# DJjjjhao/FIRA-ICSE

Measured on AMD Instinct MI355X. Metric: training commits/sec (FIRA default config), higher is better.
Workload: dtype f32; 1 GPU; BASELINE configs[1]: FIRA training step (fwd+bwd+Adam, dropout 0.1/0.2), batch 32 commits/GPU, fp32, 650-node graphs (mean nnz 1066/graph), vocab 24650; global_batch=32, parallelism=dp1

## Files before the change

### fira_icse_amd/_lib.py

```python
from __future__ import annotations

import ctypes as C
import os

HERE = os.path.dirname(os.path.abspath(__file__))
LIB_PATH = os.environ.get("FIRA_HIP_LIB") or os.path.join(HERE, "libfira_hip.so")


class FiraError(RuntimeError):
    pass


class Dims(C.Structure):
    _fields_ = [("sou_len", C.c_int32), ("sub_len", C.c_int32), ("ast_len", C.c_int32), ("tar_len", C.c_int32),
                ("d_model", C.c_int32), ("n_head", C.c_int32), ("n_layer", C.c_int32), ("vocab", C.c_int32),
                ("ast_vocab", C.c_int32), ("d_ff", C.c_int32)]


class Batch(C.Structure):
    _fields_ = [("B", C.c_int32), ("nnz", C.c_int32), ("sou", C.c_void_p), ("tar", C.c_void_p), ("mark", C.c_void_p),
                ("ast_change", C.c_void_p), ("tar_label", C.c_void_p), ("sub_token", C.c_void_p),
                ("n_nodes", C.c_int32), ("node_rows", C.c_void_p), ("rowptr", C.c_void_p), ("col", C.c_void_p),
                ("val", C.c_void_p), ("n_code", C.c_int32), ("code_rows", C.c_void_p), ("code_mark", C.c_void_p),
                ("n_mem", C.c_int32), ("mem_rows", C.c_void_p), ("mem_dst", C.c_void_p), ("head_rows", C.c_void_p),
                ("n_head_rows", C.c_int32), ("n_emb_items", C.c_int32), ("emb_item_tok", C.c_void_p),
                ("emb_item_ptr", C.c_void_p), ("emb_rows", C.c_void_p), ("n_ast_items", C.c_int32),
                ("ast_rows", C.c_void_p), ("ast_ids", C.c_void_p), ("dec_off", C.c_void_p), ("n_dec_rows", C.c_int32),
                ("dec_off_host", C.c_void_p)]


class TrainOpts(C.Structure):
    _fields_ = [("dropout", C.c_float), ("gcn_dropout", C.c_float), ("seed", C.c_uint64), ("compact_head", C.c_int32),
                ("dtype", C.c_int32), ("compact_dec", C.c_int32), ("zero_grads", C.c_int32)]


class LrSchedule(C.Structure):
    _fields_ = [("kind", C.c_int32), ("base_lr", C.c_float), ("warmup_steps", C.c_int32), ("decay_steps", C.c_int32),
                ("min_lr", C.c_float)]


class AdamOpts(C.Structure):
    _fields_ = [("lr", C.c_float), ("beta1", C.c_float), ("beta2", C.c_float), ("eps", C.c_float), ("step", C.c_int32),
                ("m", C.c_void_p), ("v", C.c_void_p), ("sched", C.POINTER(LrSchedule))]


def sched_ptr(sched):
    return None if sched is None else C.pointer(sched)


class ClipState(C.Structure):
    _fields_ = [("sq", C.c_float * 4), ("norm", C.c_float), ("coef", C.c_float), ("zero_flag", C.c_int32),
                ("n_clipped", C.c_int32), ("n_nonfinite", C.c_int32), ("reserved", C.c_int32 * 7)]


_P, _I, _F, _L, _Z = C.c_void_p, C.c_int, C.c_float, C.c_int64, C.c_size_t
_U64, _U32 = C.c_uint64, C.c_uint32
_DP, _BP, _OP = C.POINTER(Dims), C.POINTER(Batch), C.POINTER(TrainOpts)

SIGNATURES = {
    "fira_last_error": (C.c_char_p, []),
    "fira_abi_version": (_I, []),
    "fira_param_count": (_I, [_DP]),
    "fira_param_info": (_I, [_DP, _I, C.c_char_p, C.POINTER(_L), C.POINTER(_L), C.POINTER(C.c_int32), C.POINTER(_L)]),
    "fira_param_total": (_L, [_DP]),
    "fira_workspace_bytes": (_Z, [_DP, _I, _I]),
    "fira_decode_workspace_bytes": (_Z, [_DP, _I, _I]),
    "fira_decode_workspace_bytes_ex": (_Z, [_DP, _I, _I, _I]),
    "fira_gemm_f32": (_I, [_P, _I, _I, _I, _I, _I, _P, _I, _P, _I, _P, _I, _P, _I, _I]),
    "fira_gemm_bf16": (_I, [_P, _I, _I, _I, _I, _I, _P, _I, _P, _I, _P, _I, _P, _I, _I]),
    "fira_weight_shadow": (_I, [_P, _I, _I, _P, _P, _P]),
    "fira_gemm_bf16_wb": (_I, [_P, _I, _I, _I, _P, _I, _P, _I, _P, _I, _P, _I, _I]),
    "fira_csr_spmm_f32": (_I, [_P, _I, _P, _P, _P, _P, _I, _P, _I, _I, _I]),
    "fira_csr_spmm": (_I, [_P, _I, _L, _P, _P, _P, _P, _I, _P, _I, _I, _I, _I]),
    "fira_gcn_layer_fwd": (_I, [_P, _I, _P, _P, _P, _P, _P, _P, _P, _P, _P, _P, _P, _P, _P, _F, _U64, _U32, _I]),
    "fira_gcn_layer_bwd": (_I, [_P, _I, _P, _P, _P, _P, _P, _P, _P, _I]),
    "fira_gcn_weight_planes": (_I, [_P, _I, _P, _P]),
    "fira_linear_x3": (_I, [_P, _I, _I, _P, _I, _P, _P, _P, _I, _I]),
    "fira_linear_dgrad_x3": (_I, [_P, _I, _I, _P, _I, _P, _P, _I, _I, _I]),
    "fira_dgrad_x3_splitk_planes_bytes": (_Z, [_I]),
    "fira_dgrad_x3_splitk": (_I, [_P, _I, _I, _P, _I, _P, _P, _P, _I, _I]),
    "fira_head_logits_x3_scratch_bytes": (_Z, [_I]),
    "fira_head_logits_x3": (_I, [_P, _I, _I, _P, _I, _P, _P, _P, _I, _P]),
    "fira_combination_block_fwd": (_I, [_P, _I, _P, _P, _P, _P, _P, _P, _P, _I, _P, _P, _P, _P, _P, _P, _P, _P, _P, _F, _U64, _U32, _U32, _I]),
    "fira_combination_block_bwd": (_I, [_P, _I, _P, _P, _P, _P, _P, _P, _P, _P, _P, _I, _P, _P, _P, _P, _P, _P, _I, _P, _F, _U64, _U32, _U32, _I]),
    "fira_combination_block_bwd_part_floats": (_I, []),
    "fira_embed_gather_fwd": (_I, [_P, _I, _I, _P, _P, _P, _P, _I, _I]),
    "fira_embed_gather_bwd": (_I, [_P, _I, _I, _P, _P, _P, _I, _I, _I]),
    "fira_combination_fwd": (_I, [_P, _I, _P, _P, _P, _P, _F, _U64, _U32]),
    "fira_combination_bwd": (_I, [_P, _I, _P, _P, _P, _P, _P, _P, _F, _U64, _U32]),
    "fira_add_layernorm_fwd": (_I, [_P, _I, _P, _P, _P, _P, _P, _P, _F, _U64, _U32]),
    "fira_linear_presum_f32": (_I, [_P, _I, _I, _P, _I, _P, _P, _P, _P, _F, _U64, _U32]),
    "fira_ln_linear_f32": (_I, [_P, _I, _I, _P, _I, _P, _P, _P, _I, _I, _P, _P, _P, _P]),
    "fira_ln_bwd_linear_f32": (_I, [_P, _I, _I, _P, _P, _P, _P, _P, _P, _P, _P, _P, _P, _P, _P, _F, _U64, _U32]),
    "fira_linear_layernorm_bf16_fwd": (_I, [_P, _I, _P, _I, _P, _I, _P, _P, _P, _P, _P, _P, _P, _F, _U64, _U32]),
    "fira_add_layernorm_bwd": (_I, [_P, _I, _P, _P, _P, _P, _P, _P, _P, _P, _F, _U64, _U32]),
    "fira_dropout_mask": (_I, [_P, _U64, _U32, _L, _F, _P]),
    "fira_colsum_f32": (_I, [_P, _I, _I, _P, _I, _P]),
    "fira_attention_fwd": (_I, [_P, _I, _I, _I, _I, _P, _I, _P, _I, _P, _I, _P, _I, _I, _P, _I]),
    "fira_attention_bwd": (_I, [_P, _I, _I, _I, _I, _P, _I, _P, _I, _P, _I, _P, _I, _I, _P, _I, _P, _I,
                                _P, _I, _P, _I, _P, _I]),
    "fira_attention_fwd_ex": (_I, [_P, _I, _I, _I, _I, _P, _I, _P, _I, _P, _I, _P, _I, _I, _P, _I, _P, _I, _I, _P]),
    "fira_attention_bwd_ex": (_I, [_P, _I, _I, _I, _I, _P, _I, _P, _I, _P, _I, _P, _I, _I, _P, _I, _P, _I,
                                   _P, _I, _P, _I, _P, _I, _P, _I, _I, _P]),
    "fira_decode_attention": (_I, [_P, _I, _I, _I, _P, _I, _P, _I, _P, _I, _P, _P, _I, _I, _I, _I, _P, _P, _I, _P, _P, _P]),
    "fira_copy_score_fwd": (_I, [_P, _I, _I, _I, _P, _P, _P, _P, _P]),
    "fira_copy_score_bwd": (_I, [_P, _I, _I, _I, _P, _P, _P, _P, _P, _P, _P, _P]),
    "fira_head_loss": (_I, [_P, _I, _I, _I, _I, _P, _P, _I, _P, _P, _P, _P, _P, _P, _P, _I]),
    "fira_adam_step": (_I, [_P, _L, _P, _P, _P, _P, _F, _F, _F, _F, _I, _P]),
    "fira_adam_step_mb": (_I, [_P, _L, _P, _P, _P, _P, _P, _F, _F, _F, _F, _I, _P, _P]),
    "fira_inv_count": (_I, [_P, _P, _P]),
    "fira_adam_step_count": (_I, [_P, _L, _P, _P, _P, _P, _F, _F, _F, _F, _I, _P]),
    "fira_pack_stats": (_I, [_P, _P, _P, _P]),
    "fira_debug_chain": (_I, [_P, _I, _I, _P]),
    "fira_train_fwd_bwd": (_I, [_P, _DP, _BP, _P, _P, _P, _Z, _OP, _P, _P, _P]),
    "fira_train_step": (_I, [_P, _DP, _BP, _P, _P, _P, _Z, _OP, _P, _P, C.POINTER(AdamOpts)]),
    "fira_gemm_wgrad_panel": (_I, [_P, _I, _I, _I, _I, _P, _I, _P, _I, _P, _I, _P, _P, _Z]),
    "fira_ffn_fwd": (_I, [_P, _I, _I] + [_P] * 11 + [_F, _U64, _U32, _I]),
    "fira_ffn_bwd": (_I, [_P, _I, _I] + [_P] * 17 + [_F, _U64, _U32, _I]),
    "fira_head_topk": (_I, [_P, _I, _I, _I, _P, _P, _P, _P, _I, _P, _P, _I]),
    "fira_train_step_rows": (_I, [_P, _DP, _BP, _P, _P, _P, _Z, _OP, _P, _P, C.POINTER(AdamOpts), _P]),
    "fira_adam_rows_sync": (_I, [_P, _DP, _P, C.POINTER(AdamOpts), _P]),
    "fira_adam_rows_catchup": (_I, [_P, _DP, _P, C.POINTER(AdamOpts), _P, _I, _P, _I]),
    "fira_adam_rows_step": (_I, [_P, _DP, _P, _P, C.POINTER(AdamOpts), _P, _P, _P, _I]),
    "fira_train_step_begin_rows": (_I, [_P, _DP, _BP, _P, _P, _P, _Z, _OP, _P, _P, _P, C.POINTER(AdamOpts), _P]),
    "fira_train_step_end_rows": (_I, [_P, _P, C.POINTER(AdamOpts), _P, _P, _P]),
    "fira_grad_sqsum_scratch_bytes": (_Z, []),
    "fira_grad_sqsum": (_I, [_P, _L, _P, _P, _I, _P]),
    "fira_clip_finish": (_I, [_P, _P, _I, _P, _P, _F]),
    "fira_adam_step_clip": (_I, [_P, _L, _P, _P, _P, _P, _F, _F, _F, _F, _I, _P, _P, _P]),
    "fira_adam_rows_step_clip": (_I, [_P, _DP, _P, _P, C.POINTER(AdamOpts), _P, _P, _P, _I, _P]),
    "fira_train_step_clip": (_I, [_P, _DP, _BP, _P, _P, _P, _Z, _OP, _P, _P, C.POINTER(AdamOpts), _P, _F, _P, _P]),
    "fira_lr_at": (_F, [C.POINTER(LrSchedule), _I]),
    "fira_lr_schedule_check": (_I, [C.POINTER(LrSchedule)]),
    "fira_train_step_begin": (_I, [_P, _DP, _BP, _P, _P, _P, _Z, _OP, _P, _P, _P]),
    "fira_train_step_end": (_I, [_P, _P, C.POINTER(AdamOpts), _P, _P]),
    "fira_f32_to_bf16": (_I, [_P, _L, _P, _P]),
    "fira_bf16_to_f32": (_I, [_P, _L, _P, _P]),
    "fira_prof_enable": (None, [_I]),
    "fira_prof_report": (_I, [_I, C.POINTER(C.c_double), C.POINTER(C.c_double), C.POINTER(C.c_double), C.POINTER(_L)]),
    "fira_param_groups": (_I, [_DP, C.POINTER(_L), C.POINTER(_L)]),
    "fira_host_node_lists": (_I, [_I, _I, _I, _I, _I] + [_P] * 7 + [_I] + [_P] * 14),
    "fira_host_collate_csr": (_I, [_I, _I, _P, _L, _P, _P, _P, _P, _P, _P, _P]),
    "fira_forward_dev": (_I, [_P, _DP, _BP, _P, _P, _Z, _P, _P, _P, _I]),
    "fira_dev_bleu_stats": (_I, [_P, _I, _I, _I, _I, _I, _P, _P, _P, _P, _P, _P]),
    "fira_mbr_bleu_stats": (_I, [_P, _I, _I, _I, _P, _P, _P]),
    "fira_constrain_dist": (_I, [_P, _DP, _I, _I, _P, _P, _P, _P, _I, _I, _P, _I, _P, _P, _P]),
    "fira_merge_dist": (_I, [_P, _DP, _I, _I, _P, _P, _P, _P, _P]),
    "fira_mix_dist": (_I, [_P, _I, _I, _I, C.POINTER(_P), C.POINTER(_F), _P, _P, _P]),
    "fira_decode_begin": (_I, [_P, _DP, _BP, _P, _P, _Z, _I]),
    "fira_decode_begin_ex": (_I, [_P, _DP, _BP, _P, _P, _Z, _I, _I]),
    "fira_decode_step_ex": (_I, [_P, _DP, _P, _P, _Z, _I, _I, _I, _P, _P, _P, _P, _P, _I]),
    "fira_beam_prepare": (_I, [_P, _I, _I, _I, _I, _P, _P, _P, _P, _P, _P]),
    "fira_beam_select": (_I, [_P, _DP, _I, _I, _P, _P, _P, _P, _P, _P, _P, _P, _P, _P, _P, _P, _P]),
    "fira_beam_select_scored": (_I, [_P, _DP, _I, _I, _P, _P, _P, _P, _P, _P, _P, _P, _P, _P, _P, _P, _P, _P, _I, _F, _P]),
    "fira_greedy_advance": (_I, [_P, _DP, _I, _I, _P, _P, _P, _P, _P, _P, _P, _P, _P, _P]),
    "fira_decode_step": (_I, [_P, _DP, _P, _P, _Z, _I, _I, _I, _P, _P, _P, _P, _P]),
    "fira_decode_step_sample": (_I, [_P, _DP, _P, _P, _Z, _I, _I, _I, _P, _P, _P, _F, _I, _F, _P, _P, _P, _I]),
    "fira_decode_step_score": (_I, [_P, _DP, _P, _P, _Z, _I, _I, _I] + [_P] * 15 + [_I]),
    "fira_sample_advance": (_I, [_P, _DP, _I, _I, _I, _P, _P, _P, _P, _P, _P, _P, _P, _P, _P, _P]),
    "fira_decoder_forward": (_I, [_P, _DP, _P, _P, _Z, _I, _P, _P, _P, _P]),
    "fira_decode_memory": (_P, [_DP, _P, _I, _I]),
    "fira_decode_mem_valid": (_P, [_DP, _P, _I, _I]),
}


def _ensure_built():
    if os.path.exists(LIB_PATH):
        return
    import fcntl
    from . import build as _build
    with open(os.path.join(HERE, ".build.lock"), "w") as lock:
        fcntl.flock(lock, fcntl.LOCK_EX)
        try:
            if not os.path.exists(LIB_PATH):
                _build.build()
        finally:
            fcntl.flock(lock, fcntl.LOCK_UN)


def load():
    try:
        _ensure_built()
    except Exception as e:
        raise ImportError(
            "fira_icse_amd: %s is missing and could not be built (%s). Build it with `python -m fira_icse_amd.build` "
            "(needs hipcc, gfx950). There is no CPU fallback." % (LIB_PATH, e))
    lib = C.CDLL(LIB_PATH)
    if lib.fira_abi_version() != 10:
        raise ImportError("libfira_hip.so ABI version mismatch")
    for name, (res, args) in SIGNATURES.items():
        fn = getattr(lib, name)
        fn.restype = res
        fn.argtypes = args
    return lib


_lib = None


def lib():
    global _lib
    if _lib is None:
        _lib = load()
    return _lib


_host_warned = False
_host_failed = False


def host_lib():
    global _host_warned, _host_failed
    if _host_failed:
        return None
    try:
        return lib()
    except (ImportError, OSError, AttributeError) as e:
        _host_failed = True
        if not _host_warned:
            _host_warned = True
            import warnings
            warnings.warn("fira_icse_amd: libfira_hip.so unavailable (%s); host collate falls back to numpy" % (e,))
        return None


def check(rc: int, what: str = ""):
    if rc != 0:
        msg = lib().fira_last_error()
        raise FiraError("%s failed: %s" % (what or "libfira_hip call", msg.decode() if msg else "unknown error"))


def ptr(t):
    return None if t is None else C.c_void_p(t.data_ptr())


def cur_stream():
    import torch
    return C.c_void_p(torch.cuda.current_stream().cuda_stream)


def make_dims(cfg) -> Dims:
    return Dims(cfg.sou_len, cfg.sub_token_len, cfg.ast_change_len, cfg.tar_len, cfg.embedding_dim, cfg.num_head,
                cfg.num_layers, cfg.vocab_size, cfg.ast_change_vocab_size, 4 * cfg.embedding_dim)
```

### fira_icse_amd/csrc/attention.hip

```cpp
#include "engine.h"
#include "epilogue.h"
#include "mfma_frag.h"

namespace fira {

constexpr float SQRT_DH = 5.656854249492381f;
constexpr float INV_SQRT_DH = 1.0f / SQRT_DH;
constexpr int MAX_TK = 384;

constexpr float LOG2E = 1.4426950408889634f;
constexpr float SCORE2 = INV_SQRT_DH * LOG2E;
constexpr float MASKED2 = -1e9f * LOG2E;
__device__ __forceinline__ constexpr int acc_c(int s) { return (s & 3) + 8 * (s >> 2); }
__device__ __forceinline__ uint32_t low_bits(int n) { return n <= 0 ? 0u : (n >= 32 ? 0xffffffffu : (1u << n) - 1u); }
__device__ __forceinline__ float bit_select(int sel, float a, float b) {
    return __int_as_float((sel & __float_as_int(a)) | (~sel & __float_as_int(b)));
}
__device__ __forceinline__ int bit_of(uint32_t word, int c) { return __builtin_amdgcn_sbfe((int)word, c, 1); }

__device__ __forceinline__ void buf_frag(float (&f)[16], rsrc_t r, unsigned off) {
#pragma unroll
    for (int i = 0; i < 4; ++i) {
        const f32x4v v = __builtin_bit_cast(f32x4v, __builtin_amdgcn_raw_buffer_load_b128(r, off + 16u * i, 0, 0));
        f[4 * i + 0] = v.x; f[4 * i + 1] = v.y; f[4 * i + 2] = v.z; f[4 * i + 3] = v.w;
    }
}
__device__ __forceinline__ void buf_rows(float (&f)[16], rsrc_t r, unsigned off0, unsigned ld4) {
#pragma unroll
    for (int s = 0; s < 16; ++s) f[s] = buf_load_f32(r, off0 + (unsigned)acc_c(s) * ld4);
}
__device__ __forceinline__ rsrc_t rows_rsrc(const float* base, int n, int ld) {
    return buf_rsrc(base, n > 0 ? (unsigned)(n - 1) * (unsigned)ld * 4u + 128u : 0u);
}

struct AttnRanges { int qb, tq, k0, tk; };
__device__ __forceinline__ AttnRanges attn_ranges(const int32_t* __restrict__ q_off, const int32_t* __restrict__ k_off, int b,
                                                  int bk, int Tq, int Tk, bool selfk, int lane) {
    int v = 0;
    const int32_t* src = nullptr;
    if (lane < 2 && q_off) src = q_off + b + lane;
    if (lane >= 2 && lane < 4 && k_off && !selfk) src = k_off + bk + (lane - 2);
    if (src) v = *src;
    AttnRanges r;
    r.qb = q_off ? __builtin_amdgcn_readlane(v, 0) : b * Tq;
    r.tq = q_off ? __builtin_amdgcn_readlane(v, 1) - r.qb : Tq;
    r.k0 = (k_off && !selfk) ? __builtin_amdgcn_readlane(v, 2) : 0;
    r.tk = selfk ? r.tq : (k_off ? min(__builtin_amdgcn_readlane(v, 3) - r.k0, Tk) : Tk);
    return r;
}

struct TileMask {
    bool ok;
    uint32_t valid;
    uint32_t outside;
    bool live;
};
__device__ __forceinline__ TileMask tile_mask(int kvld, int n_in, int kh) {
    TileMask m;
    m.ok = kvld != 0;
    const uint32_t vbits = (uint32_t)__ballot(m.ok);
    m.live = vbits != 0;
    m.valid = vbits >> (4 * kh);
    m.outside = ~low_bits(n_in) >> (4 * kh);
    return m;
}

template <int NW, bool BF>
__global__ __launch_bounds__(NW * 64) void attention_fwd_kernel(int H, int Tq, int Tk, const float* __restrict__ Q,
                                                                int ldq, const float* __restrict__ K, int ldk,
                                                                const float* __restrict__ V, int ldv,
                                                                const int32_t* __restrict__ key_valid, int causal,
                                                                int q_pos0, float* __restrict__ O, int ldo, int kb,
                                                                int kvb, int qpk, const int32_t* __restrict__ q_off,
                                                                int self_kv, const int32_t* __restrict__ k_off) {
    __shared__ float sm_red[NW][32];
    __shared__ float sm_o[NW > 1 ? NW * 1024 : 1];
    const int b = blockIdx.x / H, h = blockIdx.x % H;
    const int bk = b / qpk;
    const int t = threadIdx.x, lane = t & 63, wave = t >> 6;
    const int l31 = lane & 31, kh = lane >> 5;
    const bool selfk = q_off && self_kv;
    const AttnRanges rg = attn_ranges(q_off, k_off, b, bk, Tq, Tk, selfk, lane);
    const int qb = rg.qb, tq = rg.tq, k0 = rg.k0, tk = rg.tk;
    const int NT = (tk + 31) / 32;
    if (tk <= 0) {
        for (int idx = t; idx < tq * FIRA_DH; idx += NW * 64)
            O[((size_t)qb + idx / FIRA_DH) * ldo + h * FIRA_DH + idx % FIRA_DH] = 0.f;
        return;
    }
    const size_t krow0 = selfk ? (size_t)qb : (k_off ? (size_t)k0 : (size_t)bk * kb);
    const rsrc_t rQ = rows_rsrc(Q + (size_t)qb * ldq + h * FIRA_DH, tq, ldq);
    const rsrc_t rK = rows_rsrc(K + krow0 * ldk + h * FIRA_DH, tk, ldk);
    const rsrc_t rV = rows_rsrc(V + krow0 * ldv + h * FIRA_DH, tk, ldv);
    const rsrc_t rO = rows_rsrc(O + (size_t)qb * ldo + h * FIRA_DH, tq, ldo);
    const rsrc_t rM = buf_rsrc(key_valid + (k_off && !selfk ? (size_t)k0 : (size_t)bk * kvb), (unsigned)tk * 4u);
    const unsigned ldk4 = (unsigned)ldk * 4u, ldv4 = (unsigned)ldv * 4u, ldo4 = (unsigned)ldo * 4u;
    const int kt = wave;
    const bool mine = kt < NT;

    float bq[16], ak[16], vv[16];
    int kvld = 0;
    buf_frag(bq, rQ, (unsigned)l31 * (unsigned)ldq * 4u + (unsigned)kh * 64u);
    if (mine) {
        buf_frag(ak, rK, (unsigned)(kt * 32 + l31) * ldk4 + (unsigned)kh * 64u);
        buf_rows(vv, rV, (unsigned)(kt * 32 + 4 * kh) * ldv4 + (unsigned)l31 * 4u, ldv4);
        kvld = __builtin_amdgcn_raw_buffer_load_b32(rM, (unsigned)(kt * 32 + l31) * 4u, 0, 0);
    }
    const TileMask tm = tile_mask(kvld, tk - kt * 32, kh);
    const bool live = mine && tm.live;
    const uint32_t maskedT = ~tm.valid | (causal ? ~low_bits(l31 + q_pos0 - kt * 32 - 4 * kh + 1) : 0u);

    f32x16 st;
    float mx = -INFINITY;
    if (live) {
#pragma unroll
        for (int s = 0; s < 16; ++s) vv[s] = bit_select(bit_of(tm.valid, acc_c(s)), vv[s], 0.f);
        f32x16 acc;
#pragma unroll
        for (int r = 0; r < 16; ++r) acc[r] = 0.f;
        acc = chain16<BF>(ak, bq, acc);
#pragma unroll
        for (int r = 0; r < 16; ++r) {
            float x = bit_select(bit_of(maskedT, acc_c(r)), MASKED2, acc[r] * SCORE2);
            x = bit_select(bit_of(tm.outside, acc_c(r)), -INFINITY, x);
            st[r] = x;
            mx = fmaxf(mx, x);
        }
    } else {
#pragma unroll
        for (int r = 0; r < 16; ++r) {
            const float x = mine ? bit_select(bit_of(tm.outside, acc_c(r)), -INFINITY, MASKED2) : -INFINITY;
            st[r] = x;
            mx = fmaxf(mx, x);
        }
    }
    mx = fmaxf(mx, __shfl_xor(mx, 32, 64));
    if (NW > 1) {
        if (kh == 0) sm_red[wave][l31] = mx;
        __syncthreads();
#pragma unroll
        for (int w = 0; w < NW; ++w) mx = fmaxf(mx, sm_red[w][l31]);
        __syncthreads();
    }
    float sum = 0.f;
#pragma unroll
    for (int r = 0; r < 16; ++r) {
        const float p = __builtin_amdgcn_exp2f(st[r] - mx);
        st[r] = p;
        sum += p;
    }
    sum += __shfl_xor(sum, 32, 64);
    if (NW > 1) {
        if (kh == 0) sm_red[wave][l31] = sum;
        __syncthreads();
        sum = 0.f;
#pragma unroll
        for (int w = 0; w < NW; ++w) sum += sm_red[w][l31];
    }
    const float inv_sum = 1.0f / sum;
    f32x16 o;
#pragma unroll
    for (int r = 0; r < 16; ++r) o[r] = 0.f;
    if (live) {
        float pn[16];
#pragma unroll
        for (int s = 0; s < 16; ++s) pn[s] = st[s] * inv_sum;
        o = chain16<BF>(pn, vv, o);
    }
    if (NW > 1) {
        const int nwa = min(NW, NT);
        if (wave < nwa) {
#pragma unroll
            for (int r = 0; r < 16; ++r) sm_o[wave * 1024 + r * 64 + lane] = o[r];
        }
        __syncthreads();
        for (int idx = t; idx < 1024; idx += NW * 64) {
            float v = 0.f;
            for (int w = 0; w < nwa; ++w) v += sm_o[w * 1024 + idx];
            const int r = idx >> 6, ln = idx & 63;
            __builtin_amdgcn_raw_buffer_store_b32(__float_as_int(v), rO,
                                                  (unsigned)acc_row(r, ln >> 5) * ldo4 + (unsigned)(ln & 31) * 4u, 0, 0);
        }
    } else {
#pragma unroll
        for (int r = 0; r < 16; ++r)
            __builtin_amdgcn_raw_buffer_store_b32(__float_as_int(o[r]), rO,
                                                  (unsigned)(4 * kh + acc_c(r)) * ldo4 + (unsigned)l31 * 4u, 0, 0);
    }
}

template <int NW, bool BF>
__global__ __launch_bounds__(NW * 64) void attention_bwd_kernel(
    int H, int Tq, int Tk, const float* __restrict__ Q, int ldq, const float* __restrict__ K, int ldk,
    const float* __restrict__ V, int ldv, const int32_t* __restrict__ key_valid, int causal, int q_pos0,
    const float* __restrict__ O, int ldo, const float* __restrict__ dO, int lddo, float* __restrict__ dQ, int lddq,
    float* __restrict__ dK, int lddk, float* __restrict__ dV, int lddv, const int32_t* __restrict__ q_off, int self_kv,
    const int32_t* __restrict__ k_off) {
    __shared__ float sm_red[NW][32];
    __shared__ __attribute__((aligned(16))) float sm_m[32], sm_sum[32], sm_delta[32];
    __shared__ float sm_o[NW > 1 ? NW * 1024 : 1];
    const int b = blockIdx.x / H, h = blockIdx.x % H;
    const int t = threadIdx.x, lane = t & 63, wave = t >> 6;
    const int l31 = lane & 31, kh = lane >> 5;
    const bool selfk = q_off && self_kv;
    const AttnRanges rg = attn_ranges(q_off, k_off, b, b, Tq, Tk, selfk, lane);
    const int qb = rg.qb, tq = rg.tq, k0 = rg.k0, tk = rg.tk;
    const size_t kbase = selfk ? (size_t)qb : (k_off ? (size_t)k0 : (size_t)b * Tk);
    const int NT = (tk + 31) / 32;
    if (tk <= 0) {
        for (int idx = t; idx < tq * FIRA_DH; idx += NW * 64)
            dQ[((size_t)qb + idx / FIRA_DH) * lddq + h * FIRA_DH + idx % FIRA_DH] = 0.f;
        return;
    }
    const rsrc_t rQ = rows_rsrc(Q + (size_t)qb * ldq + h * FIRA_DH, tq, ldq);
    const rsrc_t rO = rows_rsrc(O + (size_t)qb * ldo + h * FIRA_DH, tq, ldo);
    const rsrc_t rdO = rows_rsrc(dO + (size_t)qb * lddo + h * FIRA_DH, tq, lddo);
    const rsrc_t rdQ = rows_rsrc(dQ + (size_t)qb * lddq + h * FIRA_DH, tq, lddq);
    const rsrc_t rK = rows_rsrc(K + kbase * ldk + h * FIRA_DH, tk, ldk);
    const rsrc_t rV = rows_rsrc(V + kbase * ldv + h * FIRA_DH, tk, ldv);
    const rsrc_t rdK = rows_rsrc(dK + kbase * lddk + h * FIRA_DH, tk, lddk);
    const rsrc_t rdV = rows_rsrc(dV + kbase * lddv + h * FIRA_DH, tk, lddv);
    const rsrc_t rM = buf_rsrc(key_valid + (k_off && !selfk ? (size_t)k0 : (size_t)b * Tk), (unsigned)tk * 4u);
    const unsigned ldq4 = (unsigned)ldq * 4u, ldk4 = (unsigned)ldk * 4u, ldv4 = (unsigned)ldv * 4u;
    const unsigned lddo4 = (unsigned)lddo * 4u, lddq4 = (unsigned)lddq * 4u, lddk4 = (unsigned)lddk * 4u, lddv4 = (unsigned)lddv * 4u;
    const int kt = wave;
    const bool mine = kt < NT;

    float bq[16], bdo[16], bo[16];
    const unsigned fq = (unsigned)kh * 64u;
    buf_frag(bq, rQ, (unsigned)l31 * ldq4 + fq);
    buf_frag(bdo, rdO, (unsigned)l31 * lddo4 + fq);
    buf_frag(bo, rO, (unsigned)l31 * (unsigned)ldo * 4u + fq);
    float ak[16], av[16], kvv[16];
    float qrow[16], dorow[16];
    int kvld = 0;
    if (mine) {
        const unsigned krow = (unsigned)(kt * 32 + l31);
        buf_frag(ak, rK, krow * ldk4 + fq);
        buf_frag(av, rV, krow * ldv4 + fq);
        buf_rows(kvv, rK, (unsigned)(kt * 32 + 4 * kh) * ldk4 + (unsigned)l31 * 4u, ldk4);
        kvld = __builtin_amdgcn_raw_buffer_load_b32(rM, krow * 4u, 0, 0);
        buf_rows(qrow, rQ, (unsigned)(4 * kh) * ldq4 + (unsigned)l31 * 4u, ldq4);
        buf_rows(dorow, rdO, (unsigned)(4 * kh) * lddo4 + (unsigned)l31 * 4u, lddo4);
    }
    const TileMask tm = tile_mask(kvld, tk - kt * 32, kh);
    const bool live = mine && tm.live;
    const uint32_t maskedT = ~tm.valid | (causal ? ~low_bits(l31 + q_pos0 - kt * 32 - 4 * kh + 1) : 0u);
    float delta;
    {
        float d = 0.f;
#pragma unroll
        for (int s = 0; s < 16; ++s) d = fmaf(bdo[s], bo[s], d);
        delta = d + __shfl_xor(d, 32, 64);
    }

    f32x16 st;
    float mx = -INFINITY;
    if (live) {
#pragma unroll
        for (int s = 0; s < 16; ++s) kvv[s] = bit_select(bit_of(tm.valid, acc_c(s)), kvv[s], 0.f);
        if (!tm.ok) {
#pragma unroll
            for (int s = 0; s < 16; ++s) { ak[s] = 0.f; av[s] = 0.f; }
        }
        f32x16 acc;
#pragma unroll
        for (int r = 0; r < 16; ++r) acc[r] = 0.f;
        acc = chain16<BF>(ak, bq, acc);
#pragma unroll
        for (int r = 0; r < 16; ++r) {
            float x = bit_select(bit_of(maskedT, acc_c(r)), MASKED2, acc[r] * SCORE2);
            x = bit_select(bit_of(tm.outside, acc_c(r)), -INFINITY, x);
            st[r] = x;
            mx = fmaxf(mx, x);
        }
    } else {
#pragma unroll
        for (int r = 0; r < 16; ++r) {
            const float x = mine ? bit_select(bit_of(tm.outside, acc_c(r)), -INFINITY, MASKED2) : -INFINITY;
            st[r] = x;
            mx = fmaxf(mx, x);
        }
    }
    mx = fmaxf(mx, __shfl_xor(mx, 32, 64));
    if (NW > 1) {
        if (kh == 0) sm_red[wave][l31] = mx;
        __syncthreads();
#pragma unroll
        for (int w = 0; w < NW; ++w) mx = fmaxf(mx, sm_red[w][l31]);
        __syncthreads();
    }
    float sum = 0.f;
#pragma unroll
    for (int r = 0; r < 16; ++r) {
        const float p = __builtin_amdgcn_exp2f(st[r] - mx);
        st[r] = p;
        sum += p;
    }
    sum += __shfl_xor(sum, 32, 64);
    if (NW > 1) {
        if (kh == 0) sm_red[wave][l31] = sum;
        __syncthreads();
        sum = 0.f;
#pragma unroll
        for (int w = 0; w < NW; ++w) sum += sm_red[w][l31];
    }
    const float inv_sum = 1.0f / sum;
    if (wave == 0 && kh == 0) {
        sm_m[l31] = mx;
        sm_sum[l31] = inv_sum;
        sm_delta[l31] = delta;
    }
    __syncthreads();

    f32x16 dq;
#pragma unroll
    for (int r = 0; r < 16; ++r) dq[r] = 0.f;
    if (live) {
        f32x16 dpt;
#pragma unroll
        for (int r = 0; r < 16; ++r) dpt[r] = 0.f;
        dpt = chain16<BF>(av, bdo, dpt);
        float dsv[16];
        const float sc = inv_sum * INV_SQRT_DH;
#pragma unroll
        for (int s = 0; s < 16; ++s)
            dsv[s] = bit_select(bit_of(maskedT, acc_c(s)), 0.f, st[s] * sc * (dpt[s] - delta));
        dq = chain16<BF>(dsv, kvv, dq);
    }
    if (NW > 1) {
        const int nwa = min(NW, NT);
        if (wave < nwa) {
#pragma unroll
            for (int r = 0; r < 16; ++r) sm_o[wave * 1024 + r * 64 + lane] = dq[r];
        }
        __syncthreads();
        for (int idx = t; idx < 1024; idx += NW * 64) {
            float v = 0.f;
            for (int w = 0; w < nwa; ++w) v += sm_o[w * 1024 + idx];
            const int r = idx >> 6, ln = idx & 63;
            __builtin_amdgcn_raw_buffer_store_b32(__float_as_int(v), rdQ,
                                                  (unsigned)acc_row(r, ln >> 5) * lddq4 + (unsigned)(ln & 31) * 4u, 0, 0);
        }
    } else {
#pragma unroll
        for (int r = 0; r < 16; ++r)
            __builtin_amdgcn_raw_buffer_store_b32(__float_as_int(dq[r]), rdQ,
                                                  (unsigned)(4 * kh + acc_c(r)) * lddq4 + (unsigned)l31 * 4u, 0, 0);
    }

    if (mine) {
        f32x16 dk, dv;
#pragma unroll
        for (int r = 0; r < 16; ++r) { dk[r] = 0.f; dv[r] = 0.f; }
        if (live) {
            float qm[16], qs[16], qd[16];
#pragma unroll
            for (int g = 0; g < 4; ++g) {
                const f32x4v m4 = *reinterpret_cast<const f32x4v*>(&sm_m[4 * kh + 8 * g]);
                const f32x4v s4 = *reinterpret_cast<const f32x4v*>(&sm_sum[4 * kh + 8 * g]);
                const f32x4v d4 = *reinterpret_cast<const f32x4v*>(&sm_delta[4 * kh + 8 * g]);
#pragma unroll
                for (int j = 0; j < 4; ++j) { qm[4 * g + j] = m4[j]; qs[4 * g + j] = s4[j]; qd[4 * g + j] = d4[j]; }
            }
            f32x16 sN, dpN;
#pragma unroll
            for (int r = 0; r < 16; ++r) { sN[r] = 0.f; dpN[r] = 0.f; }
            sN = chain16<BF>(bq, ak, sN);
            dpN = chain16<BF>(bdo, av, dpN);
            const int key = kt * 32 + l31;
            const uint32_t maskedN = tm.ok ? (causal ? low_bits(key - q_pos0 - 4 * kh) : 0u) : 0xffffffffu;
            const float gone = key < tk ? MASKED2 : -INFINITY;
            float pv[16], dsn[16];
#pragma unroll
            for (int s = 0; s < 16; ++s) {
                const int sel = bit_of(maskedN, acc_c(s));
                const float x = bit_select(sel, gone, sN[s] * SCORE2);
                const float p = __builtin_amdgcn_exp2f(x - qm[s]) * qs[s];
                pv[s] = p;
                dsn[s] = bit_select(sel, 0.f, p * (dpN[s] - qd[s]) * INV_SQRT_DH);
            }
            dk = chain16<BF>(dsn, qrow, dk);
            dv = chain16<BF>(pv, dorow, dv);
        }
#pragma unroll
        for (int r = 0; r < 16; ++r) {
            const unsigned row = (unsigned)(kt * 32 + 4 * kh + acc_c(r));
            __builtin_amdgcn_raw_buffer_store_b32(__float_as_int(dk[r]), rdK, row * lddk4 + (unsigned)l31 * 4u, 0, 0);
            __builtin_amdgcn_raw_buffer_store_b32(__float_as_int(dv[r]), rdV, row * lddv4 + (unsigned)l31 * 4u, 0, 0);
        }
    }
}

__device__ __forceinline__ f32x4v widen4(uint2 u) {
    return f32x4v{__uint_as_float(u.x << 16), __uint_as_float(u.x & 0xffff0000u), __uint_as_float(u.y << 16),
                  __uint_as_float(u.y & 0xffff0000u)};
}
template <int NSLOT, bool KV16>
__global__ __launch_bounds__(256) void decode_attention_kernel(int H, int Tk, const float* __restrict__ Q, int ldq,
                                                               const void* __restrict__ Kv, int ldk,
                                                               const void* __restrict__ Vv, int ldv,
                                                               const int32_t* __restrict__ key_valid, float* __restrict__ O,
                                                               int ldo, int kb, int kvb, int qpk,
                                                               const float* __restrict__ Knew,
                                                               const float* __restrict__ Vnew, int ldn,
                                                               float* __restrict__ Kc_out, float* __restrict__ Vc_out,
                                                               const int32_t* __restrict__ k_off) {
    __shared__ int sm_list[MAX_TK];
    __shared__ int sm_cnt[8];
    __shared__ float sm_f[4][36];
    const int bk = blockIdx.x / H, h = blockIdx.x % H;
    const int t = threadIdx.x, lane = t & 63, wave = t >> 6;
    const int r = lane >> 3, c = lane & 7;
    int nv;
    const int kbeg = k_off ? k_off[bk] : 0;
    if (k_off) Tk = min(Tk, k_off[bk + 1] - kbeg);
    const size_t krow0 = k_off ? (size_t)kbeg : (size_t)bk * kb;
    {
        const int32_t* kvp = key_valid + (k_off ? (size_t)kbeg : (size_t)bk * kvb);
        const int k0 = t, k1 = t + 256;
        const bool v0 = k0 < Tk && kvp[k0] != 0;
        const bool v1 = k1 < Tk && kvp[k1] != 0;
        const unsigned long long m0 = __ballot(v0), m1 = __ballot(v1);
        if (lane == 0) { sm_cnt[wave] = __popcll(m0); sm_cnt[4 + wave] = __popcll(m1); }
        __syncthreads();
        int base0 = 0, base1 = 0, tot0 = 0, tot1 = 0;
#pragma unroll
        for (int w = 0; w < 4; ++w) {
            const int c0 = sm_cnt[w], c1 = sm_cnt[4 + w];
            if (w < wave) { base0 += c0; base1 += c1; }
            tot0 += c0; tot1 += c1;
        }
        nv = tot0 + tot1;
        const unsigned long long below = (1ull << lane) - 1ull;
        if (v0) sm_list[base0 + __popcll(m0 & below)] = k0;
        if (v1) sm_list[tot0 + base1 + __popcll(m1 & below)] = k1;
        __syncthreads();
    }
    const size_t hoff = (size_t)h * FIRA_DH + c * 4;
    const float* K = static_cast<const float*>(Kv);
    const float* V = static_cast<const float*>(Vv);
    const float* Kb = K + krow0 * ldk + hoff;
    const float* Vb = V + krow0 * ldv + hoff;
    const uint16_t* Kh = static_cast<const uint16_t*>(Kv) + krow0 * ldk + hoff;
    const uint16_t* Vh = static_cast<const uint16_t*>(Vv) + krow0 * ldv + hoff;
    f32x4v kf[NSLOT], vf[NSLOT];
    bool have[NSLOT];
#pragma unroll
    for (int j = 0; j < NSLOT; ++j) {
        const int idx = j * 32 + wave * 8 + r;
        have[j] = idx < nv;
        const int key = have[j] ? sm_list[idx] : 0;
        const float* pk = Kb + (size_t)key * ldk;
        const float* pv = Vb + (size_t)key * ldv;
        if (Knew && key == Tk - 1) {
            pk = Knew + (size_t)bk * ldn + hoff;
            pv = Vnew + (size_t)bk * ldn + hoff;
        }
        if (KV16) {
            kf[j] = have[j] ? widen4(*reinterpret_cast<const uint2*>(Kh + (size_t)key * ldk)) : f32x4v{0.f, 0.f, 0.f, 0.f};
            vf[j] = have[j] ? widen4(*reinterpret_cast<const uint2*>(Vh + (size_t)key * ldv)) : f32x4v{0.f, 0.f, 0.f, 0.f};
        } else {
            kf[j] = have[j] ? *reinterpret_cast<const f32x4v*>(pk) : f32x4v{0.f, 0.f, 0.f, 0.f};
            vf[j] = have[j] ? *reinterpret_cast<const f32x4v*>(pv) : f32x4v{0.f, 0.f, 0.f, 0.f};
        }
    }
    if (Knew && Kc_out && t < 16) {
        const int cc = t & 7;
        const size_t src = (size_t)bk * ldn + (size_t)h * FIRA_DH + cc * 4;
        const size_t dst = ((size_t)bk * kb + (Tk - 1)) * ldk + (size_t)h * FIRA_DH + cc * 4;
        if (t < 8) *reinterpret_cast<f32x4v*>(Kc_out + dst) = *reinterpret_cast<const f32x4v*>(Knew + src);
        else *reinterpret_cast<f32x4v*>(Vc_out + ((size_t)bk * kb + (Tk - 1)) * ldv + (size_t)h * FIRA_DH + cc * 4) =
                 *reinterpret_cast<const f32x4v*>(Vnew + src);
    }
    for (int qi = 0; qi < qpk; ++qi) {
        const int b = bk * qpk + qi;
        const f32x4v q4 = *reinterpret_cast<const f32x4v*>(Q + (size_t)b * ldq + hoff);
        float sc[NSLOT];
        float mx = -INFINITY;
#pragma unroll
        for (int j = 0; j < NSLOT; ++j) {
            float d = q4.x * kf[j].x;
            d = fmaf(q4.y, kf[j].y, d); d = fmaf(q4.z, kf[j].z, d); d = fmaf(q4.w, kf[j].w, d);
            d = sum8(d);
            sc[j] = have[j] ? d * INV_SQRT_DH : -INFINITY;
            mx = fmaxf(mx, sc[j]);
        }
        mx = wave_max(mx);
        if (lane == 0) sm_f[wave][33] = mx;
        __syncthreads();
        mx = fmaxf(fmaxf(sm_f[0][33], sm_f[1][33]), fmaxf(sm_f[2][33], sm_f[3][33]));
        f32x4v acc = {0.f, 0.f, 0.f, 0.f};
        float sum = 0.f;
#pragma unroll
        for (int j = 0; j < NSLOT; ++j) {
            const float p = have[j] ? __expf(sc[j] - mx) : 0.f;
            sum += p;
            acc += vf[j] * p;
        }
        sum += dpp_take<DPP_ROR8, 0xf>(sum, sum);
        acc.x += dpp_take<DPP_ROR8, 0xf>(acc.x, acc.x); acc.y += dpp_take<DPP_ROR8, 0xf>(acc.y, acc.y);
        acc.z += dpp_take<DPP_ROR8, 0xf>(acc.z, acc.z); acc.w += dpp_take<DPP_ROR8, 0xf>(acc.w, acc.w);
#pragma unroll
        for (int o = 16; o < 64; o <<= 1) {
            sum += __shfl_xor(sum, o, 64);
            acc.x += __shfl_xor(acc.x, o, 64); acc.y += __shfl_xor(acc.y, o, 64);
            acc.z += __shfl_xor(acc.z, o, 64); acc.w += __shfl_xor(acc.w, o, 64);
        }
        if (lane < 8) {
            *reinterpret_cast<f32x4v*>(&sm_f[wave][lane * 4]) = acc;
            if (lane == 0) sm_f[wave][34] = sum;
        }
        __syncthreads();
        if (t < 32) {
            const float tot = (sm_f[0][34] + sm_f[1][34]) + (sm_f[2][34] + sm_f[3][34]);
            const float o = (sm_f[0][t] + sm_f[1][t]) + (sm_f[2][t] + sm_f[3][t]);
            O[(size_t)b * ldo + (size_t)h * FIRA_DH + t] = nv > 0 ? o / tot : 0.f;
        }
        __syncthreads();
    }
}

__global__ __launch_bounds__(256) void decode_self_block_kernel(int Tk, int T, const float* __restrict__ qkv,
                                                                float* __restrict__ Kc, float* __restrict__ Vc,
                                                                const int32_t* __restrict__ hist,
                                                                const float* __restrict__ WoT, const float* __restrict__ bo,
                                                                const float* __restrict__ xres,
                                                                const float* __restrict__ gamma, const float* __restrict__ beta,
                                                                const float* __restrict__ WqT, const float* __restrict__ bq,
                                                                float* __restrict__ xa, float* __restrict__ qc) {
    __shared__ __attribute__((aligned(16))) float s_q[FIRA_D], s_o[FIRA_D], s_x[FIRA_D];
    __shared__ float s_p[8][32];
    __shared__ float s_red[2][4];
    __shared__ __attribute__((aligned(16))) float s_part[4][FIRA_D];
    const int row = blockIdx.x, t = threadIdx.x, lane = t & 63, wave = t >> 6;
    const float* my = qkv + (size_t)row * 3 * FIRA_D;
    const float knew = my[FIRA_D + t], vnew = my[2 * FIRA_D + t];
    s_q[t] = my[t];
    float* kc_row = Kc + (size_t)row * T * FIRA_D;
    float* vc_row = Vc + (size_t)row * T * FIRA_D;
    kc_row[(size_t)(Tk - 1) * FIRA_D + t] = knew;
    vc_row[(size_t)(Tk - 1) * FIRA_D + t] = vnew;
    __syncthreads();
    {
        const int h = t >> 5, j = t & 31;
        const bool valid = j < Tk && hist[(size_t)row * T + j] != 0;
        const float* kp = (j == Tk - 1) ? my + FIRA_D + h * FIRA_DH : kc_row + (size_t)min(j, Tk - 1) * FIRA_D + h * FIRA_DH;
        float d = 0.f;
#pragma unroll
        for (int c = 0; c < FIRA_DH / 4; ++c) {
            const f32x4v k4 = *reinterpret_cast<const f32x4v*>(kp + c * 4);
            const f32x4v q4 = *reinterpret_cast<const f32x4v*>(&s_q[h * FIRA_DH + c * 4]);
            d = fmaf(q4.x, k4.x, d); d = fmaf(q4.y, k4.y, d); d = fmaf(q4.z, k4.z, d); d = fmaf(q4.w, k4.w, d);
        }
        const float sc = valid ? d * INV_SQRT_DH : -INFINITY;
        float mx = sc;
#pragma unroll
        for (int o = 1; o < 32; o <<= 1) mx = fmaxf(mx, __shfl_xor(mx, o, 64));
        const float pr = valid ? __expf(sc - mx) : 0.f;
        float sum = pr;
#pragma unroll
        for (int o = 1; o < 32; o <<= 1) sum += __shfl_xor(sum, o, 64);
        s_p[h][j] = sum > 0.f ? pr / sum : 0.f;
    }
    __syncthreads();
    {
        const int h = t >> 5;
        float o = 0.f;
        int j = 0;
        for (; j + 4 <= Tk - 1; j += 4) {
            const float v0 = vc_row[(size_t)j * FIRA_D + t], v1 = vc_row[(size_t)(j + 1) * FIRA_D + t];
            const float v2 = vc_row[(size_t)(j + 2) * FIRA_D + t], v3 = vc_row[(size_t)(j + 3) * FIRA_D + t];
            o = fmaf(s_p[h][j], v0, o); o = fmaf(s_p[h][j + 1], v1, o); o = fmaf(s_p[h][j + 2], v2, o); o = fmaf(s_p[h][j + 3], v3, o);
        }
        for (; j < Tk - 1; ++j) o = fmaf(s_p[h][j], vc_row[(size_t)j * FIRA_D + t], o);
        o = fmaf(s_p[h][Tk - 1], vnew, o);
        s_o[t] = o;
    }
    __syncthreads();
    auto matvec = [&](const float* __restrict__ WT, const float* v, float bias_n) -> float {
        f32x4v acc = {0.f, 0.f, 0.f, 0.f};
        const float* wp = WT + (size_t)(wave * 64) * FIRA_D + lane * 4;
#pragma unroll
        for (int k0 = 0; k0 < 64; k0 += 16) {
            f32x4v w[16];
#pragma unroll
            for (int u = 0; u < 16; ++u) w[u] = *reinterpret_cast<const f32x4v*>(wp + (size_t)(k0 + u) * FIRA_D);
#pragma unroll
            for (int u = 0; u < 16; ++u) acc += w[u] * v[wave * 64 + k0 + u];
        }
        __syncthreads();
        *reinterpret_cast<f32x4v*>(&s_part[wave][lane * 4]) = acc;
        __syncthreads();
        return bias_n + ((s_part[0][t] + s_part[1][t]) + (s_part[2][t] + s_part[3][t]));
    };
    const float sres = matvec(WoT, s_o, bo[t]) + xres[(size_t)row * FIRA_D + t];
    float part = wave_sum(sres);
    if (lane == 0) s_red[0][wave] = part;
    __syncthreads();
    const float mean = ((s_red[0][0] + s_red[0][1]) + (s_red[0][2] + s_red[0][3])) * (1.0f / FIRA_D);
    const float dv = sres - mean;
    part = wave_sum(dv * dv);
    if (lane == 0) s_red[1][wave] = part;
    __syncthreads();
    const float var = ((s_red[1][0] + s_red[1][1]) + (s_red[1][2] + s_red[1][3])) * (1.0f / FIRA_D);
    const float y = dv * (1.0f / sqrtf(var + 1e-5f)) * gamma[t] + beta[t];
    xa[(size_t)row * FIRA_D + t] = y;
    s_x[t] = y;
    __syncthreads();
    qc[(size_t)row * FIRA_D + t] = matvec(WqT, s_x, bq[t]);
}
int decode_self_block(hipStream_t s, int BR, int Tk, int T, const float* qkv, float* Kc, float* Vc, const int32_t* hist,
                      const float* WoT, const float* bo, const float* xres, const float* gamma, const float* beta,
                      const float* WqT, const float* bq, float* xa, float* qc) {
    ProfScope prof(s, PROF_ATTN, 0.0);
    if (BR <= 0) return 0;
    FIRA_REQUIRE(Tk >= 1 && Tk <= 32 && Tk <= T, "decode_self_block: %d keys (at most 32)", Tk);
    hipLaunchKernelGGL(decode_self_block_kernel, dim3(BR), dim3(256), 0, s, Tk, T, qkv, Kc, Vc, hist, WoT, bo, xres, gamma, beta,
                       WqT, bq, xa, qc);
    FIRA_CHECK_LAUNCH("decode_self_block");
    return 0;
}

int decode_attention_kv16(hipStream_t s, int BR, int H, int Tk, const float* Q, int ldq, const uint16_t* K, int ldk,
                          const uint16_t* V, int ldv, const int32_t* key_valid, float* O, int ldo, int kb, int kvb, int qpk,
                          const int32_t* k_off) {
    ProfScope prof(s, PROF_ATTN, 0.0);
    if (BR <= 0) return 0;
    FIRA_REQUIRE(Tk >= 1 && Tk <= MAX_TK && qpk >= 1 && BR % qpk == 0 && kb >= Tk && kvb >= Tk, "decode_attention: bad geometry");
    FIRA_REQUIRE(ldq % 4 == 0 && ldk % 4 == 0 && ldv % 4 == 0 && (uintptr_t)Q % 16 == 0 && (uintptr_t)K % 8 == 0 &&
                     (uintptr_t)V % 8 == 0, "decode_attention: rows must be 8-byte (bf16) / 16-byte (fp32) aligned");
    const dim3 grid((BR / qpk) * H);
    if (Tk <= 32)
        hipLaunchKernelGGL((decode_attention_kernel<1, true>), grid, dim3(256), 0, s, H, Tk, Q, ldq, K, ldk, V, ldv, key_valid, O,
                           ldo, kb, kvb, qpk, nullptr, nullptr, 0, nullptr, nullptr, k_off);
    else
        hipLaunchKernelGGL((decode_attention_kernel<12, true>), grid, dim3(256), 0, s, H, Tk, Q, ldq, K, ldk, V, ldv, key_valid, O,
                           ldo, kb, kvb, qpk, nullptr, nullptr, 0, nullptr, nullptr, k_off);
    FIRA_CHECK_LAUNCH("decode_attention_kv16");
    return 0;
}
int decode_attention(hipStream_t s, int BR, int H, int Tk, const float* Q, int ldq, const float* K, int ldk,
                     const float* V, int ldv, const int32_t* key_valid, float* O, int ldo, int kb, int kvb, int qpk,
                     const float* Knew, const float* Vnew, int ldn, float* Kc_out, float* Vc_out, const int32_t* k_off) {
    ProfScope prof(s, PROF_ATTN, 0.0);
    if (BR <= 0) return 0;
    FIRA_REQUIRE(Tk >= 1 && Tk <= MAX_TK && qpk >= 1 && BR % qpk == 0 && kb >= Tk && kvb >= Tk, "decode_attention: bad geometry");
    FIRA_REQUIRE(ldq % 4 == 0 && ldk % 4 == 0 && ldv % 4 == 0 && (uintptr_t)Q % 16 == 0 && (uintptr_t)K % 16 == 0 &&
                     (uintptr_t)V % 16 == 0 && (!Knew || (ldn % 4 == 0 && (uintptr_t)Knew % 16 == 0 && (uintptr_t)Vnew % 16 == 0)),
                 "decode_attention: rows must be 16-byte aligned");
    FIRA_REQUIRE(!Knew || (qpk == 1 && !k_off), "decode_attention: merged new keys need one query per K/V entry and dense key rows");
    const dim3 grid((BR / qpk) * H);
    if (Tk <= 32)
        hipLaunchKernelGGL((decode_attention_kernel<1, false>), grid, dim3(256), 0, s, H, Tk, Q, ldq, K, ldk, V, ldv, key_valid, O,
                           ldo, kb, kvb, qpk, Knew, Vnew, ldn, Kc_out, Vc_out, k_off);
    else
        hipLaunchKernelGGL((decode_attention_kernel<12, false>), grid, dim3(256), 0, s, H, Tk, Q, ldq, K, ldk, V, ldv, key_valid, O,
                           ldo, kb, kvb, qpk, Knew, Vnew, ldn, Kc_out, Vc_out, k_off);
    FIRA_CHECK_LAUNCH("decode_attention");
    return 0;
}

static int check_geometry(const char* who, int Tq, int Tk, int ldq, int ldk, int ldv, const void* Q, const void* K,
                          const void* V) {
    FIRA_REQUIRE(Tq >= 1 && Tq <= 32, "%s: Tq=%d must be in 1..32", who, Tq);
    FIRA_REQUIRE(Tk >= 1 && Tk <= MAX_TK, "%s: Tk=%d must be in 1..%d", who, Tk, MAX_TK);
    FIRA_REQUIRE(ldq % 4 == 0 && ldk % 4 == 0 && ldv % 4 == 0 && (uintptr_t)Q % 16 == 0 && (uintptr_t)K % 16 == 0 &&
                     (uintptr_t)V % 16 == 0,
                 "%s: Q/K/V rows must be 16-byte aligned", who);
    return 0;
}

int attention_fwd_ex(hipStream_t s, int B, int H, int Tq, int Tk, const float* Q, int ldq, const float* K, int ldk,
                     const float* V, int ldv, const int32_t* key_valid, int causal, int q_pos0, float* O, int ldo,
                     int kb, int kvb, int qpk, const int32_t* q_off, int self_kv, int bf16, const int32_t* k_off) {
    ProfScope prof(s, PROF_ATTN, 0.0);
    if (B <= 0) return 0;
    if (int e = check_geometry("attention_fwd", Tq, Tk, ldq, ldk, ldv, Q, K, V)) return e;
    FIRA_REQUIRE(kb >= Tk && kvb >= Tk && qpk >= 1, "attention_fwd: bad batch strides");
#define FIRA_ATT_FWD(NW_, BF_)                                                                                      \
    hipLaunchKernelGGL((attention_fwd_kernel<NW_, BF_>), dim3(B * H), dim3(NW_ * 64), 0, s, H, Tq, Tk, Q, ldq, K, ldk, V, \
                       ldv, key_valid, causal, q_pos0, O, ldo, kb, kvb, qpk, q_off, self_kv, k_off)
    if (Tk <= 32) { if (bf16) FIRA_ATT_FWD(1, true); else FIRA_ATT_FWD(1, false); }
    else { if (bf16) FIRA_ATT_FWD(12, true); else FIRA_ATT_FWD(12, false); }
#undef FIRA_ATT_FWD
    FIRA_CHECK_LAUNCH("attention_fwd");
    return 0;
}
int attention_fwd(hipStream_t s, int B, int H, int Tq, int Tk, const float* Q, int ldq, const float* K, int ldk,
                  const float* V, int ldv, const int32_t* key_valid, int causal, int q_pos0, float* O, int ldo,
                  const int32_t* q_off, int self_kv, int bf16, const int32_t* k_off) {
    return attention_fwd_ex(s, B, H, Tq, Tk, Q, ldq, K, ldk, V, ldv, key_valid, causal, q_pos0, O, ldo, Tk, Tk, 1, q_off, self_kv,
                            bf16, k_off);
}

int attention_bwd(hipStream_t s, int B, int H, int Tq, int Tk, const float* Q, int ldq, const float* K, int ldk,
                  const float* V, int ldv, const int32_t* key_valid, int causal, int q_pos0, const float* O, int ldo,
                  const float* dO, int lddo, float* dQ, int lddq, float* dK, int lddk, float* dV, int lddv,
                  const int32_t* q_off, int self_kv, int bf16, const int32_t* k_off) {
    ProfScope prof(s, PROF_ATTN, 0.0);
    if (B <= 0) return 0;
    if (int e = check_geometry("attention_bwd", Tq, Tk, ldq, ldk, ldv, Q, K, V)) return e;
    FIRA_REQUIRE(ldo % 4 == 0 && lddo % 4 == 0 && (uintptr_t)O % 16 == 0 && (uintptr_t)dO % 16 == 0,
                 "attention_bwd: O/dO rows must be 16-byte aligned");
#define FIRA_ATT_BWD(NW_, BF_)                                                                                      \
    hipLaunchKernelGGL((attention_bwd_kernel<NW_, BF_>), dim3(B * H), dim3(NW_ * 64), 0, s, H, Tq, Tk, Q, ldq, K, ldk, V, \
                       ldv, key_valid, causal, q_pos0, O, ldo, dO, lddo, dQ, lddq, dK, lddk, dV, lddv, q_off, self_kv, k_off)
    if (Tk <= 32) { if (bf16) FIRA_ATT_BWD(1, true); else FIRA_ATT_BWD(1, false); }
    else { if (bf16) FIRA_ATT_BWD(12, true); else FIRA_ATT_BWD(12, false); }
#undef FIRA_ATT_BWD
    FIRA_CHECK_LAUNCH("attention_bwd");
    return 0;
}

}

extern "C" {
int fira_attention_fwd(void* stream, int B, int H, int Tq, int Tk, const float* Q, int ldq, const float* K, int ldk,
                       const float* V, int ldv, const int32_t* key_valid, int causal, int q_pos0, float* O, int ldo) {
    return fira::attention_fwd((hipStream_t)stream, B, H, Tq, Tk, Q, ldq, K, ldk, V, ldv, key_valid, causal, q_pos0, O,
                               ldo);
}
int fira_decode_attention(void* stream, int BR, int H, int Tk, const float* Q, int ldq, const float* K, int ldk,
                          const float* V, int ldv, const int32_t* key_valid, float* O, int ldo, int kb, int kvb, int qpk,
                          const float* Knew, const float* Vnew, int ldn, float* Kc_out, float* Vc_out,
                          const int32_t* k_off) {
    FIRA_REQUIRE(Q && K && V && key_valid && O, "fira_decode_attention: null pointer argument");
    return fira::decode_attention((hipStream_t)stream, BR, H, Tk, Q, ldq, K, ldk, V, ldv, key_valid, O, ldo, kb, kvb, qpk, Knew,
                                  Vnew, ldn, Kc_out, Vc_out, k_off);
}
int fira_attention_bwd(void* stream, int B, int H, int Tq, int Tk, const float* Q, int ldq, const float* K, int ldk,
                       const float* V, int ldv, const int32_t* key_valid, int causal, int q_pos0, const float* O,
                       int ldo, const float* dO, int lddo, float* dQ, int lddq, float* dK, int lddk, float* dV,
                       int lddv) {
    return fira::attention_bwd((hipStream_t)stream, B, H, Tq, Tk, Q, ldq, K, ldk, V, ldv, key_valid, causal, q_pos0, O,
                               ldo, dO, lddo, dQ, lddq, dK, lddk, dV, lddv);
}
int fira_attention_fwd_ex(void* stream, int B, int H, int Tq, int Tk, const float* Q, int ldq, const float* K, int ldk,
                          const float* V, int ldv, const int32_t* key_valid, int causal, int q_pos0, float* O, int ldo,
                          const int32_t* q_off, int self_kv, int dtype, const int32_t* k_off) {
    FIRA_REQUIRE(dtype == FIRA_F32 || dtype == FIRA_BF16, "fira_attention_fwd_ex: dtype must be FIRA_F32 or FIRA_BF16");
    FIRA_REQUIRE(!(k_off && self_kv), "fira_attention_fwd_ex: k_off (ragged memory rows) and self_kv exclude each other");
    return fira::attention_fwd((hipStream_t)stream, B, H, Tq, Tk, Q, ldq, K, ldk, V, ldv, key_valid, causal, q_pos0, O,
                               ldo, q_off, self_kv, dtype == FIRA_BF16, k_off);
}
int fira_attention_bwd_ex(void* stream, int B, int H, int Tq, int Tk, const float* Q, int ldq, const float* K, int ldk,
                          const float* V, int ldv, const int32_t* key_valid, int causal, int q_pos0, const float* O,
                          int ldo, const float* dO, int lddo, float* dQ, int lddq, float* dK, int lddk, float* dV,
                          int lddv, const int32_t* q_off, int self_kv, int dtype, const int32_t* k_off) {
    FIRA_REQUIRE(dtype == FIRA_F32 || dtype == FIRA_BF16, "fira_attention_bwd_ex: dtype must be FIRA_F32 or FIRA_BF16");
    FIRA_REQUIRE(!(k_off && self_kv), "fira_attention_bwd_ex: k_off (ragged memory rows) and self_kv exclude each other");
    return fira::attention_bwd((hipStream_t)stream, B, H, Tq, Tk, Q, ldq, K, ldk, V, ldv, key_valid, causal, q_pos0, O,
                               ldo, dO, lddo, dQ, lddq, dK, lddk, dV, lddv, q_off, self_kv, dtype == FIRA_BF16, k_off);
}
}
```

### fira_icse_amd/csrc/engine.h

```cpp
#pragma once
#include "common.h"
#include <string>
#include <vector>

namespace fira {

int gemm_f32(hipStream_t s, int tA, int tB, int M, int N, int K, const float* A, int lda, const float* B, int ldb,
             float* C, int ldc, const float* bias, int flags, int splitk);
int gemm_f32_ex(hipStream_t s, int tA, int tB, int M, int N, int K, const float* A, int lda, const float* B, int ldb,
                float* C, int ldc, const float* bias, int flags, int splitk, float* colsum,
                const int32_t* c_rows = nullptr, const float* relu_mask = nullptr);
int gemm_bf16_ex(hipStream_t s, int tA, int tB, int M, int N, int K, const float* A, int lda, const float* B, int ldb,
                 float* C, int ldc, const float* bias, int flags, int splitk, float* colsum,
                 const int32_t* c_rows = nullptr, const float* relu_mask = nullptr);
struct ShadowEntry { int64_t offset; int rows, cols, pitch_t; int64_t offset_t; };
constexpr int SHADOW_MAX = 64;
struct ShadowTable {
    int n = 0;
    int64_t wbt_elems = 0;
    int tile_start[SHADOW_MAX + 1] = {0};
    ShadowEntry e[SHADOW_MAX];
};
int weight_shadows(hipStream_t s, const ShadowTable& tab, const float* P, uint16_t* Wb, uint16_t* WbT);
int gemm_bf16_wb_ex(hipStream_t s, int M, int N, int K, const float* A, int lda, const uint16_t* Bb, int ldb, float* C,
// ... 1 lines not shown
                    const float* relu_mask = nullptr);
int gemm_bf16_group_add_wgrad(hipStream_t s, int M, int N, int K, const float* A, int lda, const float* B, int ldb,
                              float* C, int ldc, float* colsum, int max_split = 0);
int gemm_bf16_group_flush(hipStream_t s);
bool gemm_bf16_takes(int M, int N, int K);
void gemm_bf16_group_reset();
bool gemm_bf16_group_full();
bool gemm_wgrad_panel_takes(int M, int N, int K, const float* A, int lda, const float* B, int ldb, int ldc);
void gemm_wgrad_panel_reset();
bool gemm_wgrad_panel_full();
int gemm_wgrad_panel_pending();
int gemm_wgrad_panel_add(int M, int N, int K, const float* A, int lda, const float* B, int ldb, float* C, int ldc, float* colsum);
int gemm_wgrad_panel_flush(hipStream_t s, int np);
void gemm_wgrad_panel_scratch(float* buf, size_t n_floats);
int gemm_wgrad_panel(hipStream_t s, int np, int M, int N, int K, const float* A, int lda, const float* B, int ldb, float* C,
                     int ldc, float* colsum);
int gemm_group_add_wgrad(hipStream_t s, int M, int N, int K, const float* A, int lda, const float* B, int ldb, float* C,
                         int ldc, float* colsum, int max_split = 0);
int gemm_group_flush(hipStream_t s);
void gemm_group_reset();
bool gemm_group_full();
void gemm_set_pad_stream(hipStream_t s);
struct EpiRes;
bool gemm_tile32_takes(int tB, int M, int N, int K, const float* A, int lda, const float* B, int ldb);
bool gemm_tile32_try(hipStream_t s, int tB, int M, int N, int K, const float* A, int lda, const float* B, int ldb,
                     float* C, int ldc, const float* bias, int flags, int* rc, const int32_t* c_rows,
                     const float* relu_mask, const int32_t* a_rows, const EpiRes* er);
bool gemm_tile32_ln_try(hipStream_t s, int M, int N, const float* S, int lds, const float* W, const float* bias, float* Y,
                        int ldy, int flags, const float* gamma, const float* beta, float* x_out, float* stats_out, int* rc);
int gemm_tile32_lnb_blocks(int M);
bool gemm_tile32_lnb_try(hipStream_t s, int M, int N, const float* dy, const float* W, int ldw, float* dX, int lddx,
                         const float* relu_mask, const float* sum, const float* stats, const float* gamma, float* ds,
                         float* dx_drop, float* part, float dropout, uint64_t seed, uint32_t site, int* rc,
                         uint32_t idx0 = 0);
bool gemm_small_try(hipStream_t s, int tA, int tB, int M, int N, int K, const float* A, int lda, const float* B, int ldb,
                    float* C, int ldc, const float* bias, int flags, int* rc, const int32_t* c_rows = nullptr,
                    const float* relu_mask = nullptr);
int csr_spmm(hipStream_t s, int n_rows, const int32_t* rowptr, const int32_t* col, const float* val, const float* X,
             int ldx, float* Y, int ldy, int graph_rows, int variant);
int csr_spmm_ex(hipStream_t s, int n_rows, const int32_t* rowptr, const int32_t* col, const float* val, const float* X,
                int ldx, float* Y, int ldy, int graph_rows, int variant, int accum, float* rowsum);
int gcn_fused_fwd(hipStream_t s, int n_rows, const int32_t* rowptr, const int32_t* col, const float* val, const float* X,
                  const float* Wk, const float* bias, const float* r1_col, const float* gamma, const float* beta, float* sum,
                  float* y, float* stats, float* rowsum_out, const int32_t* slot2, float* y2, float dropout, uint64_t seed,
                  uint32_t site, int bf16, const uint16_t* Wx = nullptr);
int gcn_fused_bwd(hipStream_t s, int n_rows, const int32_t* rowptr, const int32_t* col, const float* val, const float* dY,
                  const float* Wk, float* u_out, float* acc_out, int bf16, const uint16_t* Wx = nullptr);
int gcn_split_planes(hipStream_t s, int n, const float* const* src, uint16_t* const* dst);
size_t head_logits_x3_scratch_elems(int R);
int head_logits_x3(hipStream_t s, int R, int V, const float* x, int ldx, const float* W, const float* bias, float* out, int ldo,
                   uint16_t* xplanes);
int transpose256(hipStream_t s, int nl, const float* W, float* Wt);
int linear_x3(hipStream_t s, int M, const float* X, int ldx, const uint16_t* Wx, int nb, const float* bias, float* out, int ldo,
              bool one_plane);
int split_planes_t(hipStream_t s, const float* W, int V, uint16_t* planes, bool one_plane);
int dgrad_x3_splitk(hipStream_t s, int M, int K, const float* A, int lda, const uint16_t* Wx, float* out, int ldo, bool one_plane);
int linear_x3_kacc(hipStream_t s, int M, const float* A, int lda, const uint16_t* Wx, int nkb, float* out, int ldo, bool accum,
                   bool one_plane);
int comb_fused_fwd(hipStream_t s, int n_rows, const float* Xc, const float* WqT, const float* WkT, const float* WoT,
                   const float* bqk, const float* bo, const float* vtab, int ldv, const int32_t* mark, float* qk, float* c,
                   const float* gamma, const float* beta, float* sum, float* y, const int32_t* y_rows, float* stats,
                   float dropout, uint64_t seed, uint32_t site_gate, uint32_t site_out, int bf16, const uint16_t* Wx = nullptr);
int comb_fused_bwd_parts();
int comb_fused_bwd(hipStream_t s, int n_rows, float* dG, const int32_t* rows, const float* sum, const float* stats,
                   const float* gamma, const float* Wo, const float* Wqk, const float* qk, const float* vtab, int ldv,
                   const int32_t* mark, float* dYc, float* dqk, float* part_ln, float* part_v, float dropout, uint64_t seed,
                   uint32_t site_gate, uint32_t site_out, int bf16, const uint16_t* WTx = nullptr);
struct TransposeTable { int n = 0; const float* src[24]; float* dst[24]; };
int transpose256_table(hipStream_t s, const TransposeTable& tab);
int embed_gather_fwd(hipStream_t s, int B, int L, const int32_t* idx, const float* table, const float* pos, float* out,
                     int out_bstride, int out_off);
int embed_grouped_bwd(hipStream_t s, int n_items, const int32_t* item_tok, const int32_t* item_ptr, const int32_t* rows,
                      float* dtable, const float* dnode);
int embed_list_bwd_small(hipStream_t s, int n, const int32_t* rows, const int32_t* ids, float* dtable, const float* dnode,
                         int table_rows);
int embed_gather_bwd(hipStream_t s, int B, int L, const int32_t* idx, float* dtable, const float* dout,
                     int out_bstride, int out_off, int padding_idx);
int embed_gather_bwd_small(hipStream_t s, int B, int L, const int32_t* idx, float* dtable, const float* dout,
                           int out_bstride, int out_off, int padding_idx, int table_rows);
int combination_fwd(hipStream_t s, int M, const float* qk, const float* vtab, int ldv, const int32_t* mark, float* out,
                    float dropout, uint64_t seed, uint32_t site);
int combination_bwd(hipStream_t s, int M, const float* qk, const float* vtab, int ldv, const int32_t* mark,
                    const float* dout, float* dqk, float* dvtab, int lddv, float dropout, uint64_t seed, uint32_t site,
                    float* part = nullptr);
int combination_bwd_blocks(int M);
struct RedEntry { float* dst; const float* src; int width, n_part, stride; };
constexpr int RED_MAX = 96;
struct RedTable {
    int n = 0;
    int wg_start[RED_MAX + 1] = {0};
    RedEntry e[RED_MAX];
};
int deferred_reduce(hipStream_t s, RedTable& tab);
int add_layernorm_fwd(hipStream_t s, int M, float* x, const float* res, const float* gamma, const float* beta,
                      float* y, float* stats, float dropout, uint64_t seed, uint32_t site, const int32_t* y_rows, const float* r1_row = nullptr,
                      const float* r1_col = nullptr,
                      const int32_t* slot2 = nullptr, float* y2 = nullptr,
                      uint32_t idx0 = 0);
bool gemm_bf16_k256_try(hipStream_t s, int M, int N, int K, const float* A, int lda, const uint16_t* Bb, int ldb, float* C,
                        int ldc, const float* bias, int flags, const int32_t* c_rows, const float* relu_mask, int* rc);
bool linear_ln_bf16_try(hipStream_t s, int M, int K, const float* X, int ldx, const uint16_t* Wb, int ldb, const float* bias,
                        const float* res, const float* gamma, const float* beta, float* sum, float* y, float* stats,
                        float dropout, uint64_t seed, uint32_t site, const int32_t* y_rows, const float* r1_row,
                        const float* r1_col, int* rc, bool force = false);
int add_layernorm_bwd(hipStream_t s, int M, const float* dy, const float* sum, const float* stats, const float* gamma,
                      float* ds, float* dx_drop, float* dgamma, float* dbeta, float dropout, uint64_t seed,
                      uint32_t site, const int32_t* rows = nullptr,
                      float* part = nullptr,
                      const float* row_w = nullptr, uint32_t idx0 = 0);
int add_layernorm_bwd_blocks(int M);
int gcn_bias_unfold(hipStream_t s, const float* W2, const float* b1, const float* dc, float* dW2, float* db1);
struct UnfoldEntry { const float *W2, *b1, *dc; float *dW2, *db1; };
struct UnfoldTable { int n = 0; UnfoldEntry e[16]; };
int gcn_bias_unfold_all(hipStream_t s, const UnfoldTable& tab);
int gcn_fold_weights(hipStream_t s, int n_layers, const float* const* W2, const float* const* W1, const float* const* b1,
                     float* W21, float* W21t, float* c21);
int gcn_unfold_products(hipStream_t s, int n_layers, const float* const* dW21, const float* const* W1, const float* const* W2,
                        float* const* dW1, float* const* dW2);
int colsum(hipStream_t s, int M, int N, const float* X, int ldx, float* out, const float* row_weight = nullptr);
int rank2_rows(hipStream_t s, int M, const float* g, const float* w, float* out);
int prep(hipStream_t s, int B, int L, int S, int T, const int32_t* sou, const int32_t* sub, const int32_t* tar,
         int32_t* mem_valid, int32_t* tar_valid, float* pos_code, float* pos_tar, int R, const int32_t* rows,
         int32_t* compact_row, int32_t* iota, float* loss_sum = nullptr, int32_t* n_tok = nullptr,
         int Nc = 0, const int32_t* code_rows = nullptr, int Cc = 0, int32_t* code_slot = nullptr,
         const int32_t* mem_rows = nullptr, int Mc = 0, int32_t* mem_slot = nullptr,
         const int32_t* dec_off = nullptr, int32_t* row_bt = nullptr, int32_t* rows_c = nullptr,
         const int32_t* mem_dst = nullptr, int32_t* mem_off = nullptr, int32_t* mem_valid_c = nullptr);
struct AdamRowsView;
int embed_rows_fwd(hipStream_t s, int R, int T, const int32_t* row_bt, const int32_t* idx, const float* table,
                   const float* pos, float* out, const AdamRowsView* vw = nullptr);
int embed_rows_bwd(hipStream_t s, int R, const int32_t* row_bt, const int32_t* idx, float* dtable, const float* dout,
                   int padding_idx);
int node_features(hipStream_t s, int Nc, const int32_t* node_rows, int N, int L, int S, const int32_t* sou,
                  const int32_t* sub, const int32_t* ast, const float* emb, const float* ast_emb, const float* pos_code,
                  float* X, const int32_t* slot2 = nullptr, float* X2 = nullptr,
                  const AdamRowsView* vw = nullptr);
int rows_move(hipStream_t s, int mode, int R, int W, float* out, const float* in, const int32_t* src, const int32_t* dst);
int rows_move_ld(hipStream_t s, int mode, int R, int W, float* out, int ld_out, const float* in, int ld_in,
                 const int32_t* src, const int32_t* dst);
int rows_gather_idx(hipStream_t s, int R, float* compact, const float* src, const int32_t* rows);
int rows_scatter_add_idx(hipStream_t s, int R, const float* compact, float* dst, const int32_t* rows);
int fill_pos_tables(hipStream_t s, int L, float* pos_code, int T, float* pos_tar);
int tar_mask(hipStream_t s, int n, const int32_t* tar, int32_t* valid);
int permute_cache(hipStream_t s, int nl, int BR, int T, int len, const int32_t* parent, const float* ksrc,
                  const float* vsrc, float* kdst, float* vdst, const int32_t* hist_src, int32_t* hist_dst);
int mark_history(hipStream_t s, int BR, int T, int step, const int32_t* tokens, int32_t* hist);
int decode_embed(hipStream_t s, int BR, int T, int step, const int32_t* tokens, const float* table, const float* pos_row,
                 float* x, int32_t* hist);

int attention_fwd(hipStream_t s, int B, int H, int Tq, int Tk, const float* Q, int ldq, const float* K, int ldk,
                  const float* V, int ldv, const int32_t* key_valid, int causal, int q_pos0, float* O, int ldo,
                  const int32_t* q_off = nullptr, int self_kv = 0,
                  int bf16 = 0,
                  const int32_t* k_off = nullptr);
int attention_fwd_ex(hipStream_t s, int B, int H, int Tq, int Tk, const float* Q, int ldq, const float* K, int ldk,
                     const float* V, int ldv, const int32_t* key_valid, int causal, int q_pos0, float* O, int ldo,
                     int kb, int kvb, int qpk, const int32_t* q_off = nullptr, int self_kv = 0, int bf16 = 0,
                     const int32_t* k_off = nullptr);
int decode_attention(hipStream_t s, int BR, int H, int Tk, const float* Q, int ldq, const float* K, int ldk,
                     const float* V, int ldv, const int32_t* key_valid, float* O, int ldo, int kb, int kvb, int qpk,
                     const float* Knew = nullptr, const float* Vnew = nullptr, int ldn = 0, float* Kc_out = nullptr,
                     float* Vc_out = nullptr, const int32_t* k_off = nullptr);
int decode_self_block(hipStream_t s, int BR, int Tk, int T, const float* qkv, float* Kc, float* Vc, const int32_t* hist,
                      const float* WoT, const float* bo, const float* xres, const float* gamma, const float* beta,
                      const float* WqT, const float* bq, float* xa, float* qc);
int decode_attention_kv16(hipStream_t s, int BR, int H, int Tk, const float* Q, int ldq, const uint16_t* K, int ldk,
                          const uint16_t* V, int ldv, const int32_t* key_valid, float* O, int ldo, int kb, int kvb, int qpk,
                          const int32_t* k_off = nullptr);
int rows_to_bf16(hipStream_t s, int64_t n, const float* in, uint16_t* out);
int rows_from_bf16(hipStream_t s, int64_t n, const uint16_t* in, float* out);
int attention_bwd(hipStream_t s, int B, int H, int Tq, int Tk, const float* Q, int ldq, const float* K, int ldk,
                  const float* V, int ldv, const int32_t* key_valid, int causal, int q_pos0, const float* O, int ldo,
                  const float* dO, int lddo, float* dQ, int lddq, float* dK, int lddk, float* dV, int lddv,
                  const int32_t* q_off = nullptr, int self_kv = 0, int bf16 = 0, const int32_t* k_off = nullptr);
int copy_score_fwd(hipStream_t s, int B, int T, int S, const float* src, const float* tgt, const float* w,
                   const float* bias, float* score);
int copy_score_fwd_ex(hipStream_t s, int B, int T, int S, const float* src, const float* tgt, const float* w,
                      const float* bias, float* score, int qpk, const int32_t* mem_valid,
                      const int32_t* tar_label = nullptr, int V = 0,
                      const int32_t* t_off = nullptr);
int copy_score_bwd_ex(hipStream_t s, int B, int T, int S, const float* src, const float* tgt, const float* w,
                      const float* dscore, float* dsrc, float* dtgt, float* dw, float* dbias, const int32_t* mem_valid,
                      float* part = nullptr, const int32_t* t_off = nullptr);
int copy_score_bwd_blocks(int B, int S);
constexpr int COPY_PART_STRIDE = 264;
int decode_dist(hipStream_t s, int R, int V, int S, const float* logits, int ldl, const float* score,
                const int32_t* mem_valid, int qpk, const float* gate_logits, float* dist, int32_t* best_id,
                float* best_p, const float* x = nullptr, const float* wp = nullptr, const float* bp = nullptr);
int inv_count(hipStream_t s, const int32_t* n_tok, float* out);
int sample_dist(hipStream_t s, int R, int n_sample, int V, int S, const float* logits, int ldl, const float* score,
                const int32_t* mem_valid, const float* x, const float* wp, const float* bp, int T, int step,
                const int32_t* key, const uint64_t* seed_dev, float temperature, int top_k, float top_p, float* dist,
                int32_t* best_id, float* best_p);
int score_dist(hipStream_t s, int R, int n_cand, int V, int L, int S, const float* logits, int ldl, const float* score,
               const int32_t* mem_valid, const float* x, const float* wp, const float* bp, const int32_t* target,
               const int32_t* label, const int32_t* sou, const int32_t* sub, float* dist, float* p_word, float* p_entry,
               int32_t* entry, float* copy_share, float* p_label, int32_t* top_id, float* logp_word, float* logp_entry,
               float* logp_label);
int row_topk(hipStream_t s, int R, int V, int k, const float* logits, int ldl, int32_t* ids, float* vals);
int copy_score_bwd(hipStream_t s, int B, int T, int S, const float* src, const float* tgt, const float* w,
                   const float* dscore, float* dsrc, float* dtgt, float* dw, float* dbias);
int head_loss(hipStream_t s, int BT, int T, int V, int S, const int32_t* compact_row, float* logits, int ldl,
              float* score, const int32_t* mem_valid, float* gate_logits, const int32_t* tar_label, float* loss_sum,
              int32_t* n_tok, int32_t* argmax_out, int want_grad,
              const int32_t* row_bt = nullptr);
int adam_step(hipStream_t s, int64_t n, float* p, const float* g, float* m, float* v, float lr, float beta1,
              float beta2, float eps, int step, const float* scale_ptr, int scale_is_count = 0);
int adam_step_mb(hipStream_t s, int64_t n, float* p, const float* g0, const float* g1, float* m, float* v, float lr,
                 float beta1, float beta2, float eps, int step, const int32_t* n0, const int32_t* n1);
constexpr int ADAM_ROWS_K = 32;
struct AdamRowsHist { float bc1[ADAM_ROWS_K], bc2s[ADAM_ROWS_K], lr[ADAM_ROWS_K]; };
struct AdamLr {
    float lr = 0.f;
    bool scheduled = false;
    fira_lr_schedule sched{};
    float at(int step) const { return scheduled ? fira_lr_at(&sched, step) : lr; }
};
inline AdamLr adam_lr(const fira_adam_opts& ad) {
    AdamLr r;
    r.lr = ad.lr;
    if (ad.sched) { r.scheduled = true; r.sched = *ad.sched; }
    return r;
}
struct AdamRowsTables { float *p, *m, *v; int64_t off[2]; int rows[2]; int32_t* last; };
struct AdamRowsView {
    const float *m = nullptr, *v = nullptr;
    const int32_t* last = nullptr;
    int to = 0;
    float beta1 = 0.f, beta2 = 0.f, eps = 0.f, gz = 0.f;
    AdamRowsHist h;
};
AdamRowsView adam_rows_view(const AdamRowsTables& tb, int table, const AdamLr& lr, float beta1, float beta2, float eps, int to);
struct AdamRowsLists { int n_lists; int end[4]; int table[4]; const int32_t* ids[4]; };
int adam_rows_step(hipStream_t s, const AdamRowsTables& tb, const float* g, const AdamLr& lr, float beta1, float beta2, float eps,
                   int step, const int32_t* n0, const float* count, int tables = 3);
int adam_rows_catchup(hipStream_t s, const AdamRowsTables& tb, const AdamRowsLists* ls, const AdamLr& lr, float beta1, float beta2,
                      float eps, int to);
AdamRowsHist adam_rows_hist(const AdamLr& lr, float beta1, float beta2, int end);
struct ClipClose {
    const int32_t* n_tok;
    const float* count;
    float max_norm;
    int n_slots;
};
size_t grad_sqsum_scratch_bytes();
int grad_sqsum(hipStream_t s, int64_t n, const float* g, fira_clip_state* st, int slot, void* scratch, const ClipClose* fin);
int clip_finish(hipStream_t s, fira_clip_state* st, const ClipClose& fin);
int adam_step_clip(hipStream_t s, int64_t n, float* p, const float* g, float* m, float* v, float lr, float beta1, float beta2,
                   float eps, int step, const int32_t* n0, const float* count, const fira_clip_state* st);
int adam_rows_step_clip(hipStream_t s, const AdamRowsTables& tb, const float* g, const AdamLr& lr, float beta1, float beta2, float eps,
                        int step, const int32_t* n0, const float* count, int tables, const fira_clip_state* st);

struct ParamInfo {
    std::string name;
    int64_t offset = -1, numel = 0;
    int ndim = 0;
    int64_t shape[2] = {0, 0};
};

struct EncLayer {
    int64_t wqk, bqk, w2, b2, wo, bo, ln1g, ln1b, fc1w, fc1b, fc2w, fc2b, ln2g, ln2b;
};
struct DecLayer {
    int64_t wqkv, bqkv, wo_s, bo_s, lns_g, lns_b, wq_c, bq_c, wkv_c, bkv_c, wo_c, bo_c, lnc_g, lnc_b, w1, b1, w2, b2,
        lnf_g, lnf_b;
};
struct Layout {
    fira_dims d;
    std::vector<ParamInfo> infos;
    int64_t total = 0;
    int64_t split = 0, live = 0;
    int64_t emb, ast_emb, mark_emb, w2_all, b2_all, dec_emb, wkv_all, bkv_all, wout, bout, ws, wt, wres, bres, wp, bp;
    std::vector<EncLayer> enc;
    std::vector<DecLayer> dec;
};
const Layout* get_layout(const fira_dims* d);

}
```

### fira_icse_amd/csrc/engine.hip

```cpp
#include "engine.h"
#include <hip/hip_ext.h>
#include "epilogue.h"
#include <stdlib.h>
#include <map>
#include <mutex>

namespace fira {

static int64_t shadow_wbt_elems(const Layout& L);

struct Arena {
    char* base;
    size_t used = 0;
    explicit Arena(void* b) : base((char*)b) {}
    template <typename T>
    T* get(size_t n) {
        size_t bytes = (n * sizeof(T) + 255) / 256 * 256;
        T* p = base ? (T*)(base + used) : nullptr;
        used += bytes;
        return p;
    }
    float* f(size_t n) { return get<float>(n); }
};

struct EncSave {
    float *Xc, *qk, *c, *s1, *st1, *Z, *s2, *st2;
};
struct DecSave {
    float *qkv, *ao, *s_a, *st_a, *x_a, *qc, *ao2, *s_c, *st_c, *x_c, *h, *s_f, *st_f, *x_f;
};

struct EncGrad {
    float *dY2, *dYc, *dqk;
};
struct DecGrad {
    float *dYf, *dh, *dYc, *dq, *dYs, *dqkv;
};


static constexpr int KV_ROW_PAD = 64;

struct Plan {
    int B, NB, CB, MB, TB, N, L, S, A, T, V, ldl, nl, F;
    int kvp;
    float *pos_code, *pos_tar;
    int32_t *mem_valid, *tar_valid, *compact_row, *iota, *code_slot, *mem_slot, *row_bt, *rows_c;
    int32_t *mem_off, *mem_valid_c;
    std::vector<float*> X;
    std::vector<EncSave> enc;
    std::vector<DecSave> dec;
    std::vector<EncGrad> encg;
    std::vector<DecGrad> decg;
    float *vtab_all, *H, *mem, *mem_c, *src_c, *x0, *kv_all, *src, *tgt, *score, *gate, *dec_c, *logits;
    float *W21, *c21, *rsum;
    float *W21t;
    uint16_t *W21x = nullptr, *W21tx = nullptr;
    uint16_t *WcX = nullptr, *WcTX = nullptr;
    uint16_t* WkvX = nullptr;
    float* WkvT = nullptr;
    uint16_t* WkvTX = nullptr;
    uint16_t* WoutTX = nullptr;
    uint16_t *xh_planes = nullptr;
    float *WcT;
    float *dW21, *dc21;
    float *inv_ntok;
    float *dXa, *dXb, *dNB2, *dCB_a, *dvtab_all;
    float *zero_beg = nullptr, *zero_end = nullptr;
    uint16_t *wb = nullptr, *wbt = nullptr;
    uint16_t *w21b = nullptr, *w21bt = nullptr;
    float* red_buf = nullptr;
    size_t red_cap = 0;
    float* panel_scratch = nullptr;
    size_t panel_floats = 0;
    float *dmem_c, *dsrc, *dsrc_c, *dtgt, *dkv_all, *ddec, *ddec_c, *dT_a, *dT_c;

    size_t build(void* ws, const fira_dims& d, int B_, bool training) {
        Arena a(ws);
        B = B_; L = d.sou_len; S = d.sub_len; A = d.ast_len; T = d.tar_len; V = d.vocab; nl = d.n_layer; F = d.d_ff;
        N = L + S + A;
        NB = B * N; CB = B * L; MB = B * (L + S); TB = B * T;
        ldl = (V + 63) / 64 * 64;
        const size_t D = FIRA_D;
        pos_code = a.f((size_t)L * D);
        pos_tar = a.f((size_t)T * D);
        mem_valid = a.get<int32_t>((size_t)MB);
        tar_valid = a.get<int32_t>((size_t)TB);
        compact_row = a.get<int32_t>((size_t)TB);
        iota = a.get<int32_t>((size_t)TB);
        row_bt = a.get<int32_t>((size_t)TB);
        rows_c = a.get<int32_t>((size_t)TB);
        code_slot = a.get<int32_t>((size_t)NB);
        mem_slot = a.get<int32_t>((size_t)NB);
        mem_off = a.get<int32_t>((size_t)B + 1);
        mem_valid_c = a.get<int32_t>((size_t)MB);
        inv_ntok = a.f(64);
        {
            const Layout* lay = get_layout(&d);
            const size_t tot = lay ? (size_t)lay->total : 0;
            wb = a.get<uint16_t>(tot);
            wbt = a.get<uint16_t>((lay ? (size_t)shadow_wbt_elems(*lay) : 0) + 64);
            w21b = a.get<uint16_t>((size_t)nl * D * D);
            w21bt = a.get<uint16_t>((size_t)nl * D * D + 64);
        }
        X.resize(nl + 1);
        for (int l = 0; l <= nl; ++l) X[l] = a.f((size_t)NB * D);
        enc.resize(nl);
        for (int l = 0; l < nl; ++l) {
            EncSave& e = enc[l];
            e.Xc = a.f((size_t)CB * D); e.qk = a.f((size_t)CB * 2 * D); e.c = a.f((size_t)CB * D);
            e.s1 = a.f((size_t)CB * D); e.st1 = a.f((size_t)CB * 2);
            e.Z = a.f((size_t)NB * D); e.s2 = a.f((size_t)NB * D); e.st2 = a.f((size_t)NB * 2);
        }
        vtab_all = a.f((size_t)4 * nl * D);
        W21 = a.f((size_t)nl * D * D); c21 = a.f((size_t)nl * D); rsum = a.f((size_t)NB);
        W21t = a.f((size_t)nl * D * D);
        W21x = a.get<uint16_t>((size_t)nl * 3 * D * D);
        W21tx = a.get<uint16_t>((size_t)nl * 3 * D * D);
        WcX = a.get<uint16_t>((size_t)nl * 9 * D * D);
        WcTX = a.get<uint16_t>((size_t)nl * 9 * D * D);
        WkvX = a.get<uint16_t>((size_t)nl * 6 * D * D);
        WkvT = a.f((size_t)nl * 2 * D * D);
        WkvTX = a.get<uint16_t>((size_t)nl * 6 * D * D);
        WoutTX = a.get<uint16_t>((size_t)cdiv(V, D) * 3 * D * D);
        xh_planes = a.get<uint16_t>(head_logits_x3_scratch_elems(TB));
        WcT = a.f((size_t)nl * 3 * D * D);
        H = a.f((size_t)NB * D);
        mem = a.f((size_t)MB * D);
        mem_c = a.f((size_t)MB * D);
        src_c = a.f((size_t)MB * D);
        x0 = a.f((size_t)TB * D);
        kvp = nl * 2 * D + KV_ROW_PAD;
        kv_all = a.f((size_t)MB * kvp);
        dec.resize(nl);
        for (int l = 0; l < nl; ++l) {
            DecSave& e = dec[l];
            e.qkv = a.f((size_t)TB * 3 * D); e.ao = a.f((size_t)TB * D); e.s_a = a.f((size_t)TB * D);
            e.st_a = a.f((size_t)TB * 2); e.x_a = a.f((size_t)TB * D); e.qc = a.f((size_t)TB * D);
            e.ao2 = a.f((size_t)TB * D); e.s_c = a.f((size_t)TB * D); e.st_c = a.f((size_t)TB * 2);
            e.x_c = a.f((size_t)TB * D); e.h = a.f((size_t)TB * F); e.s_f = a.f((size_t)TB * D);
            e.st_f = a.f((size_t)TB * 2); e.x_f = a.f((size_t)TB * D);
        }
        src = a.f((size_t)MB * D); tgt = a.f((size_t)TB * D);
        score = a.f((size_t)TB * (L + S)); gate = a.f((size_t)TB * 2);
        dec_c = a.f((size_t)TB * D); logits = a.f((size_t)TB * ldl);
        if (training) {
            dXa = a.f((size_t)NB * D); dXb = a.f((size_t)NB * D); dNB2 = a.f((size_t)NB * D);
            dCB_a = a.f((size_t)CB * D);
            red_cap = (size_t)nl * ((size_t)cdiv(NB, 16) * 4 * D + (size_t)cdiv(CB, 16) * 2 * D)
                    + (size_t)3 * nl * cdiv(TB, 16) * 2 * D
                    + (size_t)nl * std::max((size_t)cdiv(CB, 16) * 4 * D, (size_t)comb_fused_bwd_parts() * 6 * D + 64)
                    + (size_t)cdiv(L + S, 16) * B * COPY_PART_STRIDE + 4096;
            red_buf = a.f(red_cap);
            panel_floats = (size_t)320 * 256 * 256;
            panel_scratch = a.f(panel_floats);
            zero_beg = (float*)a.get<char>(0);
            dvtab_all = a.f((size_t)4 * nl * D);
            dW21 = a.f((size_t)nl * D * D + (size_t)nl * D); dc21 = dW21 + (size_t)nl * D * D;
            dtgt = a.f((size_t)TB * D);
            ddec_c = a.f((size_t)TB * D);
            zero_end = (float*)a.get<char>(0);
            dmem_c = a.f((size_t)MB * D); dsrc = a.f((size_t)MB * D); dsrc_c = a.f((size_t)MB * D);
            dkv_all = a.f((size_t)MB * kvp);
            ddec = a.f((size_t)TB * D);
            dT_a = a.f((size_t)TB * D); dT_c = a.f((size_t)TB * D);
            encg.resize(nl);
            decg.resize(nl);
            for (int l = 0; l < nl; ++l) {
                EncGrad& g = encg[l];
                g.dY2 = a.f((size_t)NB * D); g.dYc = a.f((size_t)CB * D);
                g.dqk = a.f((size_t)CB * 2 * D);
                DecGrad& h = decg[l];
                h.dYf = a.f((size_t)TB * D); h.dh = a.f((size_t)TB * F); h.dYc = a.f((size_t)TB * D);
                h.dq = a.f((size_t)TB * D); h.dYs = a.f((size_t)TB * D); h.dqkv = a.f((size_t)TB * 3 * D);
            }
        }
        return a.used;
    }
};

#define TRY(x)                 \
    do {                       \
        if (int e__ = (x)) return e__; \
    } while (0)

static int zero(hipStream_t s, void* p, size_t bytes) {
    hipError_t e = hipMemsetAsync(p, 0, bytes, s);
    if (e != hipSuccess) return set_err("hipMemsetAsync: %s", hipGetErrorString(e));
    return 0;
}

static thread_local int g_dtype = 0;
static thread_local int g_lanes = 1;
struct DtypeScope {
    int prev;
    explicit DtypeScope(int d) : prev(g_dtype) { g_dtype = d; }
    ~DtypeScope() { g_dtype = prev; }
};
static thread_local const float* g_P = nullptr;
static thread_local int64_t g_total = 0;
static thread_local const uint16_t* g_Wb = nullptr;
static thread_local const uint16_t* g_WbT = nullptr;
static thread_local const ShadowTable* g_tab = nullptr;
static thread_local const float* g_W21 = nullptr;
static thread_local int64_t g_W21n = 0;
static thread_local const uint16_t* g_W21b = nullptr;
static thread_local const uint16_t* g_W21bT = nullptr;

static const ShadowTable* shadow_table(const Layout& L) {
    static std::mutex mu;
    static std::map<const Layout*, ShadowTable*> cache;
    std::lock_guard<std::mutex> g(mu);
    auto it = cache.find(&L);
    if (it != cache.end()) return it->second;
    ShadowTable* t = new ShadowTable();
    const int D = FIRA_D;
    auto add = [&](int64_t off, int rows, int cols) {
        if (t->n == SHADOW_MAX) return;
        const int pitch = (rows + 7) / 8 * 8;
        t->e[t->n] = ShadowEntry{off, rows, cols, pitch, t->wbt_elems};
        t->wbt_elems += ((int64_t)cols * pitch + 63) / 64 * 64;
        t->tile_start[t->n + 1] = t->tile_start[t->n] + cdiv(rows, 64) * cdiv(cols, 64);
        ++t->n;
    };
    for (int l = 0; l < L.d.n_layer; ++l) {
        add(L.enc[l].wqk, 2 * D, D);
        add(L.enc[l].wo, D, D);
        add(L.dec[l].wqkv, 3 * D, D);
        add(L.dec[l].wo_s, D, D);
        add(L.dec[l].wq_c, D, D);
        add(L.dec[l].wo_c, D, D);
        add(L.dec[l].w1, L.d.d_ff, D);
        add(L.dec[l].w2, D, L.d.d_ff);
    }
    add(L.wkv_all, L.d.n_layer * 2 * D, D);
    add(L.wout, L.d.vocab, D);
    add(L.ws, D, D);
    add(L.wt, D, D);
    cache[&L] = t;
    return t;
}
static int64_t shadow_wbt_elems(const Layout& L) { return shadow_table(L)->wbt_elems; }
struct ShadowScope {
    ShadowScope(const float* P, int64_t total, const uint16_t* wb, const uint16_t* wbt, const ShadowTable* tab) {
        g_P = P; g_total = total; g_Wb = wb; g_WbT = wbt; g_tab = tab;
    }
    ~ShadowScope() {
        g_P = nullptr; g_total = 0; g_Wb = nullptr; g_WbT = nullptr; g_tab = nullptr;
        g_W21 = nullptr; g_W21n = 0; g_W21b = nullptr; g_W21bT = nullptr;
    }
};
static bool shadow_of(const float* W, bool transposed, const uint16_t** out, int* ld) {
    if (!g_Wb || !g_tab) return false;
    if (g_W21b && W >= g_W21 && W < g_W21 + g_W21n) {
        const int64_t off = W - g_W21;
        if (off % (FIRA_D * FIRA_D)) return false;
        *out = (transposed ? g_W21bT : g_W21b) + off;
        *ld = FIRA_D;
        return true;
    }
    if (W < g_P || W >= g_P + g_total) return false;
    const int64_t off = W - g_P;
    for (int i = 0; i < g_tab->n; ++i) {
        const ShadowEntry& e = g_tab->e[i];
        if (off < e.offset || off >= e.offset + (int64_t)e.rows * e.cols) continue;
        const int64_t rel = off - e.offset;
        if (rel % e.cols) return false;
        if (!transposed) { *out = g_Wb + off; *ld = e.cols; }
        else { *out = g_WbT + e.offset_t + rel / e.cols; *ld = e.pitch_t; }
        return true;
    }
    return false;
}
static inline int gemm_any(hipStream_t s, int tA, int tB, int M, int N, int K, const float* A, int lda, const float* B,
                           int ldb, float* C, int ldc, const float* bias, int flags, int splitk, float* colsum,
                           const int32_t* c_rows = nullptr, const float* relu_mask = nullptr) {
    if (g_dtype == 1) {
        const uint16_t* wb;
        int ldw;
        if (!tA && !colsum && gemm_bf16_takes(M, N, K) && lda % 4 == 0 && shadow_of(B, !tB, &wb, &ldw) &&
            (tB ? ldb == K : ldb == N) && ldw % 8 == 0 && ((uintptr_t)wb % 16) == 0)
            return gemm_bf16_wb_ex(s, M, N, K, A, lda, wb, ldw, C, ldc, bias, flags, splitk, c_rows, relu_mask);
        return gemm_bf16_ex(s, tA, tB, M, N, K, A, lda, B, ldb, C, ldc, bias, flags, splitk, colsum, c_rows, relu_mask);
    }
    return gemm_f32_ex(s, tA, tB, M, N, K, A, lda, B, ldb, C, ldc, bias, flags, splitk, colsum, c_rows, relu_mask);
}

static inline int linear(hipStream_t s, int M, int N, int K, const float* X, int ldx, const float* W, const float* b,
                         float* Y, int ldy, int flags = 0) {
    return gemm_any(s, 0, 1, M, N, K, X, ldx, W, K, Y, ldy, b, flags, 0, nullptr);
}
static inline int linear_ln(hipStream_t s, int M, int K, const float* X, int ldx, const float* W, const float* b,
                            const float* res, const float* gamma, const float* beta, float* sum, float* y, float* stats,
                            float p_drop, uint64_t seed, uint32_t st, const int32_t* y_rows = nullptr,
                            const float* r1_row = nullptr, const float* r1_col = nullptr,
                            const int32_t* slot2 = nullptr, float* y2 = nullptr, int n2 = 0, const int32_t* rows2 = nullptr,
                            uint32_t idx0 = 0) {
    bool fused = false;
    int rc = 0;
    if (g_dtype != 0 && idx0 == 0 && g_lanes == 1) {
        const uint16_t* wb;
        int ldw;
        fused = shadow_of(W, false, &wb, &ldw) && ldw == K &&
                linear_ln_bf16_try(s, M, K, X, ldx, wb, ldw, b, res, gamma, beta, sum, y, stats, p_drop, seed, st, y_rows, r1_row,
                                   r1_col, &rc);
    }
    if (fused) {
        TRY(rc);
        if (y2 && n2 > 0) TRY(rows_move(s, 0, n2, FIRA_D, y2, y, rows2, nullptr));
        return 0;
    }
    TRY(linear(s, M, FIRA_D, K, X, ldx, W, b, sum, FIRA_D));
    return add_layernorm_fwd(s, M, sum, res, gamma, beta, y, stats, p_drop, seed, st, y_rows, r1_row, r1_col, slot2, y2, idx0);
}
static inline bool linear_presum(hipStream_t s, int M, int K, const float* X, int ldx, const float* W, const float* b,
                                 const float* res, float* sum, float p_drop, uint64_t seed, uint32_t st, int* rc,
                                 uint32_t idx0 = 0) {
    if (g_dtype != 0 || !gemm_tile32_takes(1, M, FIRA_D, K, X, ldx, W, K)) return false;
    EpiRes er;
    er.res = res; er.ldr = FIRA_D; er.p = p_drop; er.inv_keep = p_drop > 0.f ? 1.0f / (1.0f - p_drop) : 1.0f;
    er.seed = seed; er.site = st; er.idx0 = idx0;
    ProfScope prof(s, PROF_GEMM, 2.0 * M * FIRA_D * (double)K, 4.0 * ((double)M * K + (double)FIRA_D * K + 2.0 * M * FIRA_D));
    return gemm_tile32_try(s, 1, M, FIRA_D, K, X, ldx, W, K, sum, FIRA_D, b, 0, rc, nullptr, nullptr, nullptr, &er);
}
static inline int linear_dgrad(hipStream_t s, int M, int N, int K, const float* dY, int lddy, const float* W, float* dX,
                               int lddx, bool accum) {
    return gemm_any(s, 0, 0, M, K, N, dY, lddy, W, K, dX, lddx, nullptr, accum ? FIRA_GEMM_ACCUM : 0, 0, nullptr);
// ... 471 lines not shown
    if (c.row_step)
        vw_emb = adam_rows_view(adam_rows_tables(L, nullptr, c.rows_ad, c.row_step), 1, c.rows_lr, c.rows_ad.beta1, c.rows_ad.beta2,
                                c.rows_ad.eps, c.rows_ad.step - 1);
    TRY(node_features(s, Nc, bt.node_rows, p.N, p.L, p.S, bt.sou, bt.sub_token, bt.ast_change, c.P + L.emb, c.P + L.ast_emb,
                      p.pos_code, p.X[0], p.code_slot, p.enc[0].Xc, &vw_emb));
    TRY(linear(s, 4, p.nl * D, D, c.P + L.mark_emb, D, c.P + L.w2_all, c.P + L.b2_all, p.vtab_all, p.nl * D));
    for (int l = 0; l < p.nl; ++l) {
        const EncLayer& w = L.enc[l];
        EncSave& e = p.enc[l];
        float* X = p.X[l];
        if (l < 8) {
            if (l == 0 && ev_comb) TRY(main_wait(s, ev_comb, __LINE__));
            else if (l == 0 && ev_fold0) { TRY(main_wait(s, ev_fold0, __LINE__)); fold_waited = true; }
            const float* wt = p.WcT + (size_t)l * 3 * D * D;
            TRY(comb_fused_fwd(s, Cc, e.Xc, wt, wt + (size_t)D * D, wt + (size_t)2 * D * D, c.P + w.bqk, c.P + w.bo,
                               p.vtab_all + l * D, p.nl * D, bt.code_mark, e.qk, e.c, c.P + w.ln1g, c.P + w.ln1b, e.s1, X,
                               bt.code_rows, e.st1, c.p_drop, c.seed, site(l, SITE_GATE), site(l, SITE_COMB_OUT), g_dtype == 1,
                               comb_x3_on(p.nl) ? p.WcX + (size_t)l * 9 * D * D : nullptr));
        } else {
        TRY(linear(s, Cc, 2 * D, D, e.Xc, D, c.P + w.wqk, c.P + w.bqk, e.qk, 2 * D));
        TRY(combination_fwd(s, Cc, e.qk, p.vtab_all + l * D, p.nl * D, bt.code_mark, e.c, c.p_drop, c.seed, site(l, SITE_GATE)));
        TRY(linear_ln(s, Cc, D, e.c, D, c.P + w.wo, c.P + w.bo, e.Xc, c.P + w.ln1g, c.P + w.ln1b, e.s1, X, e.st1, c.p_drop,
                      c.seed, site(l, SITE_COMB_OUT), bt.code_rows));
        }
        const bool fused = gcn_fused_on();
        if (!fused) TRY(csr_spmm_ex(s, Nc, bt.rowptr, bt.col, bt.val, X, D, e.Z, D, 0, 1, 0, l == 0 ? p.rsum : nullptr));
        if (l == 0 && ev_fold0 && !fold_waited) TRY(main_wait(s, ev_fold0, __LINE__));
        if (l == 1 && ev_fold && ev_fold != ev_fold0) TRY(main_wait(s, ev_fold, __LINE__));
        const bool last = l + 1 == p.nl;
        if (fused)
            TRY(gcn_fused_fwd(s, Nc, bt.rowptr, bt.col, bt.val, X, p.W21t + (size_t)l * D * D, c.P + w.fc2b, p.c21 + (size_t)l * D,
                              c.P + w.ln2g, c.P + w.ln2b, e.s2, p.X[l + 1], e.st2, l == 0 ? p.rsum : nullptr,
                              last ? p.mem_slot : p.code_slot, last ? p.mem_c : p.enc[l + 1].Xc, c.p_gcn, c.seed,
                              site(l, SITE_GCN), g_dtype == 1, gcn_x3_on(p.nl) ? p.W21x + (size_t)l * 3 * D * D : nullptr));
        else
        TRY(linear_ln(s, Nc, D, e.Z, D, p.W21 + (size_t)l * D * D, c.P + w.fc2b, X, c.P + w.ln2g, c.P + w.ln2b, e.s2,
                      p.X[l + 1], e.st2, c.p_gcn, c.seed, site(l, SITE_GCN), nullptr, p.rsum, p.c21 + (size_t)l * D,
                      last ? p.mem_slot : p.code_slot, last ? p.mem_c : p.enc[l + 1].Xc, last ? Mc : Cc,
                      last ? bt.mem_rows : bt.code_rows));
    }
    c.deferred = false;
    if (defer_memory_proj && side_on() && p.nl <= 16) {
        TRY(aux_fork(s));
        hipStream_t ss = side().aux;
        const bool kvx = c.G && kv_x3_on(p.nl);
        if (kvx) {
            const float* src[24];
            uint16_t* dst[24];
            for (int j = 0; j < p.nl * 2; ++j) { src[j] = c.P + L.wkv_all + (size_t)j * D * D; dst[j] = p.WkvX + (size_t)j * 3 * D * D; }
            TRY(gcn_split_planes(ss, p.nl * 2, src, dst));
        }
        for (int l = 0; l < p.nl; ++l) {
            const size_t o = (size_t)l * 2 * D;
            if (kvx) {
                const int l1 = l == 0 ? std::min(2, p.nl) : p.nl;
                if (l == 0 || l == std::min(2, p.nl))
                    TRY(linear_x3(ss, Mc, p.mem_c, D, p.WkvX + (size_t)l * 2 * 3 * D * D, (l1 - l) * 2, c.P + L.bkv_all + o, p.kv_all + o,
                                  p.kvp, g_dtype == 1));
            } else
            TRY(gemm_any(ss, 0, 1, Mc, 2 * D, D, p.mem_c, D, c.P + L.wkv_all + o * D, D, p.kv_all + o, p.kvp, c.P + L.bkv_all + o, 0,
                         0, nullptr));
            if (l == std::min(1, p.nl - 1) || l == p.nl - 1) TRY(side_mark(&c.ev_kv[l]));
        }
        TRY(gemm_any(ss, 0, 1, Mc, D, D, p.mem_c, D, c.P + L.ws, D, p.src, D, nullptr, 0, 0, nullptr, bt.mem_dst));
        TRY(side_mark(&c.ev_src));
        if (kvx && p.nl * 2 <= 24) {
            TransposeTable tt;
            const float* src[24];
            uint16_t* dst[24];
            for (int j = 0; j < p.nl * 2; ++j) {
                tt.src[tt.n] = c.P + L.wkv_all + (size_t)j * D * D; tt.dst[tt.n++] = p.WkvT + (size_t)j * D * D;
                src[j] = p.WkvT + (size_t)j * D * D; dst[j] = p.WkvTX + (size_t)j * 3 * D * D;
            }
            TRY(transpose256_table(ss, tt));
            TRY(gcn_split_planes(ss, p.nl * 2, src, dst));
            c.kv_planes = true;
        }
        if (c.G && g_dtype == 1) {
            TRY(split_planes_t(ss, c.P + L.wout, p.V, p.WoutTX, true));
            c.wout_planes = true;
        }
        c.deferred = true;
        return 0;
    }
    TRY(gemm_any(s, 0, 1, Mc, KV, D, p.mem_c, D, c.P + L.wkv_all, D, p.kv_all, p.kvp, c.P + L.bkv_all, 0, 0, nullptr));
    TRY(gemm_any(s, 0, 1, Mc, D, D, p.mem_c, D, c.P + L.ws, D, p.src, D, nullptr, 0, 0, nullptr, bt.mem_dst));
    return 0;
}

static int decoder_forward(Ctx& c) {
    Plan& p = *c.pl;
    const Layout& L = *c.L;
    const int D = FIRA_D, H = L.d.n_head, Sm = p.L + p.S;
    if (c.row_bt) {
        AdamRowsView vw;
        if (c.row_step)
            vw = adam_rows_view(adam_rows_tables(L, nullptr, c.rows_ad, c.row_step), 0, c.rows_lr, c.rows_ad.beta1, c.rows_ad.beta2,
                                c.rows_ad.eps, c.rows_ad.step - 1);
        TRY(embed_rows_fwd(c.s, c.Td, p.T, c.row_bt, c.bt->tar, c.P + L.dec_emb, p.pos_tar, p.x0, &vw));
    } else {
        if (c.row_step) TRY(adam_rows_prefetch(c, c.s));
        TRY(embed_gather_fwd(c.s, p.B, p.T, c.bt->tar, c.P + L.dec_emb, p.pos_tar, p.x0, p.T, 0));
    }
    ProfDecoderTag prof_tag;
    TRY(decoder_lanes(c));
    ProfScope prof_region(c.s, PROF_DEC_REGION, 0.0);
    TRY(lanes_fork(c));
    struct LaneState {
        const float *x = nullptr, *pend_sum = nullptr, *pend_g = nullptr, *pend_b = nullptr;
        float *pend_y = nullptr, *pend_st = nullptr;
        int kv_waited = 0;
    } state[2];
    for (int k = 0; k < c.n_lanes; ++k) state[k].x = p.x0;
    for (int l = 0; l < p.nl; ++l) {
        const DecLayer& w = L.dec[l];
        DecSave& e = p.dec[l];
        const bool last = l + 1 == p.nl;
        for (int k = 0; k < c.n_lanes; ++k) {
            const Lane& ln = c.lanes[k];
            LaneState& st = state[k];
            hipStream_t s = ln.s;
            const size_t r0 = (size_t)ln.r0;
            const int nr = ln.nr;
            const uint32_t idx0 = (uint32_t)(r0 * D);
            auto consume = [&](int N, const float* W, const float* b, float* Y, int flags) -> int {
                if (st.pend_sum) {
                    int rc = 0;
                    float* sum = const_cast<float*>(st.pend_sum) + r0 * D;
                    const bool fused = gemm_tile32_ln_try(s, nr, N, sum, D, W, b, Y + r0 * N, N, flags, st.pend_g, st.pend_b,
                                                          st.pend_y + r0 * D, st.pend_st + r0 * 2, &rc);
                    if (!fused)
                        rc = add_layernorm_fwd(s, nr, sum, nullptr, st.pend_g, st.pend_b, st.pend_y + r0 * D, st.pend_st + r0 * 2, 0.f, 0, 0,
                                               nullptr);
                    st.pend_sum = nullptr;
                    if (rc || fused) return rc;
                }
                return linear(s, nr, N, D, st.x + r0 * D, D, W, b, Y + r0 * N, N, flags);
            };
            auto close_block = [&](int K, const float* X, const float* W, const float* b, const float* res, const float* g,
                                   const float* be, float* sum, float* y, float* stt, uint32_t site_id, bool may_defer,
                                   const int32_t* slot2, float* y2, int n2, const int32_t* rows2) -> int {
                int rc = 0;
                if (may_defer && linear_presum(s, nr, K, X + r0 * K, K, W, b, res + r0 * D, sum + r0 * D, c.p_drop, c.seed, site_id,
                                               &rc, idx0)) {
                    st.pend_sum = sum; st.pend_g = g; st.pend_b = be; st.pend_y = y; st.pend_st = stt;
                    return rc;
                }
                return linear_ln(s, nr, K, X + r0 * K, K, W, b, res + r0 * D, g, be, sum + r0 * D, y + r0 * D, stt + r0 * 2, c.p_drop,
                                 c.seed, site_id, nullptr, nullptr, nullptr, slot2 ? slot2 + r0 : nullptr, y2, n2, rows2, idx0);
            };
            const int32_t* q_off = c.dec_off ? c.dec_off + ln.b0 : nullptr;
            TRY(consume(3 * D, c.P + w.wqkv, c.P + w.bqkv, e.qkv, 0));
            TRY(attention_fwd(s, ln.nb, H, p.T, p.T, e.qkv, 3 * D, e.qkv + D, 3 * D, e.qkv + 2 * D, 3 * D, p.tar_valid + (size_t)ln.b0 * p.T,
                              1, 0, e.ao, D, q_off, 1, attn_bf16()));
            TRY(close_block(D, e.ao, c.P + w.wo_s, c.P + w.bo_s, st.x, c.P + w.lns_g, c.P + w.lns_b, e.s_a, e.x_a, e.st_a,
                            site(l, SITE_SELF), true, nullptr, nullptr, 0, nullptr));
            st.x = e.x_a;
            TRY(consume(D, c.P + w.wq_c, c.P + w.bq_c, e.qc, 0));
            if (c.deferred) {
                int m = l;
                while (m < p.nl - 1 && c.ev_kv[m] == nullptr) ++m;
                if (c.ev_kv[m] != nullptr && st.kv_waited < m + 1) {
                    TRY(main_wait(s, c.ev_kv[m], __LINE__));
                    st.kv_waited = m + 1;
                }
            }
            TRY(attention_fwd(s, ln.nb, H, p.T, Sm, e.qc, D, p.kv_all + l * 2 * D, p.kvp, p.kv_all + l * 2 * D + D, p.kvp,
                              c.kv_ragged ? p.mem_valid_c : p.mem_valid, 0, 0, e.ao2, D, q_off, 0, attn_bf16(),
                              c.kv_ragged ? p.mem_off + ln.b0 : nullptr));
            TRY(close_block(D, e.ao2, c.P + w.wo_c, c.P + w.bo_c, e.x_a, c.P + w.lnc_g, c.P + w.lnc_b, e.s_c, e.x_c, e.st_c,
                            site(l, SITE_CROSS), true, nullptr, nullptr, 0, nullptr));
            st.x = e.x_c;
            TRY(consume(p.F, c.P + w.w1, c.P + w.b1, e.h, FIRA_GEMM_RELU));
            const bool head_copy = last && c.rows != nullptr && c.R > 0;
            TRY(close_block(p.F, e.h, c.P + w.w2, c.P + w.b2, e.x_c, c.P + w.lnf_g, c.P + w.lnf_b, e.s_f, e.x_f, e.st_f,
                            site(l, SITE_FFN), !last, head_copy ? p.compact_row : nullptr, head_copy ? p.dec_c : nullptr,
                            head_copy ? c.R : 0, head_copy ? c.rows : nullptr));
            st.x = e.x_f;
        }
    }
    TRY(lanes_join(c));
    return 0;
}

static int head_forward(Ctx& c, int R, const int32_t* rows, float* loss_sum, int32_t* n_tok, int32_t* argmax_out,
                        int want_grad) {
    Plan& p = *c.pl;
    const Layout& L = *c.L;
    hipStream_t s = c.s;
    const int D = FIRA_D, Sm = p.L + p.S;
    const float* dec = p.dec[p.nl - 1].x_f;
    const float* dec_rows = (c.rows != nullptr && rows == c.rows) ? p.dec_c : dec;
    if (dec_rows == dec && R != c.Td) {
        TRY(rows_gather_idx(s, R, p.dec_c, dec, rows));
        dec_rows = p.dec_c;
    }
    if (g_dtype == 0 && R >= 64 && R <= p.TB)
        TRY(head_logits_x3(s, R, p.V, dec_rows, D, c.P + L.wout, c.P + L.bout, p.logits, p.ldl, p.xh_planes));
    else
    TRY(linear(s, R, p.V, D, dec_rows, D, c.P + L.wout, c.P + L.bout, p.logits, p.ldl));
    TRY(gemm_any(s, 0, 1, c.Td, D, D, dec, D, c.P + L.wt, D, p.tgt, D, nullptr, 0, 0, nullptr));
    if (c.deferred) TRY(main_wait(s, c.ev_src, __LINE__));
    TRY(copy_score_fwd_ex(s, p.B, p.T, Sm, p.src, p.tgt, c.P + L.wres, c.P + L.bres, p.score, 1, p.mem_valid,
                          argmax_out ? nullptr : c.bt->tar_label, p.V, c.dec_off));
    TRY(linear(s, c.Td, 2, D, dec, D, c.P + L.wp, c.P + L.bp, p.gate, 2));
    TRY(head_loss(s, c.Td, p.T, p.V, Sm, p.compact_row, p.logits, p.ldl, p.score, p.mem_valid, p.gate,
                  c.bt->tar_label, loss_sum, n_tok, argmax_out, want_grad, c.row_bt));
    return 0;
}

static inline int enc_wgrad_every(int n_rows, int n_layers) {
    static const int forced = [] { const char* e = getenv("FIRA_ENC_WGRAD_EVERY"); const int v = e ? atoi(e) : 0; return v >= 1 ? v : 0; }();
    if (forced) return forced;
    return n_rows <= 32768 ? std::max(1, n_layers) : 1;
}

static int group_a_final_stream(hipStream_t s, hipStream_t* out) {
    SideStream& sd = side();
    *out = s;
    if (sd.stream && sd.enabled) {
        TRY(aux_fork(s));
        hipEvent_t e2 = sd.ev();
        if (hipEventRecord(e2, sd.stream) != hipSuccess || hipStreamWaitEvent(sd.aux, e2, 0) != hipSuccess)
            return set_err("group-A mark: weight-gradient stream mark failed");
        *out = sd.aux;
    }
    return 0;
}

struct BwdMid {
    hipEvent_t ev_dmem = nullptr;
    hipEvent_t ev_groupA = nullptr;
};

static int backward_decoder(Ctx& c, int R, const int32_t* rows, hipEvent_t mid_event, BwdMid& mid) {
    Plan& p = *c.pl;
    const Layout& L = *c.L;
    hipStream_t s = c.s;
    const int D = FIRA_D, H = L.d.n_head, KV = p.nl * 2 * D, Sm = p.L + p.S;
    const fira_batch& bt = *c.bt;
    const int Nc = bt.n_nodes, Cc = bt.n_code, Mc = bt.n_mem;
    const float* dec = p.dec[p.nl - 1].x_f;
    float* G = c.G;

    gemm_group_reset();
    gemm_bf16_group_reset();
    gemm_wgrad_panel_reset();
    gemm_wgrad_panel_scratch(p.panel_scratch, p.panel_floats);
    red().reset(p.red_buf, p.red_cap);
    const bool so = side_on();
    hipStream_t ss = so ? side().aux : s;
    hipEvent_t ev_dfc = nullptr;
    if (c.ev_zero) TRY(main_wait(s, c.ev_zero, __LINE__));
    else TRY(zero(s, p.zero_beg, (size_t)((char*)p.zero_end - (char*)p.zero_beg)));
    if (R > 0) {
        if (so) TRY(aux_fork(s));
        if (c.wout_planes) TRY(dgrad_x3_splitk(ss, R, p.V, p.logits, p.ldl, p.WoutTX, p.ddec_c, D, g_dtype == 1));
        else
        TRY(gemm_any(ss, 0, 0, R, D, p.V, p.logits, p.ldl, c.P + L.wout, D, p.ddec_c, D, nullptr, FIRA_GEMM_ACCUM, 0,
                        nullptr));
        if (so) TRY(side_mark(&ev_dfc));
    }
    if (R > 0)
        TRY(linear_wgrad(s, R, p.V, D, p.logits, p.ldl, (c.rows != nullptr && rows == c.rows) ? p.dec_c : dec, D, G + L.wout,
                         G + L.bout, PANEL_VOCAB));
    if (g_dtype == 0) TRY(rank2_rows(s, c.Td, p.gate, c.P + L.wp, p.ddec));
    else TRY(linear_dgrad(s, c.Td, 2, D, p.gate, 2, c.P + L.wp, p.ddec, D, false));
    TRY(linear_wgrad_grouped(s, c.Td, 2, D, p.gate, 2, dec, D, G + L.wp, G + L.bp));
    {
        const int nb = copy_score_bwd_blocks(p.B, Sm);
        float* part = red().alloc((size_t)nb * COPY_PART_STRIDE);
        TRY(copy_score_bwd_ex(s, p.B, p.T, Sm, p.src, p.tgt, c.P + L.wres, p.score, p.dsrc, p.dtgt, G + L.wres, G + L.bres,
                              p.mem_valid, part, c.dec_off));
        if (part) {
            red().add(G + L.wres, part, D, nb, COPY_PART_STRIDE);
            red().add(G + L.bres, part + D, 1, nb, COPY_PART_STRIDE);
        }
    }
    TRY(linear_dgrad(s, c.Td, D, D, p.dtgt, D, c.P + L.wt, p.ddec, D, true));
    TRY(linear_wgrad_grouped(s, c.Td, D, D, p.dtgt, D, dec, D, G + L.wt, nullptr));
    TRY(rows_move(s, 0, Mc, D, p.dsrc_c, p.dsrc, bt.mem_dst, nullptr));
    if (so) TRY(aux_fork(s));
    TRY(linear_dgrad(ss, Mc, D, D, p.dsrc_c, D, c.P + L.ws, p.dmem_c, D, false));
    TRY(linear_wgrad_grouped(s, Mc, D, D, p.dsrc_c, D, p.mem_c, D, G + L.ws, nullptr, 8));
    if (R > 0) {
        if (ev_dfc) TRY(main_wait(s, ev_dfc, __LINE__));
        TRY(rows_scatter_add_idx(s, R, p.ddec_c, p.ddec, rows));
    }

    float *bx = p.ddec, *by = p.dT_a, *bz = p.dT_c;
    constexpr int DEC_WGRAD_EVERY = 3;
    const int dec_every = p.nl % DEC_WGRAD_EVERY != 0 ? 0 : DEC_WGRAD_EVERY;
    {
    ProfScope prof_region(s, PROF_DEC_REGION, 0.0);
    TRY(lanes_fork(c));
    auto aux_fork_all = [&]() -> int { return c.n_lanes > 1 ? lanes_fork_to(c, side().aux) : aux_fork(s); };
    auto flush_wgrads_all = [&]() -> int {
        if (c.n_lanes == 1) return flush_grouped_wgrads(s);
        SideStream& sd = side();
        if (!(sd.stream && sd.enabled)) return 0;
        TRY(lanes_fork_to(c, sd.stream));
        return flush_wgrad_queues(sd.stream);
    };
    for (int l = p.nl - 1; l >= 0; --l) {
        ProfDecoderTag prof_tag;
        const DecLayer& w = L.dec[l];
        DecSave& e = p.dec[l];
        DecGrad& g = p.decg[l];
        const float* x_in = l == 0 ? p.x0 : p.dec[l - 1].x_f;
        hipEvent_t ev_kv_done[2] = {nullptr, nullptr};
        auto dmem_pair = [&]() -> int {
            if (!(so && (l % 2 == 0 || l == 0))) return 0;
            const int nlay = std::min(2, p.nl - l);
            const size_t o = (size_t)l * 2 * D;
            if (c.n_lanes > 1 && ev_kv_done[0] && ev_kv_done[1]) {
                for (int k = 0; k < c.n_lanes; ++k)
                    if (hipStreamWaitEvent(ss, ev_kv_done[k], 0) != hipSuccess) return set_err("lane -> auxiliary stream fork failed");
            } else
            TRY(aux_fork_all());
            prof_decoder_tag(-1);
            const int rc_kv = c.kv_planes
                    ? linear_x3_kacc(ss, Mc, p.dkv_all + o, p.kvp, p.WkvTX + (size_t)l * 2 * 3 * D * D, nlay * 2, p.dmem_c, D, true, g_dtype == 1)
                    : linear_dgrad(ss, Mc, nlay * 2 * D, D, p.dkv_all + o, p.kvp, c.P + L.wkv_all + o * D, p.dmem_c, D, true);
            prof_decoder_tag(+1);
            return rc_kv;
        };
        for (int k = 0; k < c.n_lanes; ++k) {
            const Lane& ln = c.lanes[k];
            hipStream_t ls = ln.s;
            const size_t r0 = (size_t)ln.r0;
            const int nr = ln.nr;
            const uint32_t idx0 = (uint32_t)(r0 * D);
            const int32_t* q_off = c.dec_off ? c.dec_off + ln.b0 : nullptr;
            const bool q = k == 0;
            TRY(ln_bwd_dgrad(ls, nr, p.F, bx + r0 * D, e.s_f + r0 * D, e.st_f + r0 * 2, c.P + w.lnf_g, by + r0 * D, g.dYf + r0 * D,
                             G + w.lnf_g, G + w.lnf_b, c.p_drop, c.seed, site(l, SITE_FFN), c.P + w.w2, p.F, g.dh + r0 * p.F, p.F,
                             e.h + r0 * p.F, idx0));
            if (q) TRY(linear_wgrad_grouped(s, c.Td, D, p.F, g.dYf, D, e.h, p.F, G + w.w2, G + w.b2));
            if (q) TRY(linear_wgrad_grouped(s, c.Td, p.F, D, g.dh, p.F, e.x_c, D, G + w.w1, G + w.b1));
            TRY(linear_dgrad(ls, nr, p.F, D, g.dh + r0 * p.F, p.F, c.P + w.w1, by + r0 * D, D, true));
            TRY(ln_bwd_dgrad(ls, nr, D, by + r0 * D, e.s_c + r0 * D, e.st_c + r0 * 2, c.P + w.lnc_g, bz + r0 * D, g.dYc + r0 * D,
                             G + w.lnc_g, G + w.lnc_b, c.p_drop, c.seed, site(l, SITE_CROSS), c.P + w.wo_c, D, bx + r0 * D, D, nullptr,
                             idx0));
            if (q) TRY(linear_wgrad_grouped(s, c.Td, D, D, g.dYc, D, e.ao2, D, G + w.wo_c, G + w.bo_c));
            TRY(attention_bwd(ls, ln.nb, H, p.T, Sm, e.qc, D, p.kv_all + l * 2 * D, p.kvp, p.kv_all + l * 2 * D + D, p.kvp,
                              p.mem_valid_c, 0, 0, e.ao2, D, bx, D, g.dq, D, p.dkv_all + l * 2 * D, p.kvp,
                              p.dkv_all + l * 2 * D + D, p.kvp, q_off, 0, attn_bf16(), p.mem_off + ln.b0));
            if (c.n_lanes == 1) TRY(dmem_pair());
            else if (so && l % 2 == 0 && k < 2) {
                ev_kv_done[k] = side().ev();
                if (hipEventRecord(ev_kv_done[k], ls) != hipSuccess) return set_err("lane event record failed");
            }
            if (q) TRY(linear_wgrad_grouped(s, c.Td, D, D, g.dq, D, e.x_a, D, G + w.wq_c, G + w.bq_c));
            TRY(linear_dgrad(ls, nr, D, D, g.dq + r0 * D, D, c.P + w.wq_c, bz + r0 * D, D, true));
            TRY(ln_bwd_dgrad(ls, nr, D, bz + r0 * D, e.s_a + r0 * D, e.st_a + r0 * 2, c.P + w.lns_g, by + r0 * D, g.dYs + r0 * D,
                             G + w.lns_g, G + w.lns_b, c.p_drop, c.seed, site(l, SITE_SELF), c.P + w.wo_s, D, bx + r0 * D, D, nullptr,
                             idx0));
            if (q) TRY(linear_wgrad_grouped(s, c.Td, D, D, g.dYs, D, e.ao, D, G + w.wo_s, G + w.bo_s));
            TRY(attention_bwd(ls, ln.nb, H, p.T, p.T, e.qkv, 3 * D, e.qkv + D, 3 * D, e.qkv + 2 * D, 3 * D,
                              p.tar_valid + (size_t)ln.b0 * p.T, 1, 0, e.ao, D, bx, D, g.dqkv, 3 * D, g.dqkv + D, 3 * D, g.dqkv + 2 * D,
                              3 * D, q_off, 1, attn_bf16()));
            if (q) TRY(linear_wgrad_grouped(s, c.Td, 3 * D, D, g.dqkv, 3 * D, x_in, D, G + w.wqkv, G + w.bqkv));
            TRY(linear_dgrad(ls, nr, 3 * D, D, g.dqkv + r0 * 3 * D, 3 * D, c.P + w.wqkv, by + r0 * D, D, true));
        }
        if (c.n_lanes > 1) TRY(dmem_pair());
        if (dec_every > 0 && l % dec_every == 0 && side().stream && side().enabled) {
            const int nlay = std::min(dec_every, p.nl - l);
            const size_t o = (size_t)l * 2 * D;
            prof_decoder_tag(-1);
            int rc_w = flush_wgrads_all();
            if (!rc_w)
                rc_w = wgrad_on(side().stream, PANEL_KV, Mc, nlay * 2 * D, D, p.dkv_all + o, p.kvp, p.mem_c, D, G + L.wkv_all + o * D,
                                G + L.bkv_all + o);
            prof_decoder_tag(+1);
            TRY(rc_w);
        }
        float* t = bx; bx = by; by = t;
    }
    TRY(lanes_join(c));
    }
    const float* dy = bx;
    TRY(flush_grouped_wgrads(s));
    {
        hipStream_t es = (side().stream && side().enabled) ? side().stream : s;
        if (c.row_bt) TRY(embed_rows_bwd(es, c.Td, c.row_bt, c.bt->tar, G + L.dec_emb, dy, 0));
        else TRY(embed_gather_bwd(es, p.B, p.T, c.bt->tar, G + L.dec_emb, dy, p.T, 0, 0));
    }
    hipEvent_t& ev_dmem = mid.ev_dmem;
    if (so) {
        TRY(side_mark(&ev_dmem));
    } else {
        TRY(linear_dgrad(s, Mc, KV, D, p.dkv_all, p.kvp, c.P + L.wkv_all, p.dmem_c, D, true));
    }
    if (!(side().stream && side().enabled))
        TRY(linear_wgrad(s, Mc, KV, D, p.dkv_all, p.kvp, p.mem_c, D, G + L.wkv_all, G + L.bkv_all, PANEL_KV));
    else if (dec_every == 0)
        TRY(wgrad_on(side().stream, PANEL_KV, Mc, KV, D, p.dkv_all, p.kvp, p.mem_c, D, G + L.wkv_all, G + L.bkv_all));
    TRY(deferred_reduce(side().stream && side().enabled ? side().stream : s, red().tab));
    hipEvent_t& ev_groupA = mid.ev_groupA;
    if (c.adam && side().stream && side().enabled) {
        ev_groupA = side().ev();
        if (hipEventRecord(ev_groupA, side().stream) != hipSuccess) return set_err("group-A mark failed");
    }
    if (mid_event || c.clip) {
        hipStream_t es = nullptr;
        TRY(group_a_final_stream(s, &es));
        if (mid_event) {
            hipError_t e = hipEventRecord(mid_event, es);
            if (e != hipSuccess) return set_err("hipEventRecord: %s", hipGetErrorString(e));
        }
        if (c.clip) TRY(grad_sqsum(es, L.split, G, c.clip->state, 0, c.clip->scratch, nullptr));
    }
    return 0;
}

static int backward_encoder(Ctx& c, BwdMid& mid) {
    Plan& p = *c.pl;
    const Layout& L = *c.L;
    hipStream_t s = c.s;
    const int D = FIRA_D;
    const fira_batch& bt = *c.bt;
    const int Nc = bt.n_nodes, Cc = bt.n_code, Mc = bt.n_mem;
    float* G = c.G;
    hipEvent_t ev_dmem = mid.ev_dmem, ev_groupA = mid.ev_groupA;
    float* dXn = p.dXa;
    float* other = p.dXb;
    UnfoldTable unfold_tab;
    static const bool unfold_late_off = [] { const char* e = getenv("FIRA_UNFOLD_LATE"); return e && e[0] == '0'; }();
    const bool unfold_late = !unfold_late_off && enc_group_on() && p.nl <= 16;
    const int wgrad_every = unfold_late ? enc_wgrad_every(Nc, p.nl) : 1;
    const float *uf_dW21[16], *uf_W1[16], *uf_W2[16];
    float *uf_dW1[16], *uf_dW2[16];
    int uf_n = 0;
    if (!c.ev_zero) TRY(zero(s, dXn, (size_t)Nc * D * sizeof(float)));
    if (ev_dmem) TRY(main_wait(s, ev_dmem, __LINE__));
    TRY(rows_move(s, 1, Mc, D, dXn, p.dmem_c, nullptr, bt.mem_rows));
    for (int l = p.nl - 1; l >= 0; --l) {
        const EncLayer& w = L.enc[l];
        EncSave& e = p.enc[l];
        EncGrad& g = p.encg[l];
        float* dc21 = p.dc21 + (size_t)l * D;
        bool sums = false;
        const bool room = unfold_tab.n < 16;
        TRY(ln_bwd(s, Nc, dXn, e.s2, e.st2, c.P + w.ln2g, other, g.dY2, G + w.ln2g, G + w.ln2b, c.p_gcn,
                              c.seed, site(l, SITE_GCN), nullptr, room ? p.rsum : nullptr, G + w.fc2b, dc21, &sums));
        if (sums) unfold_tab.e[unfold_tab.n++] = UnfoldEntry{c.P + w.fc2w, c.P + w.fc1b, dc21, G + w.fc2w, G + w.fc1b};
        float* dW21 = p.dW21 + (size_t)l * D * D;
        const bool grouped = enc_group_on();
        bool flushed = false;
        auto unfold = [&]() -> int {
            hipStream_t ws = s;
            if (side().stream && side().enabled) {
                if (!grouped || (!flushed && (!sums || !unfold_late))) TRY(side_fork(s));
                ws = side().stream;
            }
            if (!sums) TRY(colsum(ws, Nc, D, g.dY2, D, dc21, p.rsum));
            if (unfold_late) {
                uf_dW21[uf_n] = dW21; uf_W1[uf_n] = c.P + w.fc1w; uf_W2[uf_n] = c.P + w.fc2w;
                uf_dW1[uf_n] = G + w.fc1w; uf_dW2[uf_n] = G + w.fc2w;
                ++uf_n;
            } else {
            TRY(gemm_f32_ex(ws, 0, 1, D, D, D, dW21, D, c.P + w.fc1w, D, G + w.fc2w, D, nullptr, FIRA_GEMM_ACCUM, 0, nullptr));
            TRY(gemm_f32_ex(ws, 1, 0, D, D, D, c.P + w.fc2w, D, dW21, D, G + w.fc1w, D, nullptr, FIRA_GEMM_ACCUM, 0, nullptr));
            }
            if (!sums) TRY(gcn_bias_unfold(ws, c.P + w.fc2w, c.P + w.fc1b, dc21, G + w.fc2w, G + w.fc1b));
            return 0;
        };
        if (gcn_fused_on()) {
            TRY(gcn_fused_bwd(s, Nc, bt.rowptr, bt.col, bt.val, g.dY2, p.W21 + (size_t)l * D * D, e.Z, other, g_dtype == 1,
                              gcn_x3_on(p.nl) ? p.W21tx + (size_t)l * 3 * D * D : nullptr));
            TRY(enc_wgrad(s, Nc, D, D, e.Z, D, p.X[l], D, dW21, nullptr));
            if (!sums) TRY(colsum(s, Nc, D, g.dY2, D, G + w.fc2b));
            if (!grouped) TRY(unfold());
        } else {
        TRY(enc_wgrad(s, Nc, D, D, g.dY2, D, e.Z, D, dW21, sums ? nullptr : G + w.fc2b));
        if (!grouped) TRY(unfold());
        TRY(linear_dgrad(s, Nc, D, D, g.dY2, D, p.W21 + (size_t)l * D * D, p.dNB2, D, false));
        TRY(csr_spmm_ex(s, Nc, bt.rowptr, bt.col, bt.val, p.dNB2, D, other, D, 0, 1, 1, nullptr));
        }
        const int nb_comb = comb_fused_bwd_parts();
        float* part_ln = red().alloc((size_t)nb_comb * 6 * D, 6);
        const bool comb_done = part_ln != nullptr;
        if (comb_done) {
            float* part_v = part_ln + (size_t)nb_comb * 2 * D;
            TRY(comb_fused_bwd(s, Cc, other, bt.code_rows, e.s1, e.st1, c.P + w.ln1g, c.P + w.wo, c.P + w.wqk, e.qk,
                               p.vtab_all + l * D, p.nl * D, bt.code_mark, g.dYc, g.dqk, part_ln, part_v, c.p_drop, c.seed,
                               site(l, SITE_GATE), site(l, SITE_COMB_OUT), g_dtype == 1,
                               comb_x3_on(p.nl) ? p.WcTX + (size_t)l * 9 * D * D : nullptr));
            red().add(G + w.ln1g, part_ln, D, nb_comb, 2 * D);
            red().add(G + w.ln1b, part_ln + D, D, nb_comb, 2 * D);
            for (int k = 0; k < 4; ++k)
                red().add(p.dvtab_all + (size_t)k * p.nl * D + l * D, part_v + k * D, D, nb_comb, 4 * D);
            TRY(enc_wgrad(s, Cc, D, D, g.dYc, D, e.c, D, G + w.wo, G + w.bo));
        } else {
        TRY(ln_bwd(s, Cc, other, e.s1, e.st1, c.P + w.ln1g, other, g.dYc, G + w.ln1g, G + w.ln1b, c.p_drop,
                              c.seed, site(l, SITE_COMB_OUT), bt.code_rows));
        TRY(enc_wgrad(s, Cc, D, D, g.dYc, D, e.c, D, G + w.wo, G + w.bo));
        TRY(linear_dgrad(s, Cc, D, D, g.dYc, D, c.P + w.wo, p.dCB_a, D, false));
        {
            const int nb = combination_bwd_blocks(Cc);
            float* part = red().alloc((size_t)nb * 4 * D);
            TRY(combination_bwd(s, Cc, e.qk, p.vtab_all + l * D, p.nl * D, bt.code_mark, p.dCB_a, g.dqk,
                                p.dvtab_all + l * D, p.nl * D, c.p_drop, c.seed, site(l, SITE_GATE), part));
            if (part)
                for (int k = 0; k < 4; ++k)
                    red().add(p.dvtab_all + (size_t)k * p.nl * D + l * D, part + k * D, D, nb, 4 * D);
        }
        }
        TRY(enc_wgrad(s, Cc, 2 * D, D, g.dqk, 2 * D, e.Xc, D, G + w.wqk, G + w.bqk));
        if (grouped) {
            if ((p.nl - l) % wgrad_every == 0 || l == 0) { TRY(flush_grouped_wgrads(s)); flushed = true; }
            TRY(unfold());
        }
        if (!comb_done)
// ... 554 lines not shown
        float* kc = dp.kc[cur] + l * lay;
        float* vc = dp.vc[cur] + l * lay;
        TRY(consume(3 * D, dp.x, params + w.wqkv, params + w.bqkv, dp.qkv, 0));
        if (self_block) {
            TRY(decode_self_block(s, BR, step + 1, T, dp.qkv, kc, vc, dp.hist[cur], dp.wsT + (size_t)(2 * l) * D * D, params + w.bo_s,
                                  dp.x, params + w.lns_g, params + w.lns_b, dp.wsT + (size_t)(2 * l + 1) * D * D, params + w.bq_c, dp.xa,
                                  dp.qc));
        } else {
        TRY(decode_attention(s, BR, H, step + 1, dp.qkv, 3 * D, kc, D, vc, D, dp.hist[cur], dp.ao, D, T, T, 1,
                             dp.qkv + D, dp.qkv + 2 * D, 3 * D, kc, vc));
        TRY(close_block(D, dp.ao, params + w.wo_s, params + w.bo_s, dp.x, params + w.lns_g, params + w.lns_b, dp.xa, true));
        TRY(consume(D, dp.xa, params + w.wq_c, params + w.bq_c, dp.qc, 0));
        }
        if (flags & FIRA_DECODE_KV_BF16)
            TRY(decode_attention_kv16(s, BR, H, Sm, dp.qc, D, dp.kv16 + l * 2 * D, p.kvp, dp.kv16 + l * 2 * D + D, p.kvp, p.mem_valid_c,
                                      dp.ao, D, Sm, Sm, n_beam, p.mem_off));
        else
            TRY(decode_attention(s, BR, H, Sm, dp.qc, D, p.kv_all + l * 2 * D, p.kvp, p.kv_all + l * 2 * D + D, p.kvp, p.mem_valid_c,
                                 dp.ao, D, Sm, Sm, n_beam, nullptr, nullptr, 0, nullptr, nullptr, p.mem_off));
        TRY(close_block(D, dp.ao, params + w.wo_c, params + w.bo_c, dp.xa, params + w.lnc_g, params + w.lnc_b, dp.xc, true));
        TRY(consume(p.F, dp.xc, params + w.w1, params + w.b1, dp.h, FIRA_GEMM_RELU));
        TRY(close_block(p.F, dp.h, params + w.w2, params + w.b2, dp.xc, params + w.lnf_g, params + w.lnf_b, dp.x, true));
    }
    TRY(consume(D, dp.x, params + L.wt, nullptr, dp.tgt, 0));
    TRY(linear(s, BR, p.V, D, dp.x, D, params + L.wout, params + L.bout, dp.logits, p.ldl));
    TRY(copy_score_fwd_ex(s, BR, 1, Sm, p.src, dp.tgt, params + L.wres, params + L.bres, dp.score, n_beam, p.mem_valid));
    return 0;
}
}

extern "C" {
int fira_decode_step_ex(void* stream, const fira_dims* d, const float* params, void* workspace, size_t workspace_bytes,
                        int B, int n_beam, int step, const int32_t* tokens, const int32_t* parent, float* dist,
                        int32_t* best_id, float* best_p, int flags) {
    hipStream_t s = (hipStream_t)stream;
    DecodePlan dp;
    TRY(decode_step_body(s, d, params, workspace, workspace_bytes, B, n_beam, step, tokens, parent, flags, true,
                         "fira_decode_step_ex", dp));
    const Layout& L = *get_layout(d);
    const Plan& p = dp.enc;
    TRY(decode_dist(s, dp.BR, p.V, p.L + p.S, dp.logits, p.ldl, dp.score, p.mem_valid, n_beam, nullptr, dist, best_id, best_p,
                    dp.x, params + L.wp, params + L.bp));
    return 0;
}
int fira_decode_step_sample(void* stream, const fira_dims* d, const float* params, void* workspace, size_t workspace_bytes,
                            int B, int n_sample, int step, const int32_t* tokens, const int32_t* key, const uint64_t* seed_dev,
                            float temperature, int top_k, float top_p, float* dist, int32_t* best_id, float* best_p,
                            int flags) {
    FIRA_REQUIRE(d, "fira_decode_step_sample: bad argument");
    FIRA_REQUIRE(n_sample >= 1 && n_sample <= 8, "fira_decode_step_sample: n_sample %d outside 1..8", n_sample);
    FIRA_REQUIRE(temperature > 0.f && temperature < INFINITY, "fira_decode_step_sample: temperature %g must be finite and > 0",
                 (double)temperature);
    const int W = d->vocab + d->sou_len + d->sub_len;
    FIRA_REQUIRE(top_k >= 0 && top_k <= W, "fira_decode_step_sample: top_k %d outside 0..%d", top_k, W);
    FIRA_REQUIRE(top_p > 0.f && top_p <= 1.f, "fira_decode_step_sample: top_p %g outside (0, 1]", (double)top_p);
    FIRA_REQUIRE(key && seed_dev && best_id && best_p, "fira_decode_step_sample: key, seed_dev, best_id and best_p are required");
    hipStream_t s = (hipStream_t)stream;
    DecodePlan dp;
    TRY(decode_step_body(s, d, params, workspace, workspace_bytes, B, n_sample, step, tokens, nullptr, flags, false,
                         "fira_decode_step_sample", dp));
    const Layout& L = *get_layout(d);
    const Plan& p = dp.enc;
    TRY(sample_dist(s, dp.BR, n_sample, p.V, p.L + p.S, dp.logits, p.ldl, dp.score, p.mem_valid, dp.x, params + L.wp,
                    params + L.bp, p.T, step, key, seed_dev, temperature, top_k, top_p, dist, best_id, best_p));
    return 0;
}
int fira_decode_step_score(void* stream, const fira_dims* d, const float* params, void* workspace, size_t workspace_bytes,
                           int B, int n_cand, int step, const int32_t* tokens, const int32_t* target, const int32_t* label,
                           const int32_t* sou, const int32_t* sub_token, float* dist, float* p_word, float* p_entry,
                           int32_t* entry, float* copy_share, float* p_label, int32_t* top_id, float* logp_word,
                           float* logp_entry, float* logp_label, int flags) {
    FIRA_REQUIRE(d, "fira_decode_step_score: bad argument");
    FIRA_REQUIRE(n_cand >= 1 && n_cand <= 8, "fira_decode_step_score: n_cand %d outside 1..8", n_cand);
    FIRA_REQUIRE(target && sou && sub_token, "fira_decode_step_score: target, sou and sub_token are required");
    FIRA_REQUIRE(p_word && p_entry && entry && copy_share && top_id && logp_word && logp_entry,
                 "fira_decode_step_score: p_word, p_entry, entry, copy_share, top_id, logp_word and logp_entry are required");
    FIRA_REQUIRE((label != nullptr) == (p_label != nullptr) && (label != nullptr) == (logp_label != nullptr),
                 "fira_decode_step_score: label, p_label and logp_label are given together or not at all");
    hipStream_t s = (hipStream_t)stream;
    DecodePlan dp;
    TRY(decode_step_body(s, d, params, workspace, workspace_bytes, B, n_cand, step, tokens, nullptr, flags, false,
                         "fira_decode_step_score", dp));
    const Layout& L = *get_layout(d);
    const Plan& p = dp.enc;
    TRY(score_dist(s, dp.BR, n_cand, p.V, p.L, p.L + p.S, dp.logits, p.ldl, dp.score, p.mem_valid, dp.x, params + L.wp,
                   params + L.bp, target, label, sou, sub_token, dist, p_word, p_entry, entry, copy_share, p_label, top_id,
                   logp_word, logp_entry, logp_label));
    return 0;
}

int fira_decoder_forward(void* stream, const fira_dims* d, const float* params, void* workspace, size_t workspace_bytes,
                         int B, const int32_t* tar, const float* memory, const int32_t* mem_valid, float* out) {
    const Layout* L = get_layout(d);
    if (!L) return 1;
    FIRA_REQUIRE(params && workspace && tar && memory && mem_valid && out && B > 0, "bad argument");
    Plan p;
    const size_t need = p.build(workspace, *d, B, false);
    FIRA_REQUIRE(need <= workspace_bytes, "workspace too small: need %zu bytes, got %zu", need, workspace_bytes);
    hipStream_t s = (hipStream_t)stream;
    const int D = FIRA_D, KV = p.nl * 2 * D;
    fira_batch b{};
    b.B = B;
    b.tar = tar;
    Ctx c{s, L, &b, params, nullptr, &p, 0.f, 0.f, 0};
    c.Td = p.TB;
    TRY(fill_pos_tables(s, p.L, p.pos_code, p.T, p.pos_tar));
    hipError_t e = hipMemcpyAsync(p.mem_valid, mem_valid, (size_t)p.MB * sizeof(int32_t), hipMemcpyDeviceToDevice, s);
    if (e != hipSuccess) return set_err("hipMemcpyAsync: %s", hipGetErrorString(e));
    TRY(tar_mask(s, p.TB, tar, p.tar_valid));
    TRY(linear(s, p.MB, KV, D, memory, D, params + L->wkv_all, params + L->bkv_all, p.kv_all, p.kvp));
    TRY(decoder_forward(c));
    e = hipMemcpyAsync(out, p.dec[p.nl - 1].x_f, (size_t)p.TB * D * sizeof(float), hipMemcpyDeviceToDevice, s);
    if (e != hipSuccess) return set_err("hipMemcpyAsync: %s", hipGetErrorString(e));
    return 0;
}

__global__ void debug_tiny_kernel(float* p) { if (threadIdx.x == 0 && blockIdx.x == 0) p[0] += 1.0f; }
int fira_debug_chain(void* stream, int n, int mode, float* scratch) {
    FIRA_REQUIRE(scratch && n > 0, "fira_debug_chain: bad argument");
    TRY(side().init());
    hipStream_t s = (hipStream_t)stream;
    SideStream& sd = side();
    for (int i = 0; i < n; ++i) {
        if (mode >= 4 && mode <= 6) {
            const bool ev = mode != 6 || (i & 7) == 7;
            hipEvent_t e = ev ? sd.ev() : nullptr;
            hipExtLaunchKernelGGL(debug_tiny_kernel, dim3(240), dim3(256), 0, s, nullptr, e, 0, scratch);
            if (ev && mode != 4) {
                if (hipStreamWaitEvent(sd.stream, e, 0) != hipSuccess) return set_err("stream wait failed");
                hipLaunchKernelGGL(debug_tiny_kernel, dim3(240), dim3(256), 0, sd.stream, scratch + 64);
            }
            continue;
        }
        hipLaunchKernelGGL(debug_tiny_kernel, dim3(240), dim3(256), 0, s, scratch);
        if (mode == 1 || (mode == 3 && (i & 7) == 7)) {
            TRY(side_fork(s));
            hipLaunchKernelGGL(debug_tiny_kernel, dim3(240), dim3(256), 0, sd.stream, scratch + 64);
        } else if (mode == 2) {
            hipEvent_t e = sd.ev();
            if (hipEventRecord(e, s) != hipSuccess) return set_err("event record failed");
        }
    }
    if (mode == 1 || mode == 3 || mode == 5 || mode == 6) TRY(side_join(s, __LINE__));
    FIRA_CHECK_LAUNCH("debug_chain");
    return 0;
}

const float* fira_decode_memory(const fira_dims* d, void* workspace, int B, int n_beam) {
    if (!get_layout(d) || !workspace) return nullptr;
    DecodePlan dp;
    dp.build(workspace, *d, B, n_beam);
    return dp.enc.mem;
}
const int32_t* fira_decode_mem_valid(const fira_dims* d, void* workspace, int B, int n_beam) {
    if (!get_layout(d) || !workspace) return nullptr;
    DecodePlan dp;
    dp.build(workspace, *d, B, n_beam);
    return dp.enc.mem_valid;
}

}
```

### fira_icse_amd/ops.py

```python
from __future__ import annotations

import dataclasses

import torch

from . import _lib
from ._lib import check, cur_stream, ptr


def _f32(t):
    assert t.is_cuda and t.dtype == torch.float32 and t.is_contiguous(), "expected a contiguous fp32 CUDA tensor"
    return t


def _i32(t):
    assert t.is_cuda and t.dtype == torch.int32 and t.is_contiguous(), "expected a contiguous int32 CUDA tensor"
    return t


def gemm(A, B, *, transA=False, transB=True, bias=None, relu=False, out=None, accumulate=False, splitk=1,
         tile=0, dtype="f32"):
    for t in (A, B):
        assert t.is_cuda and t.dtype == torch.float32 and t.dim() == 2 and t.stride(1) == 1
    M, K = (A.shape[1], A.shape[0]) if transA else A.shape
# ... 143 lines not shown
    part = torch.empty(((M + 31) // 32) * 512, dtype=torch.float32, device=dy.device)
    check(_lib.lib().fira_ln_bwd_linear_f32(cur_stream(), M, N, ptr(_f32(dy)), ptr(_f32(Wt)), ptr(dX),
                                            ptr(None if relu_mask is None else _f32(relu_mask)), ptr(_f32(summ)),
                                            ptr(_f32(stats)), ptr(_f32(gamma)), ptr(ds), ptr(dxd), ptr(dg), ptr(db), ptr(part),
                                            dropout, seed, site), "fira_ln_bwd_linear_f32")
    return dX, ds, dxd, dg, db


def dropout_mask(seed, site, n, p, device="cuda"):
    out = torch.empty(n, dtype=torch.float32, device=device)
    check(_lib.lib().fira_dropout_mask(cur_stream(), seed, site, n, p, ptr(out)), "fira_dropout_mask")
    return out


def colsum(X):
    out = torch.zeros(X.shape[1], dtype=torch.float32, device=X.device)
    check(_lib.lib().fira_colsum_f32(cur_stream(), X.shape[0], X.shape[1], ptr(_f32(X)), X.stride(0), ptr(out)),
          "fira_colsum_f32")
    return out


def gcn_weight_planes(B):
    B = _f32(B).contiguous()
    n = B.numel() // (256 * 256)
    planes = torch.empty(n * 3 * 256 * 256, dtype=torch.int16, device=B.device)
    check(_lib.lib().fira_gcn_weight_planes(cur_stream(), n, ptr(B), ptr(planes)), "fira_gcn_weight_planes")
    return planes


def linear_x3(x, W, bias=None, dtype=2, ldo=None):
    x = _f32(x)
    M, N = x.shape[0], W.shape[0]
    planes = gcn_weight_planes(W)
    ldo = N if ldo is None else ldo
    out = torch.zeros((M, ldo), dtype=torch.float32, device=x.device)
    check(_lib.lib().fira_linear_x3(cur_stream(), M, N, ptr(x), x.stride(0), ptr(planes), ptr(None if bias is None else _f32(bias)),
                                    ptr(out), ldo, dtype), "fira_linear_x3")
    return out[:, :N]


def linear_dgrad_x3(dy, W, dx=None, dtype=2):
    assert dy.is_cuda and dy.dtype == torch.float32 and dy.stride(1) == 1
    M, K = dy.shape
    Wt = _f32(W).view(K // 256, 256, 256).transpose(1, 2).contiguous()
    planes = gcn_weight_planes(Wt)
    acc = dx is not None
    if dx is None:
        dx = torch.empty((M, 256), dtype=torch.float32, device=dy.device)
    check(_lib.lib().fira_linear_dgrad_x3(cur_stream(), M, K, ptr(dy), dy.stride(0), ptr(planes), ptr(dx), dx.stride(0), 1 if acc else 0,
                                          dtype), "fira_linear_dgrad_x3")
    return dx


def dgrad_x3_splitk(dy, W, dx, dtype=2):
    assert dy.is_cuda and dy.dtype == torch.float32 and dy.stride(1) == 1
    M, K = dy.shape
    ws = torch.empty(_lib.lib().fira_dgrad_x3_splitk_planes_bytes(K), dtype=torch.uint8, device=dy.device)
    check(_lib.lib().fira_dgrad_x3_splitk(cur_stream(), M, K, ptr(dy), dy.stride(0), ptr(_f32(W)), ptr(ws), ptr(dx), dx.stride(0),
                                          dtype), "fira_dgrad_x3_splitk")
    return dx


def gcn_layer_fwd(rowptr, col, val, X, W21t, bias, c21, gamma, beta, dropout=0.0, seed=0, site=0, dtype=0, want_rowsum=True):
    n = X.shape[0]
    if dtype >= 2:
        W21t = gcn_weight_planes(_f32(W21t).t().contiguous())
    else:
        W21t = _f32(W21t)
    summ, y = torch.empty_like(X), torch.empty_like(X)
    stats = torch.empty((n, 2), dtype=torch.float32, device=X.device)
    rs = torch.empty(n, dtype=torch.float32, device=X.device) if want_rowsum else None
    check(_lib.lib().fira_gcn_layer_fwd(cur_stream(), n, ptr(_i32(rowptr)), ptr(_i32(col)), ptr(_f32(val)), ptr(_f32(X)),
                                        ptr(W21t), ptr(_f32(bias)), ptr(_f32(c21)), ptr(_f32(gamma)), ptr(_f32(beta)),
                                        ptr(summ), ptr(y), ptr(stats), ptr(rs), dropout, seed, site, dtype),
          "fira_gcn_layer_fwd")
    return summ, y, stats, rs


def combination_block_fwd(Xc, Wqk, bqk, Wo, bo, vtab, mark, gamma, beta, dropout=0.0, seed=0, site_gate=0, site_out=0, y=None,
                          y_rows=None, dtype=0):
    n = Xc.shape[0]
    dev = Xc.device
    assert vtab.is_cuda and vtab.dtype == torch.float32 and vtab.stride(1) == 1 and vtab.shape[0] == 4, "vtab: fp32 rows"
    if dtype >= 2:
        WqT = WkT = WoT = gcn_weight_planes(torch.cat([_f32(Wqk), _f32(Wo)], 0))
    else:
        WqT, WkT, WoT = (_f32(Wqk[:256]).t().contiguous(), _f32(Wqk[256:]).t().contiguous(), _f32(Wo).t().contiguous())
    qk = torch.empty((n, 512), dtype=torch.float32, device=dev)
    c, summ = torch.empty_like(Xc), torch.empty_like(Xc)
    if y is None:
        y = torch.empty_like(Xc)
    stats = torch.empty((n, 2), dtype=torch.float32, device=dev)
    yr = None if y_rows is None else _i32(y_rows)
    check(_lib.lib().fira_combination_block_fwd(cur_stream(), n, ptr(_f32(Xc)), ptr(WqT), ptr(WkT), ptr(WoT), ptr(_f32(bqk)),
                                                ptr(_f32(bo)), ptr(vtab), vtab.stride(0), ptr(_i32(mark)), ptr(qk), ptr(c),
                                                ptr(_f32(gamma)), ptr(_f32(beta)), ptr(summ), ptr(y), ptr(yr), ptr(stats),
                                                dropout, seed, site_gate, site_out, dtype), "fira_combination_block_fwd")
    return qk, c, summ, y, stats


def combination_block_bwd(dG, rows, summ, stats, gamma, Wo, Wqk, qk, vtab, mark, dropout=0.0, seed=0, site_gate=0, site_out=0,
                          dtype=0):
    n = summ.shape[0]
    dev = summ.device
    assert vtab.is_cuda and vtab.dtype == torch.float32 and vtab.stride(1) == 1 and vtab.shape[0] == 4, "vtab: fp32 rows"
    dYc = torch.empty((n, 256), dtype=torch.float32, device=dev)
    dqk = torch.empty((n, 512), dtype=torch.float32, device=dev)
    dgamma, dbeta = torch.zeros(256, device=dev), torch.zeros(256, device=dev)
    dvtab = torch.zeros((4, 256), device=dev)
    part = torch.empty(_lib.lib().fira_combination_block_bwd_part_floats(), dtype=torch.float32, device=dev)
    if dtype >= 2:
        Wo = gcn_weight_planes(torch.stack([_f32(Wqk[:256]).t(), _f32(Wqk[256:]).t(), _f32(Wo).t()]).contiguous())
    else:
        Wo = _f32(Wo)
    check(_lib.lib().fira_combination_block_bwd(cur_stream(), n, ptr(_f32(dG)), ptr(_i32(rows)), ptr(_f32(summ)), ptr(_f32(stats)),
                                                ptr(_f32(gamma)), ptr(Wo), ptr(_f32(Wqk)), ptr(_f32(qk)), ptr(vtab),
                                                vtab.stride(0), ptr(_i32(mark)), ptr(dYc), ptr(dqk), ptr(dgamma), ptr(dbeta),
                                                ptr(dvtab), 256, ptr(part), dropout, seed, site_gate, site_out, dtype),
          "fira_combination_block_bwd")
    return dYc, dqk, dgamma, dbeta, dvtab


def gcn_layer_bwd(rowptr, col, val, dY, W21, dX, dtype=0):
    V = torch.empty_like(dY)
    W = gcn_weight_planes(_f32(W21).t().contiguous()) if dtype >= 2 else _f32(W21)
    check(_lib.lib().fira_gcn_layer_bwd(cur_stream(), dY.shape[0], ptr(_i32(rowptr)), ptr(_i32(col)), ptr(_f32(val)),
                                        ptr(_f32(dY)), ptr(W), ptr(V), ptr(_f32(dX)), dtype), "fira_gcn_layer_bwd")
    return V


def attention_ragged_fwd(q, k, v, key_valid, q_off, Tq, Tk, causal=False, self_kv=False, dtype=0, heads=8, k_off=None):
    B = q_off.numel() - 1
    o = torch.zeros_like(q)
    ko = None if k_off is None else _i32(k_off)
    check(_lib.lib().fira_attention_fwd_ex(cur_stream(), B, heads, Tq, Tk, ptr(q), q.stride(0), ptr(k), k.stride(0), ptr(v),
                                           v.stride(0), ptr(_i32(key_valid)), int(causal), 0, ptr(o), 256, ptr(_i32(q_off)),
                                           int(self_kv), dtype, ptr(ko)), "fira_attention_fwd_ex")
    return o


def attention_ragged_bwd(q, k, v, key_valid, o, do, q_off, Tq, Tk, causal=False, self_kv=False, dtype=0, heads=8, k_off=None,
                         fill=0.0):
    B = q_off.numel() - 1
    dq, dk, dv = torch.full_like(q, fill), torch.full_like(k, fill), torch.full_like(v, fill)
    ko = None if k_off is None else _i32(k_off)
    check(_lib.lib().fira_attention_bwd_ex(cur_stream(), B, heads, Tq, Tk, ptr(q), q.stride(0), ptr(k), k.stride(0), ptr(v),
                                           v.stride(0), ptr(_i32(key_valid)), int(causal), 0, ptr(_f32(o)), 256,
                                           ptr(_f32(do)), 256, ptr(dq), dq.stride(0), ptr(dk), dk.stride(0), ptr(dv),
                                           dv.stride(0), ptr(_i32(q_off)), int(self_kv), dtype, ptr(ko)),
          "fira_attention_bwd_ex")
    return dq, dk, dv


def attention_fwd(q, k, v, key_valid, causal=False, q_pos0=0, heads=8):
    B, Tq, _ = q.shape
    Tk = k.shape[1]
    o = torch.empty((B, Tq, 256), dtype=torch.float32, device=q.device)
    check(_lib.lib().fira_attention_fwd(cur_stream(), B, heads, Tq, Tk, ptr(q), q.stride(1), ptr(k), k.stride(1),
                                        ptr(v), v.stride(1), ptr(_i32(key_valid)), int(causal), q_pos0, ptr(o), 256),
          "fira_attention_fwd")
    return o


def decode_attention(q, k, v, key_valid, tk=None, qpk=1, heads=8, knew=None, vnew=None, k_off=None):
    BR = q.shape[0]
    if k_off is not None:
        kb = kvb = tk
        ldk, ldv = k.stride(0), v.stride(0)
    else:
        kb, kvb = k.shape[1], key_valid.shape[1]
        ldk, ldv = k.stride(1), v.stride(1)
    tk = kb if tk is None else tk
    o = torch.empty((BR, 256), dtype=torch.float32, device=q.device)
    ko = None if k_off is None else _i32(k_off)
    check(_lib.lib().fira_decode_attention(cur_stream(), BR, heads, tk, ptr(q), q.stride(0), ptr(k), ldk, ptr(v),
                                           ldv, ptr(_i32(key_valid)), ptr(o), 256, kb, kvb, qpk, ptr(knew),
                                           ptr(vnew), knew.stride(0) if knew is not None else 0,
                                           ptr(k) if knew is not None else None, ptr(v) if knew is not None else None,
                                           ptr(ko)),
          "fira_decode_attention")
    return o


def attention_bwd(q, k, v, key_valid, o, do, causal=False, q_pos0=0, heads=8):
    B, Tq, _ = q.shape
    Tk = k.shape[1]
    dq = torch.empty((B, Tq, 256), dtype=torch.float32, device=q.device)
    dk = torch.empty((B, Tk, 256), dtype=torch.float32, device=q.device)
    dv = torch.empty((B, Tk, 256), dtype=torch.float32, device=q.device)
    check(_lib.lib().fira_attention_bwd(cur_stream(), B, heads, Tq, Tk, ptr(q), q.stride(1), ptr(k), k.stride(1),
                                        ptr(v), v.stride(1), ptr(_i32(key_valid)), int(causal), q_pos0, ptr(_f32(o)),
                                        256, ptr(_f32(do)), 256, ptr(dq), 256, ptr(dk), 256, ptr(dv), 256),
          "fira_attention_bwd")
    return dq, dk, dv


def copy_score_fwd(src, tgt, w, bias):
    B, S, _ = src.shape
    T = tgt.shape[1]
    score = torch.empty((B, T, S), dtype=torch.float32, device=src.device)
    check(_lib.lib().fira_copy_score_fwd(cur_stream(), B, T, S, ptr(_f32(src)), ptr(_f32(tgt)), ptr(_f32(w)),
                                         ptr(_f32(bias)), ptr(score)), "fira_copy_score_fwd")
    return score


def copy_score_bwd(src, tgt, w, dscore):
    B, S, _ = src.shape
    T = tgt.shape[1]
    dsrc = torch.empty_like(src)
    dtgt = torch.zeros_like(tgt)
    dw = torch.zeros(256, dtype=torch.float32, device=src.device)
    db = torch.zeros(1, dtype=torch.float32, device=src.device)
    check(_lib.lib().fira_copy_score_bwd(cur_stream(), B, T, S, ptr(_f32(src)), ptr(_f32(tgt)), ptr(_f32(w)),
                                         ptr(_f32(dscore)), ptr(dsrc), ptr(dtgt), ptr(dw), ptr(db)),
          "fira_copy_score_bwd")
    return dsrc, dtgt, dw, db


def head_loss(logits, score, mem_valid, gate_logits, tar_label, V, compact_row=None, want_grad=True, argmax=False):
    B, T = tar_label.shape
    S = score.shape[-1]
    loss = torch.zeros(1, dtype=torch.float32, device=logits.device)
    ntok = torch.zeros(1, dtype=torch.int32, device=logits.device)
    ids = torch.empty((B, T), dtype=torch.int32, device=logits.device) if argmax else None
    check(_lib.lib().fira_head_loss(cur_stream(), B * T, T, V, S, ptr(compact_row), ptr(_f32(logits)),
                                    logits.stride(0), ptr(_f32(score)), ptr(_i32(mem_valid)), ptr(_f32(gate_logits)),
                                    ptr(_i32(tar_label)), ptr(loss), ptr(ntok), ptr(ids), int(want_grad)),
          "fira_head_loss")
    return loss, ntok, ids


def adam_step(p, g, m, v, lr, step, beta1=0.9, beta2=0.999, eps=1e-8, inv_scale=None):
    check(_lib.lib().fira_adam_step(cur_stream(), p.numel(), ptr(_f32(p)), ptr(_f32(g)), ptr(_f32(m)), ptr(_f32(v)),
                                    lr, beta1, beta2, eps, step, ptr(inv_scale)), "fira_adam_step")


def adam_step_count(p, g, m, v, lr, step, count, beta1=0.9, beta2=0.999, eps=1e-8):
    check(_lib.lib().fira_adam_step_count(cur_stream(), p.numel(), ptr(_f32(p)), ptr(_f32(g)), ptr(_f32(m)), ptr(_f32(v)),
                                          lr, beta1, beta2, eps, step, ptr(_f32(count))), "fira_adam_step_count")


def pack_stats(loss_sum, n_tok, out2):
    check(_lib.lib().fira_pack_stats(cur_stream(), ptr(_f32(loss_sum)), ptr(_i32(n_tok)), ptr(_f32(out2))), "fira_pack_stats")
    return out2


def adam_step_mb(p, g0, g1, m, v, lr, step, n_tok0, n_tok1=None, beta1=0.9, beta2=0.999, eps=1e-8):
    check(_lib.lib().fira_adam_step_mb(cur_stream(), p.numel(), ptr(_f32(p)), ptr(_f32(g0)), ptr(g1), ptr(_f32(m)),
                                       ptr(_f32(v)), lr, beta1, beta2, eps, step, ptr(_i32(n_tok0)), ptr(n_tok1)),
          "fira_adam_step_mb")


LR_KINDS = ("constant", "inv_sqrt", "cosine", "linear")


@dataclasses.dataclass(frozen=True)
class LrSchedule:
    kind: str = "constant"
    base_lr: float = 1e-4
    warmup_steps: int = 0
    decay_steps: int = 0
    min_lr: float = 0.0

    @staticmethod
    def make(obj) -> "LrSchedule":
        if isinstance(obj, LrSchedule):
            s = obj
        else:
            d = dict(obj)
            unknown = set(d) - {f.name for f in dataclasses.fields(LrSchedule)}
            if unknown:
                raise ValueError("lr_schedule: unknown field(s) %s" % sorted(unknown))
            s = LrSchedule(**d)
        kind = s.kind
        if isinstance(kind, int) and not isinstance(kind, bool) and 0 <= kind < len(LR_KINDS):
            kind = LR_KINDS[kind]
        kind = str(kind).replace("-", "_")
        if kind not in LR_KINDS:
            raise ValueError("lr_schedule: kind %r is not one of %s" % (s.kind, ", ".join(LR_KINDS)))
        s = LrSchedule(kind, float(s.base_lr), int(s.warmup_steps), int(s.decay_steps), float(s.min_lr))
        lr_schedule_check(s)
        return s

    def struct(self) -> "_lib.LrSchedule":
        return _lib.LrSchedule(LR_KINDS.index(self.kind), self.base_lr, self.warmup_steps, self.decay_steps, self.min_lr)

    def as_dict(self) -> dict:
        return dataclasses.asdict(self)


def _sched_struct(sched):
    return sched if isinstance(sched, _lib.LrSchedule) else sched.struct()


def lr_at(sched, step: int) -> float:
    import ctypes as C
    return float(_lib.lib().fira_lr_at(C.byref(_sched_struct(sched)), int(step)))


def lr_schedule_check(sched):
    import ctypes as C
    lib = _lib.lib()
    if lib.fira_lr_schedule_check(C.byref(_sched_struct(sched))) != 0:
        raise ValueError(lib.fira_last_error().decode())


# ... 137 lines not shown
```

### include/fira_hip.h

```cpp
#ifndef FIRA_HIP_H
#define FIRA_HIP_H

#include <stddef.h>
#include <stdint.h>

#ifdef __cplusplus
extern "C" {
#endif

#define FIRA_ABI_VERSION 10

typedef struct fira_dims {
    int32_t sou_len;
    int32_t sub_len;
    int32_t ast_len;
    int32_t tar_len;
    int32_t d_model;
    int32_t n_head;
    int32_t n_layer;
    int32_t vocab;
    int32_t ast_vocab;
    int32_t d_ff;
} fira_dims;

// ... 16 lines not shown
    const int32_t* code_mark;
    int32_t n_mem;
    const int32_t* mem_rows;
    const int32_t* mem_dst;
    const int32_t* head_rows;
    int32_t n_head_rows;
    int32_t n_emb_items;
    const int32_t* emb_item_tok;
    const int32_t* emb_item_ptr;
    const int32_t* emb_rows;
    int32_t n_ast_items;
    const int32_t* ast_rows;
    const int32_t* ast_ids;
    const int32_t* dec_off;
    int32_t n_dec_rows;
    const int32_t* dec_off_host;
} fira_batch;

typedef struct fira_train_opts {
    float    dropout;
    float    gcn_dropout;
    uint64_t seed;
    int32_t  compact_head;
    int32_t  dtype;
    int32_t  compact_dec;
    int32_t  zero_grads;
} fira_train_opts;
#define FIRA_F32 0
#define FIRA_BF16 1
#define FIRA_F32X3 2
#define FIRA_BF16X1 3

const char* fira_last_error(void);
int         fira_abi_version(void);

int    fira_param_count(const fira_dims* d);
int    fira_param_info(const fira_dims* d, int index, char* name_buf, int64_t* offset, int64_t* numel,
                       int32_t* ndim, int64_t shape[2]);
int64_t fira_param_total(const fira_dims* d);
int    fira_param_groups(const fira_dims* d, int64_t* split, int64_t* live);

size_t fira_workspace_bytes(const fira_dims* d, int B, int mode);
size_t fira_decode_workspace_bytes(const fira_dims* d, int B, int n_beam);
size_t fira_decode_workspace_bytes_ex(const fira_dims* d, int B, int n_beam, int flags);

#define FIRA_PROF_NCLASS 7
void fira_prof_enable(int on);
int  fira_prof_report(int n_class, double* ms, double* work, double* bytes, int64_t* count);


#define FIRA_GEMM_RELU 1
#define FIRA_GEMM_ACCUM 2
#define FIRA_GEMM_TILE_SHIFT 4
int fira_gemm_f32(void* stream, int transA, int transB, int M, int N, int K,
                  const float* A, int lda, const float* B, int ldb, float* C, int ldc,
                  const float* bias, int flags, int splitk);
int fira_gemm_bf16(void* stream, int transA, int transB, int M, int N, int K,
                   const float* A, int lda, const float* B, int ldb, float* C, int ldc,
                   const float* bias, int flags, int splitk);

int fira_weight_shadow(void* stream, int rows, int cols, const float* W, uint16_t* Wb, uint16_t* WbT);
int fira_gemm_bf16_wb(void* stream, int M, int N, int K, const float* A, int lda, const uint16_t* Bb, int ldb,
                      float* C, int ldc, const float* bias, int flags, int splitk);

int fira_csr_spmm_f32(void* stream, int n_rows, const int32_t* rowptr, const int32_t* col, const float* val,
                      const float* X, int ldx, float* Y, int ldy, int graph_rows, int variant);
int fira_csr_spmm(void* stream, int n_rows, int64_t nnz, const int32_t* rowptr, const int32_t* col, const float* val,
                  const float* X, int ldx, float* Y, int ldy, int graph_rows, int variant, int dtype);

int fira_gcn_layer_fwd(void* stream, int n_rows, const int32_t* rowptr, const int32_t* col, const float* val,
                       const float* X, const float* W21t, const float* bias, const float* c21, const float* gamma,
                       const float* beta, float* sum, float* y, float* stats, float* rowsum_out, float dropout,
                       uint64_t seed, uint32_t site, int dtype);
int fira_gcn_layer_bwd(void* stream, int n_rows, const int32_t* rowptr, const int32_t* col, const float* val,
                       const float* dY, const float* W21, float* V, float* dX, int dtype);
int fira_gcn_weight_planes(void* stream, int n_mats, const float* B, uint16_t* planes);
int fira_linear_x3(void* stream, int M, int N, const float* x, int ldx, const uint16_t* w_planes, const float* bias, float* out,
                   int ldo, int dtype);
int fira_linear_dgrad_x3(void* stream, int M, int K, const float* dy, int lddy, const uint16_t* wt_planes, float* dx, int lddx,
                         int accumulate, int dtype);
size_t fira_dgrad_x3_splitk_planes_bytes(int K);
int fira_dgrad_x3_splitk(void* stream, int M, int K, const float* dy, int lddy, const float* W, uint16_t* planes_ws, float* dx,
                         int lddx, int dtype);

int fira_combination_block_fwd(void* stream, int n_rows, const float* Xc, const float* WqT, const float* WkT,
                               const float* WoT, const float* bqk, const float* bo, const float* vtab, int ldv,
                               const int32_t* mark, float* qk, float* c, const float* gamma, const float* beta, float* sum,
                               float* y, const int32_t* y_rows, float* stats, float dropout, uint64_t seed,
                               uint32_t site_gate, uint32_t site_out, int dtype);

int fira_combination_block_bwd(void* stream, int n_rows, float* dG, const int32_t* rows, const float* sum, const float* stats,
                               const float* gamma, const float* Wo, const float* Wqk, const float* qk, const float* vtab,
                               int ldv, const int32_t* mark, float* dYc, float* dqk, float* dgamma, float* dbeta,
                               float* dvtab, int lddv, float* part, float dropout, uint64_t seed, uint32_t site_gate,
                               uint32_t site_out, int dtype);
int fira_combination_block_bwd_part_floats(void);

int fira_embed_gather_fwd(void* stream, int B, int L, const int32_t* idx, const float* table,
                          const float* pos, float* out, int out_bstride, int out_off);
int fira_embed_gather_bwd(void* stream, int B, int L, const int32_t* idx, float* dtable,
                          const float* dout, int out_bstride, int out_off, int padding_idx);

int fira_combination_fwd(void* stream, int M, const float* qk, const float* vtab, const int32_t* mark,
                         float* out, float dropout, uint64_t seed, uint32_t stream_id);
int fira_combination_bwd(void* stream, int M, const float* qk, const float* vtab, const int32_t* mark,
                         const float* dout, float* dqk, float* dvtab ,
                         float dropout, uint64_t seed, uint32_t stream_id);

int fira_add_layernorm_fwd(void* stream, int M, float* x, const float* res, const float* gamma,
                           const float* beta, float* y, float* stats, float dropout, uint64_t seed,
                           uint32_t stream_id);
int fira_linear_presum_f32(void* stream, int M, int K, const float* X, int ldx, const float* W, const float* bias,
                           const float* res, float* sum, float dropout, uint64_t seed, uint32_t stream_id);
int fira_ln_linear_f32(void* stream, int M, int N, const float* S, int lds, const float* W, const float* bias, float* Y,
                       int ldy, int relu, const float* gamma, const float* beta, float* x_out, float* stats_out);
int fira_ln_bwd_linear_f32(void* stream, int M, int N, const float* dy, const float* Wt, float* dX, const float* relu_mask,
                           const float* sum, const float* stats, const float* gamma, float* ds, float* dx_drop,
                           float* dgamma, float* dbeta, float* part, float dropout, uint64_t seed, uint32_t site);
int fira_linear_layernorm_bf16_fwd(void* stream, int M, const float* X, int ldx, const uint16_t* Wb, int ldb,
                                   const float* bias, const float* res, const float* gamma, const float* beta,
                                   float* sum, float* y, float* stats, float dropout, uint64_t seed,
                                   uint32_t stream_id);
int fira_add_layernorm_bwd(void* stream, int M, const float* dy, const float* sum, const float* stats,
                           const float* gamma, float* ds, float* dx_drop, float* dgamma, float* dbeta,
                           float dropout, uint64_t seed, uint32_t stream_id);

#define FIRA_SITE_GATE 0
#define FIRA_SITE_COMB_OUT 1
#define FIRA_SITE_GCN 2
#define FIRA_SITE_SELF 3
#define FIRA_SITE_CROSS 4
#define FIRA_SITE_FFN 5
#define FIRA_SITE(layer, kind) ((uint32_t)((layer) * 8 + (kind) + 1))
int fira_dropout_mask(void* stream, uint64_t seed, uint32_t site, int64_t n, float p, float* out);

int fira_colsum_f32(void* stream, int M, int N, const float* X, int ldx, float* out);

int fira_attention_fwd(void* stream, int B, int H, int Tq, int Tk, const float* Q, int ldq,
                       const float* K, int ldk, const float* V, int ldv, const int32_t* key_valid,
                       int causal, int q_pos0, float* O, int ldo);
int fira_attention_bwd(void* stream, int B, int H, int Tq, int Tk, const float* Q, int ldq,
                       const float* K, int ldk, const float* V, int ldv, const int32_t* key_valid,
                       int causal, int q_pos0, const float* O, int ldo, const float* dO, int lddo,
                       float* dQ, int lddq, float* dK, int lddk, float* dV, int lddv);
int fira_attention_fwd_ex(void* stream, int B, int H, int Tq, int Tk, const float* Q, int ldq,
                          const float* K, int ldk, const float* V, int ldv, const int32_t* key_valid,
                          int causal, int q_pos0, float* O, int ldo, const int32_t* q_off, int self_kv, int dtype,
                          const int32_t* k_off);
int fira_attention_bwd_ex(void* stream, int B, int H, int Tq, int Tk, const float* Q, int ldq,
                          const float* K, int ldk, const float* V, int ldv, const int32_t* key_valid,
                          int causal, int q_pos0, const float* O, int ldo, const float* dO, int lddo,
                          float* dQ, int lddq, float* dK, int lddk, float* dV, int lddv,
                          const int32_t* q_off, int self_kv, int dtype, const int32_t* k_off);

int fira_decode_attention(void* stream, int BR, int H, int Tk, const float* Q, int ldq, const float* K, int ldk,
                          const float* V, int ldv, const int32_t* key_valid, float* O, int ldo, int kb, int kvb, int qpk,
                          const float* Knew, const float* Vnew, int ldn, float* Kc_out, float* Vc_out,
                          const int32_t* k_off);

int fira_copy_score_fwd(void* stream, int B, int T, int S, const float* src, const float* tgt,
                        const float* w, const float* bias, float* score);
int fira_copy_score_bwd(void* stream, int B, int T, int S, const float* src, const float* tgt,
                        const float* w, const float* dscore, float* dsrc , float* dtgt ,
                        float* dw , float* dbias );

int fira_head_loss(void* stream, int BT, int T, int V, int S, const int32_t* compact_row,
                   float* logits, int ldl, float* score , const int32_t* mem_valid ,
                   float* gate_logits , const int32_t* tar_label ,
                   float* loss_sum, int32_t* n_tok, int32_t* argmax_out, int want_grad);

int fira_adam_step(void* stream, int64_t n, float* p, const float* g, float* m, float* v,
                   float lr, float beta1, float beta2, float eps, int step, const float* inv_scale_ntok);
int fira_adam_step_mb(void* stream, int64_t n, float* p, const float* g0, const float* g1, float* m, float* v,
                      float lr, float beta1, float beta2, float eps, int step, const int32_t* n_tok0,
                      const int32_t* n_tok1);
int fira_adam_step_count(void* stream, int64_t n, float* p, const float* g, float* m, float* v,
                         float lr, float beta1, float beta2, float eps, int step, const float* count);
int fira_pack_stats(void* stream, const float* loss_sum, const int32_t* n_tok, float* out2);
int fira_inv_count(void* stream, const int32_t* n_tok, float* out);

int fira_debug_chain(void* stream, int n, int mode, float* scratch);


int fira_train_fwd_bwd(void* stream, const fira_dims* d, const fira_batch* batch, const float* params,
                       float* grads, void* workspace, size_t workspace_bytes, const fira_train_opts* opts,
                       float* loss_sum, int32_t* n_tok, void* mid_event);

int fira_gemm_wgrad_panel(void* stream, int dtype, int M, int N, int K, const float* A, int lda, const float* B, int ldb,
                          float* C, int ldc, float* colsum, float* scratch, size_t scratch_floats);

int fira_ffn_fwd(void* stream, int M, int F, const float* x, const float* w1, const float* b1, const float* w2, const float* b2,
                 const float* gamma, const float* beta, float* h, float* sum, float* y, float* stats, float dropout,
                 uint64_t seed, uint32_t site, int dtype);
int fira_ffn_bwd(void* stream, int M, int F, const float* dy, const float* x, const float* h, const float* sum,
                 const float* stats, const float* w1, const float* w2, const float* gamma, float* dx, float* dyf_ws,
                 float* dh_ws, float* dw1, float* db1, float* dw2, float* db2, float* dgamma, float* dbeta, float dropout,
                 uint64_t seed, uint32_t site, int dtype);
int fira_head_topk(void* stream, int R, int V, int k, const float* x, const float* wout, const float* bout, float* logits_ws,
                   int ldl, int32_t* ids, float* vals, int dtype);

size_t fira_head_logits_x3_scratch_bytes(int R);
int fira_head_logits_x3(void* stream, int R, int V, const float* x, int ldx, const float* W, const float* bias, float* logits,
                        int ldl, void* scratch);


typedef struct fira_lr_schedule {
    int32_t kind;
    float   base_lr;
    int32_t warmup_steps;
    int32_t decay_steps;
    float   min_lr;
} fira_lr_schedule;
float fira_lr_at(const fira_lr_schedule* s, int step);
int   fira_lr_schedule_check(const fira_lr_schedule* s);

typedef struct fira_adam_opts {
    float   lr, beta1, beta2, eps;
    int32_t step;
    float*  m;
    float*  v;
    const fira_lr_schedule* sched;
} fira_adam_opts;
int fira_train_step(void* stream, const fira_dims* d, const fira_batch* batch, float* params, float* grads,
                    void* workspace, size_t workspace_bytes, const fira_train_opts* opts, float* loss_sum,
                    int32_t* n_tok, const fira_adam_opts* adam);

int fira_train_step_begin(void* stream, const fira_dims* d, const fira_batch* batch, const float* params, float* grads,
                          void* workspace, size_t workspace_bytes, const fira_train_opts* opts, float* loss_sum,
                          int32_t* n_tok, void* mid_event );
int fira_train_step_end(void* stream, float* params, const fira_adam_opts* adam, void* early_event ,
                        const float* count);

int fira_train_step_rows(void* stream, const fira_dims* d, const fira_batch* batch, float* params, float* grads,
                         void* workspace, size_t workspace_bytes, const fira_train_opts* opts, float* loss_sum,
                         int32_t* n_tok, const fira_adam_opts* adam, int32_t* row_step);
int fira_adam_rows_sync(void* stream, const fira_dims* d, float* params, const fira_adam_opts* adam, int32_t* row_step);
int fira_adam_rows_catchup(void* stream, const fira_dims* d, float* params, const fira_adam_opts* adam, int32_t* row_step,
                           int table, const int32_t* ids, int n_ids);
int fira_adam_rows_step(void* stream, const fira_dims* d, float* params, const float* grads, const fira_adam_opts* adam,
                        int32_t* row_step, const int32_t* n_tok, const float* count , int tables );
int fira_train_step_begin_rows(void* stream, const fira_dims* d, const fira_batch* batch, const float* params, float* grads,
                               void* workspace, size_t workspace_bytes, const fira_train_opts* opts, float* loss_sum,
                               int32_t* n_tok, void* mid_event, const fira_adam_opts* adam, int32_t* row_step);
int fira_train_step_end_rows(void* stream, float* params, const fira_adam_opts* adam, void* early_event, const float* count,
                             int32_t* row_step);

typedef struct fira_clip_state {
    float   sq[4];
    float   norm;
    float   coef;
    int32_t zero_flag;
    int32_t n_clipped;
    int32_t n_nonfinite;
    int32_t reserved[7];
} fira_clip_state;
size_t fira_grad_sqsum_scratch_bytes(void);
int fira_grad_sqsum(void* stream, int64_t n, const float* g, fira_clip_state* state, int slot, void* scratch);
int fira_clip_finish(void* stream, fira_clip_state* state, int n_slots, const int32_t* n_tok, const float* count,
                     float max_norm);
int fira_adam_step_clip(void* stream, int64_t n, float* p, const float* g, float* m, float* v, float lr, float beta1,
                        float beta2, float eps, int step, const int32_t* n_tok, const float* count,
                        const fira_clip_state* state);
int fira_adam_rows_step_clip(void* stream, const fira_dims* d, float* params, const float* grads, const fira_adam_opts* adam,
                             int32_t* row_step, const int32_t* n_tok, const float* count, int tables,
                             const fira_clip_state* state);
int fira_train_step_clip(void* stream, const fira_dims* d, const fira_batch* batch, float* params, float* grads,
                         void* workspace, size_t workspace_bytes, const fira_train_opts* opts, float* loss_sum,
                         int32_t* n_tok, const fira_adam_opts* adam, int32_t* row_step , float max_norm,
                         fira_clip_state* state, void* scratch);

int fira_f32_to_bf16(void* stream, int64_t n, const float* in, uint16_t* out);
int fira_bf16_to_f32(void* stream, int64_t n, const uint16_t* in, float* out);

int fira_forward_dev(void* stream, const fira_dims* d, const fira_batch* batch, const float* params,
                     void* workspace, size_t workspace_bytes, int32_t* ids_out, float* loss_sum, int32_t* n_tok,
                     int dtype );

int fira_dev_bleu_stats(void* stream, int B, int T, int V, int L, int S,
                        const int32_t* ids,
                        const int32_t* sou,    const int32_t* sub_token,
                        const int32_t* tar,
                        int32_t* hyp,
                        int32_t* stats);

int fira_mbr_bleu_stats(void* stream, int B, int n, int T,
                        const int32_t* tokens,   const int32_t* length,
                        int32_t* stats);

int fira_decode_begin(void* stream, const fira_dims* d, const fira_batch* batch, const float* params,
                      void* workspace, size_t workspace_bytes, int n_beam);
int fira_decode_step(void* stream, const fira_dims* d, const float* params, void* workspace,
                     size_t workspace_bytes, int B, int n_beam, int step, const int32_t* tokens,
                     const int32_t* parent, float* dist, int32_t* best_id, float* best_p);
#define FIRA_DECODE_KV_BF16 1
int fira_decode_begin_ex(void* stream, const fira_dims* d, const fira_batch* batch, const float* params,
                         void* workspace, size_t workspace_bytes, int n_beam, int flags);
int fira_decode_step_ex(void* stream, const fira_dims* d, const float* params, void* workspace,
                        size_t workspace_bytes, int B, int n_beam, int step, const int32_t* tokens,
                        const int32_t* parent, float* dist, int32_t* best_id, float* best_p, int flags);

int fira_beam_prepare(void* stream, int B, int n_beam, int tar_len, int step, const int32_t* gen, const int32_t* length,
                      int32_t* tokens, int32_t* finished, int32_t* active, int32_t* done);
int fira_beam_select(void* stream, const fira_dims* d, int B, int n_beam, const float* dist, const int32_t* finished,
                     const int32_t* active, const int32_t* done, const int32_t* sou, const int32_t* sub_token,
                     const int32_t* gen_in, const int32_t* len_in, const float* prob_in, int32_t* gen_out,
                     int32_t* len_out, float* prob_out, int32_t* parent);
// ... 68 lines not shown
```

Before: 13560 commits/s.

## Save softmax max and inverse sum in attention forward for reuse in backward

The decoder attention forward now writes per-row softmax statistics (row max and inverse sum) to a workspace buffer during training. A new backward kernel variant reads these stats instead of recomputing the full softmax reductions. It computes dK, dV and dQ per key tile, using an LDS-based tile transpose in place of the old cross-wave rescans. This trades extra workspace and a small store in forward for less recomputation and synchronisation in backward.

```diff
diff --git a/fira_icse_amd/_lib.py b/fira_icse_amd/_lib.py
--- a/fira_icse_amd/_lib.py
+++ b/fira_icse_amd/_lib.py
@@ -102,6 +102,10 @@
     "fira_attention_fwd_ex": (_I, [_P, _I, _I, _I, _I, _P, _I, _P, _I, _P, _I, _P, _I, _I, _P, _I, _P, _I, _I, _P]),
     "fira_attention_bwd_ex": (_I, [_P, _I, _I, _I, _I, _P, _I, _P, _I, _P, _I, _P, _I, _I, _P, _I, _P, _I,
                                    _P, _I, _P, _I, _P, _I, _P, _I, _I, _P]),
+    "fira_attention_fwd_stats": (_I, [_P, _I, _I, _I, _I, _P, _I, _P, _I, _P, _I, _P, _I, _I, _P, _I, _P, _I, _I, _P, _I, _P]),
+    "fira_attention_bwd_stats": (_I, [_P, _I, _I, _I, _I, _P, _I, _P, _I, _P, _I, _P, _I, _I, _P, _I, _P, _I,
+                                      _P, _I, _P, _I, _P, _I, _P, _I, _I, _P, _P]),
+    "fira_train_attention_stats": (_P, [_DP, _P, _I, _I, _I]),
     "fira_decode_attention": (_I, [_P, _I, _I, _I, _P, _I, _P, _I, _P, _I, _P, _P, _I, _I, _I, _I, _P, _P, _I, _P, _P, _P]),
     "fira_copy_score_fwd": (_I, [_P, _I, _I, _I, _P, _P, _P, _P, _P]),
     "fira_copy_score_bwd": (_I, [_P, _I, _I, _I, _P, _P, _P, _P, _P, _P, _P, _P]),
diff --git a/fira_icse_amd/csrc/attention.hip b/fira_icse_amd/csrc/attention.hip
--- a/fira_icse_amd/csrc/attention.hip
+++ b/fira_icse_amd/csrc/attention.hip
@@ -4,6 +4,7 @@
 
 namespace fira {
 
+typedef unsigned int u32v2_t __attribute__((__vector_size__(8)));
 constexpr float SQRT_DH = 5.656854249492381f;
 constexpr float INV_SQRT_DH = 1.0f / SQRT_DH;
 constexpr int MAX_TK = 384;
@@ -72,7 +73,8 @@
                                                                 const int32_t* __restrict__ key_valid, int causal,
                                                                 int q_pos0, float* __restrict__ O, int ldo, int kb,
                                                                 int kvb, int qpk, const int32_t* __restrict__ q_off,
-                                                                int self_kv, const int32_t* __restrict__ k_off) {
+                                                                int self_kv, const int32_t* __restrict__ k_off,
+                                                                float* __restrict__ stats) {
     __shared__ float sm_red[NW][32];
     __shared__ float sm_o[NW > 1 ? NW * 1024 : 1];
     const int b = blockIdx.x / H, h = blockIdx.x % H;
@@ -158,6 +160,11 @@
         for (int w = 0; w < NW; ++w) sum += sm_red[w][l31];
     }
     const float inv_sum = 1.0f / sum;
+    if (stats && wave == 0 && kh == 0) {
+        const rsrc_t rS = buf_rsrc(stats + ((size_t)qb * H + h) * 2, tq > 0 ? ((unsigned)(tq - 1) * (unsigned)H * 2u + 2u) * 4u : 0u);
+        const u32v2_t ms = {(unsigned)__float_as_int(mx), (unsigned)__float_as_int(inv_sum)};
+        __builtin_amdgcn_raw_buffer_store_b64(ms, rS, (unsigned)l31 * (unsigned)H * 8u, 0, 0);
+    }
     f32x16 o;
 #pragma unroll
     for (int r = 0; r < 16; ++r) o[r] = 0.f;
@@ -189,16 +196,58 @@
     }
 }
 
-template <int NW, bool BF>
+template <int NW>
+__device__ __forceinline__ void dq_combine_store(float* sm_o, const f32x16& dq, rsrc_t rdQ, unsigned lddq4, int NT, int t, int lane,
+                                                 int wave, int l31, int kh) {
+    if (NW > 1) {
+        const int nwa = min(NW, NT);
+        if (wave < nwa) {
+#pragma unroll
+            for (int r = 0; r < 16; ++r) sm_o[wave * 1024 + r * 64 + lane] = dq[r];
+        }
+        __syncthreads();
+        for (int idx = t; idx < 1024; idx += NW * 64) {
+            float v = 0.f;
+            for (int w = 0; w < nwa; ++w) v += sm_o[w * 1024 + idx];
+            const int r = idx >> 6, ln = idx & 63;
+            __builtin_amdgcn_raw_buffer_store_b32(__float_as_int(v), rdQ,
+                                                  (unsigned)acc_row(r, ln >> 5) * lddq4 + (unsigned)(ln & 31) * 4u, 0, 0);
+        }
+    } else {
+#pragma unroll
+        for (int r = 0; r < 16; ++r)
+            __builtin_amdgcn_raw_buffer_store_b32(__float_as_int(dq[r]), rdQ,
+                                                  (unsigned)(4 * kh + acc_c(r)) * lddq4 + (unsigned)l31 * 4u, 0, 0);
+    }
+}
+
+__device__ __forceinline__ void tile_transpose(float* slot, const float (&in)[16], float (&out)[16], int l31, int kh) {
+    __builtin_amdgcn_wave_barrier();
+    const int wlane = 128 * kh + (l31 ^ (8 * kh));
+#pragma unroll
+    for (int r = 0; r < 16; ++r) slot[acc_c(r) * 32 + (wlane ^ (((acc_c(r) >> 1) & 5) << 2))] = in[r];
+    __builtin_amdgcn_fence(__ATOMIC_RELEASE, "wavefront");
+    __builtin_amdgcn_wave_barrier();
+    __builtin_amdgcn_fence(__ATOMIC_ACQUIRE, "wavefront");
+    const int swz = (((l31 >> 1) & 7) << 2) ^ (4 * kh);
+#pragma unroll
+    for (int g = 0; g < 4; ++g) {
+        const f32x4v v = *reinterpret_cast<const f32x4v*>(&slot[l31 * 32 + ((8 * g) ^ swz)]);
+        out[4 * g + 0] = v.x; out[4 * g + 1] = v.y; out[4 * g + 2] = v.z; out[4 * g + 3] = v.w;
+    }
+}
+
+template <int NW, bool BF, bool ST>
 __global__ __launch_bounds__(NW * 64) void attention_bwd_kernel(
     int H, int Tq, int Tk, const float* __restrict__ Q, int ldq, const float* __restrict__ K, int ldk,
     const float* __restrict__ V, int ldv, const int32_t* __restrict__ key_valid, int causal, int q_pos0,
     const float* __restrict__ O, int ldo, const float* __restrict__ dO, int lddo, float* __restrict__ dQ, int lddq,
     float* __restrict__ dK, int lddk, float* __restrict__ dV, int lddv, const int32_t* __restrict__ q_off, int self_kv,
-    const int32_t* __restrict__ k_off) {
+    const int32_t* __restrict__ k_off,
+    const float* __restrict__ stats) {
     __shared__ float sm_red[NW][32];
     __shared__ __attribute__((aligned(16))) float sm_m[32], sm_sum[32], sm_delta[32];
-    __shared__ float sm_o[NW > 1 ? NW * 1024 : 1];
+    __shared__ __attribute__((aligned(16))) float sm_o[(NW > 1 || ST) ? NW * 1024 : 1];
     const int b = blockIdx.x / H, h = blockIdx.x % H;
     const int t = threadIdx.x, lane = t & 63, wave = t >> 6;
     const int l31 = lane & 31, kh = lane >> 5;
@@ -231,6 +280,13 @@
     buf_frag(bq, rQ, (unsigned)l31 * ldq4 + fq);
     buf_frag(bdo, rdO, (unsigned)l31 * lddo4 + fq);
     buf_frag(bo, rO, (unsigned)l31 * (unsigned)ldo * 4u + fq);
+    float smx = 0.f, sinv = 0.f;
+    if constexpr (ST) {
+        const rsrc_t rS = buf_rsrc(stats + ((size_t)qb * H + h) * 2, tq > 0 ? ((unsigned)(tq - 1) * (unsigned)H * 2u + 2u) * 4u : 0u);
+        const u32v2_t ms = __builtin_amdgcn_raw_buffer_load_b64(rS, (unsigned)l31 * (unsigned)H * 8u, 0, 0);
+        smx = __int_as_float((int)ms[0]);
+        sinv = __int_as_float((int)ms[1]);
+    }
     float ak[16], av[16], kvv[16];
     float qrow[16], dorow[16];
     int kvld = 0;
@@ -254,6 +310,69 @@
         delta = d + __shfl_xor(d, 32, 64);
     }
 
+    if constexpr (ST) {
+        auto store_rows = [&](const f32x16& v, rsrc_t r, unsigned ld4) {
+#pragma unroll
+            for (int i = 0; i < 16; ++i)
+                __builtin_amdgcn_raw_buffer_store_b32(__float_as_int(v[i]), r,
+                                                      (unsigned)(kt * 32 + 4 * kh + acc_c(i)) * ld4 + (unsigned)l31 * 4u, 0, 0);
+        };
+        f32x16 dq;
+#pragma unroll
+        for (int r = 0; r < 16; ++r) dq[r] = 0.f;
+        if (live) {
+#pragma unroll
+            for (int s = 0; s < 16; ++s) kvv[s] = bit_select(bit_of(tm.valid, acc_c(s)), kvv[s], 0.f);
+            if (!tm.ok) {
+#pragma unroll
+                for (int s = 0; s < 16; ++s) { ak[s] = 0.f; av[s] = 0.f; }
+            }
+            f32x16 acc;
+#pragma unroll
+            for (int r = 0; r < 16; ++r) acc[r] = 0.f;
+            acc = chain16<BF>(ak, bq, acc);
+            float ex[16];
+#pragma unroll
+            for (int s = 0; s < 16; ++s) {
+                float x = bit_select(bit_of(maskedT, acc_c(s)), MASKED2, acc[s] * SCORE2);
+                x = bit_select(bit_of(tm.outside, acc_c(s)), -INFINITY, x);
+                ex[s] = __builtin_amdgcn_exp2f(x - smx);
+            }
+#pragma unroll
+            for (int r = 0; r < 16; ++r) acc[r] = 0.f;
+            acc = chain16<BF>(av, bdo, acc);
+            float dd[16];
+#pragma unroll
+            for (int s = 0; s < 16; ++s) dd[s] = acc[s] - delta;
+            float* slot = sm_o + wave * 1024;
+            float tin[16], tout[16];
+#pragma unroll
+            for (int s = 0; s < 16; ++s)
+                tin[s] = bit_select(bit_of(maskedT, acc_c(s)), 0.f, ex[s] * sinv * dd[s] * INV_SQRT_DH);
+            tile_transpose(slot, tin, tout, l31, kh);
+#pragma unroll
+            for (int r = 0; r < 16; ++r) acc[r] = 0.f;
+            acc = chain16<BF>(tout, qrow, acc);
+            store_rows(acc, rdK, lddk4);
+#pragma unroll
+            for (int s = 0; s < 16; ++s) tin[s] = ex[s] * sinv;
+            tile_transpose(slot, tin, tout, l31, kh);
+#pragma unroll
+            for (int r = 0; r < 16; ++r) acc[r] = 0.f;
+            acc = chain16<BF>(tout, dorow, acc);
+            store_rows(acc, rdV, lddv4);
+            float dsv[16];
+            const float sc = sinv * INV_SQRT_DH;
+#pragma unroll
+            for (int s = 0; s < 16; ++s)
+                dsv[s] = bit_select(bit_of(maskedT, acc_c(s)), 0.f, ex[s] * sc * dd[s]);
+            dq = chain16<BF>(dsv, kvv, dq);
+        } else if (mine) {
+            store_rows(dq, rdK, lddk4);
+            store_rows(dq, rdV, lddv4);
+        }
+        dq_combine_store<NW>(sm_o, dq, rdQ, lddq4, NT, t, lane, wave, l31, kh);
+    } else {
     f32x16 st;
     float mx = -INFINITY;
     if (live) {
@@ -328,26 +447,7 @@
             dsv[s] = bit_select(bit_of(maskedT, acc_c(s)), 0.f, st[s] * sc * (dpt[s] - delta));
         dq = chain16<BF>(dsv, kvv, dq);
     }
-    if (NW > 1) {
-        const int nwa = min(NW, NT);
-        if (wave < nwa) {
-#pragma unroll
-            for (int r = 0; r < 16; ++r) sm_o[wave * 1024 + r * 64 + lane] = dq[r];
-        }
-        __syncthreads();
-        for (int idx = t; idx < 1024; idx += NW * 64) {
-            float v = 0.f;
-            for (int w = 0; w < nwa; ++w) v += sm_o[w * 1024 + idx];
-            const int r = idx >> 6, ln = idx & 63;
-            __builtin_amdgcn_raw_buffer_store_b32(__float_as_int(v), rdQ,
-                                                  (unsigned)acc_row(r, ln >> 5) * lddq4 + (unsigned)(ln & 31) * 4u, 0, 0);
-        }
-    } else {
-#pragma unroll
-        for (int r = 0; r < 16; ++r)
-            __builtin_amdgcn_raw_buffer_store_b32(__float_as_int(dq[r]), rdQ,
-                                                  (unsigned)(4 * kh + acc_c(r)) * lddq4 + (unsigned)l31 * 4u, 0, 0);
-    }
+    dq_combine_store<NW>(sm_o, dq, rdQ, lddq4, NT, t, lane, wave, l31, kh);
 
     if (mine) {
         f32x16 dk, dv;
@@ -389,6 +489,7 @@
             __builtin_amdgcn_raw_buffer_store_b32(__float_as_int(dk[r]), rdK, row * lddk4 + (unsigned)l31 * 4u, 0, 0);
             __builtin_amdgcn_raw_buffer_store_b32(__float_as_int(dv[r]), rdV, row * lddv4 + (unsigned)l31 * 4u, 0, 0);
         }
+    }
     }
 }
 
@@ -673,14 +774,15 @@
 
 int attention_fwd_ex(hipStream_t s, int B, int H, int Tq, int Tk, const float* Q, int ldq, const float* K, int ldk,
                      const float* V, int ldv, const int32_t* key_valid, int causal, int q_pos0, float* O, int ldo,
-                     int kb, int kvb, int qpk, const int32_t* q_off, int self_kv, int bf16, const int32_t* k_off) {
+                     int kb, int kvb, int qpk, const int32_t* q_off, int self_kv, int bf16, const int32_t* k_off, float* stats) {
     ProfScope prof(s, PROF_ATTN, 0.0);
     if (B <= 0) return 0;
     if (int e = check_geometry("attention_fwd", Tq, Tk, ldq, ldk, ldv, Q, K, V)) return e;
     FIRA_REQUIRE(kb >= Tk && kvb >= Tk && qpk >= 1, "attention_fwd: bad batch strides");
+    FIRA_REQUIRE((uintptr_t)stats % 8 == 0, "attention_fwd: stats must be 8-byte aligned");
 #define FIRA_ATT_FWD(NW_, BF_)                                                                                      \
     hipLaunchKernelGGL((attention_fwd_kernel<NW_, BF_>), dim3(B * H), dim3(NW_ * 64), 0, s, H, Tq, Tk, Q, ldq, K, ldk, V, \
-                       ldv, key_valid, causal, q_pos0, O, ldo, kb, kvb, qpk, q_off, self_kv, k_off)
+                       ldv, key_valid, causal, q_pos0, O, ldo, kb, kvb, qpk, q_off, self_kv, k_off, stats)
     if (Tk <= 32) { if (bf16) FIRA_ATT_FWD(1, true); else FIRA_ATT_FWD(1, false); }
     else { if (bf16) FIRA_ATT_FWD(12, true); else FIRA_ATT_FWD(12, false); }
 #undef FIRA_ATT_FWD
@@ -689,25 +791,32 @@
 }
 int attention_fwd(hipStream_t s, int B, int H, int Tq, int Tk, const float* Q, int ldq, const float* K, int ldk,
                   const float* V, int ldv, const int32_t* key_valid, int causal, int q_pos0, float* O, int ldo,
-                  const int32_t* q_off, int self_kv, int bf16, const int32_t* k_off) {
+                  const int32_t* q_off, int self_kv, int bf16, const int32_t* k_off, float* stats) {
     return attention_fwd_ex(s, B, H, Tq, Tk, Q, ldq, K, ldk, V, ldv, key_valid, causal, q_pos0, O, ldo, Tk, Tk, 1, q_off, self_kv,
-                            bf16, k_off);
+                            bf16, k_off, stats);
 }
 
 int attention_bwd(hipStream_t s, int B, int H, int Tq, int Tk, const float* Q, int ldq, const float* K, int ldk,
                   const float* V, int ldv, const int32_t* key_valid, int causal, int q_pos0, const float* O, int ldo,
                   const float* dO, int lddo, float* dQ, int lddq, float* dK, int lddk, float* dV, int lddv,
-                  const int32_t* q_off, int self_kv, int bf16, const int32_t* k_off) {
+                  const int32_t* q_off, int self_kv, int bf16, const int32_t* k_off, const float* stats) {
     ProfScope prof(s, PROF_ATTN, 0.0);
     if (B <= 0) return 0;
     if (int e = check_geometry("attention_bwd", Tq, Tk, ldq, ldk, ldv, Q, K, V)) return e;
     FIRA_REQUIRE(ldo % 4 == 0 && lddo % 4 == 0 && (uintptr_t)O % 16 == 0 && (uintptr_t)dO % 16 == 0,
                  "attention_bwd: O/dO rows must be 16-byte aligned");
-#define FIRA_ATT_BWD(NW_, BF_)                                                                                      \
-    hipLaunchKernelGGL((attention_bwd_kernel<NW_, BF_>), dim3(B * H), dim3(NW_ * 64), 0, s, H, Tq, Tk, Q, ldq, K, ldk, V, \
-                       ldv, key_valid, causal, q_pos0, O, ldo, dO, lddo, dQ, lddq, dK, lddk, dV, lddv, q_off, self_kv, k_off)
-    if (Tk <= 32) { if (bf16) FIRA_ATT_BWD(1, true); else FIRA_ATT_BWD(1, false); }
-    else { if (bf16) FIRA_ATT_BWD(12, true); else FIRA_ATT_BWD(12, false); }
+    FIRA_REQUIRE((uintptr_t)stats % 8 == 0, "attention_bwd: stats must be 8-byte aligned");
+#define FIRA_ATT_BWD(NW_, BF_, ST_)                                                                                 \
+    hipLaunchKernelGGL((attention_bwd_kernel<NW_, BF_, ST_>), dim3(B * H), dim3(NW_ * 64), 0, s, H, Tq, Tk, Q, ldq, K, ldk, V, \
+                       ldv, key_valid, causal, q_pos0, O, ldo, dO, lddo, dQ, lddq, dK, lddk, dV, lddv, q_off, self_kv, k_off, stats)
+#define FIRA_ATT_BWD_NW(NW_)                                                                                        \
+    do {                                                                                                            \
+        if (stats) { if (bf16) FIRA_ATT_BWD(NW_, true, true); else FIRA_ATT_BWD(NW_, false, true); }                \
+        else { if (bf16) FIRA_ATT_BWD(NW_, true, false); else FIRA_ATT_BWD(NW_, false, false); }                    \
+    } while (0)
+    if (Tk <= 32) FIRA_ATT_BWD_NW(1);
+    else FIRA_ATT_BWD_NW(12);
+#undef FIRA_ATT_BWD_NW
 #undef FIRA_ATT_BWD
     FIRA_CHECK_LAUNCH("attention_bwd");
     return 0;
@@ -753,4 +862,23 @@
     return fira::attention_bwd((hipStream_t)stream, B, H, Tq, Tk, Q, ldq, K, ldk, V, ldv, key_valid, causal, q_pos0, O,
                                ldo, dO, lddo, dQ, lddq, dK, lddk, dV, lddv, q_off, self_kv, dtype == FIRA_BF16, k_off);
 }
-}
+int fira_attention_fwd_stats(void* stream, int B, int H, int Tq, int Tk, const float* Q, int ldq, const float* K, int ldk,
+                             const float* V, int ldv, const int32_t* key_valid, int causal, int q_pos0, float* O, int ldo,
+                             const int32_t* q_off, int self_kv, int dtype, const int32_t* k_off, int qpk, float* stats) {
+    FIRA_REQUIRE(dtype == FIRA_F32 || dtype == FIRA_BF16, "fira_attention_fwd_stats: dtype must be FIRA_F32 or FIRA_BF16");
+    FIRA_REQUIRE(!(k_off && self_kv), "fira_attention_fwd_stats: k_off (ragged memory rows) and self_kv exclude each other");
+    FIRA_REQUIRE(qpk >= 1 && B % qpk == 0 && !(self_kv && qpk != 1), "fira_attention_fwd_stats: B must be a multiple of qpk (1 with self_kv)");
+    return fira::attention_fwd_ex((hipStream_t)stream, B, H, Tq, Tk, Q, ldq, K, ldk, V, ldv, key_valid, causal, q_pos0, O, ldo, Tk,
+                                  Tk, qpk, q_off, self_kv, dtype == FIRA_BF16, k_off, stats);
+}
+int fira_attention_bwd_stats(void* stream, int B, int H, int Tq, int Tk, const float* Q, int ldq, const float* K, int ldk,
+                             const float* V, int ldv, const int32_t* key_valid, int causal, int q_pos0, const float* O,
+                             int ldo, const float* dO, int lddo, float* dQ, int lddq, float* dK, int lddk, float* dV,
+                             int lddv, const int32_t* q_off, int self_kv, int dtype, const int32_t* k_off, const float* stats) {
+    FIRA_REQUIRE(dtype == FIRA_F32 || dtype == FIRA_BF16, "fira_attention_bwd_stats: dtype must be FIRA_F32 or FIRA_BF16");
+    FIRA_REQUIRE(!(k_off && self_kv), "fira_attention_bwd_stats: k_off (ragged memory rows) and self_kv exclude each other");
+    FIRA_REQUIRE(stats, "fira_attention_bwd_stats: stats (the forward's soft-max statistics) must be given");
+    return fira::attention_bwd((hipStream_t)stream, B, H, Tq, Tk, Q, ldq, K, ldk, V, ldv, key_valid, causal, q_pos0, O,
+                               ldo, dO, lddo, dQ, lddq, dK, lddk, dV, lddv, q_off, self_kv, dtype == FIRA_BF16, k_off, stats);
+}
+}
diff --git a/fira_icse_amd/csrc/engine.h b/fira_icse_amd/csrc/engine.h
--- a/fira_icse_amd/csrc/engine.h
+++ b/fira_icse_amd/csrc/engine.h
@@ -177,11 +177,12 @@
                   const float* V, int ldv, const int32_t* key_valid, int causal, int q_pos0, float* O, int ldo,
                   const int32_t* q_off = nullptr, int self_kv = 0,
                   int bf16 = 0,
-                  const int32_t* k_off = nullptr);
+                  const int32_t* k_off = nullptr,
+                  float* stats = nullptr);
 int attention_fwd_ex(hipStream_t s, int B, int H, int Tq, int Tk, const float* Q, int ldq, const float* K, int ldk,
                      const float* V, int ldv, const int32_t* key_valid, int causal, int q_pos0, float* O, int ldo,
                      int kb, int kvb, int qpk, const int32_t* q_off = nullptr, int self_kv = 0, int bf16 = 0,
-                     const int32_t* k_off = nullptr);
+                     const int32_t* k_off = nullptr, float* stats = nullptr);
 int decode_attention(hipStream_t s, int BR, int H, int Tk, const float* Q, int ldq, const float* K, int ldk,
                      const float* V, int ldv, const int32_t* key_valid, float* O, int ldo, int kb, int kvb, int qpk,
                      const float* Knew = nullptr, const float* Vnew = nullptr, int ldn = 0, float* Kc_out = nullptr,
@@ -197,7 +198,8 @@
 int attention_bwd(hipStream_t s, int B, int H, int Tq, int Tk, const float* Q, int ldq, const float* K, int ldk,
                   const float* V, int ldv, const int32_t* key_valid, int causal, int q_pos0, const float* O, int ldo,
                   const float* dO, int lddo, float* dQ, int lddq, float* dK, int lddk, float* dV, int lddv,
-                  const int32_t* q_off = nullptr, int self_kv = 0, int bf16 = 0, const int32_t* k_off = nullptr);
+                  const int32_t* q_off = nullptr, int self_kv = 0, int bf16 = 0, const int32_t* k_off = nullptr,
+                  const float* stats = nullptr);
 int copy_score_fwd(hipStream_t s, int B, int T, int S, const float* src, const float* tgt, const float* w,
                    const float* bias, float* score);
 int copy_score_fwd_ex(hipStream_t s, int B, int T, int S, const float* src, const float* tgt, const float* w,
diff --git a/fira_icse_amd/csrc/engine.hip b/fira_icse_amd/csrc/engine.hip
--- a/fira_icse_amd/csrc/engine.hip
+++ b/fira_icse_amd/csrc/engine.hip
@@ -28,6 +28,7 @@
 };
 struct DecSave {
     float *qkv, *ao, *s_a, *st_a, *x_a, *qc, *ao2, *s_c, *st_c, *x_c, *h, *s_f, *st_f, *x_f;
+    float *att_s = nullptr, *att_c = nullptr;
 };
 
 struct EncGrad {
@@ -172,6 +173,7 @@
                 DecGrad& h = decg[l];
                 h.dYf = a.f((size_t)TB * D); h.dh = a.f((size_t)TB * F); h.dYc = a.f((size_t)TB * D);
                 h.dq = a.f((size_t)TB * D); h.dYs = a.f((size_t)TB * D); h.dqkv = a.f((size_t)TB * 3 * D);
+                dec[l].att_s = a.f((size_t)TB * d.n_head * 2); dec[l].att_c = a.f((size_t)TB * d.n_head * 2);
             }
         }
         return a.used;
@@ -949,7 +951,7 @@
             const int32_t* q_off = c.dec_off ? c.dec_off + ln.b0 : nullptr;
             TRY(consume(3 * D, c.P + w.wqkv, c.P + w.bqkv, e.qkv, 0));
             TRY(attention_fwd(s, ln.nb, H, p.T, p.T, e.qkv, 3 * D, e.qkv + D, 3 * D, e.qkv + 2 * D, 3 * D, p.tar_valid + (size_t)ln.b0 * p.T,
-                              1, 0, e.ao, D, q_off, 1, attn_bf16()));
+                              1, 0, e.ao, D, q_off, 1, attn_bf16(), nullptr, c.G ? e.att_s : nullptr));
             TRY(close_block(D, e.ao, c.P + w.wo_s, c.P + w.bo_s, st.x, c.P + w.lns_g, c.P + w.lns_b, e.s_a, e.x_a, e.st_a,
                             site(l, SITE_SELF), true, nullptr, nullptr, 0, nullptr));
             st.x = e.x_a;
@@ -964,7 +966,7 @@
             }
             TRY(attention_fwd(s, ln.nb, H, p.T, Sm, e.qc, D, p.kv_all + l * 2 * D, p.kvp, p.kv_all + l * 2 * D + D, p.kvp,
                               c.kv_ragged ? p.mem_valid_c : p.mem_valid, 0, 0, e.ao2, D, q_off, 0, attn_bf16(),
-                              c.kv_ragged ? p.mem_off + ln.b0 : nullptr));
+                              c.kv_ragged ? p.mem_off + ln.b0 : nullptr, c.G ? e.att_c : nullptr));
             TRY(close_block(D, e.ao2, c.P + w.wo_c, c.P + w.bo_c, e.x_a, c.P + w.lnc_g, c.P + w.lnc_b, e.s_c, e.x_c, e.st_c,
                             site(l, SITE_CROSS), true, nullptr, nullptr, 0, nullptr));
             st.x = e.x_c;
@@ -1142,7 +1144,7 @@
             if (q) TRY(linear_wgrad_grouped(s, c.Td, D, D, g.dYc, D, e.ao2, D, G + w.wo_c, G + w.bo_c));
             TRY(attention_bwd(ls, ln.nb, H, p.T, Sm, e.qc, D, p.kv_all + l * 2 * D, p.kvp, p.kv_all + l * 2 * D + D, p.kvp,
                               p.mem_valid_c, 0, 0, e.ao2, D, bx, D, g.dq, D, p.dkv_all + l * 2 * D, p.kvp,
-                              p.dkv_all + l * 2 * D + D, p.kvp, q_off, 0, attn_bf16(), p.mem_off + ln.b0));
+                              p.dkv_all + l * 2 * D + D, p.kvp, q_off, 0, attn_bf16(), p.mem_off + ln.b0, e.att_c));
             if (c.n_lanes == 1) TRY(dmem_pair());
             else if (so && l % 2 == 0 && k < 2) {
                 ev_kv_done[k] = side().ev();
@@ -1156,7 +1158,7 @@
             if (q) TRY(linear_wgrad_grouped(s, c.Td, D, D, g.dYs, D, e.ao, D, G + w.wo_s, G + w.bo_s));
             TRY(attention_bwd(ls, ln.nb, H, p.T, p.T, e.qkv, 3 * D, e.qkv + D, 3 * D, e.qkv + 2 * D, 3 * D,
                               p.tar_valid + (size_t)ln.b0 * p.T, 1, 0, e.ao, D, bx, D, g.dqkv, 3 * D, g.dqkv + D, 3 * D, g.dqkv + 2 * D,
-                              3 * D, q_off, 1, attn_bf16()));
+                              3 * D, q_off, 1, attn_bf16(), nullptr, e.att_s));
             if (q) TRY(linear_wgrad_grouped(s, c.Td, 3 * D, D, g.dqkv, 3 * D, x_in, D, G + w.wqkv, G + w.bqkv));
             TRY(linear_dgrad(ls, nr, 3 * D, D, g.dqkv + r0 * 3 * D, 3 * D, c.P + w.wqkv, by + r0 * D, D, true));
         }
@@ -2017,6 +2019,12 @@
     dp.build(workspace, *d, B, n_beam);
     return dp.enc.mem;
 }
+const float* fira_train_attention_stats(const fira_dims* d, void* workspace, int B, int layer, int cross) {
+    if (!get_layout(d) || !workspace || layer < 0 || layer >= d->n_layer) return nullptr;
+    Plan p;
+    p.build(workspace, *d, B, true);
+    return cross ? p.dec[layer].att_c : p.dec[layer].att_s;
+}
 const int32_t* fira_decode_mem_valid(const fira_dims* d, void* workspace, int B, int n_beam) {
     if (!get_layout(d) || !workspace) return nullptr;
     DecodePlan dp;
diff --git a/fira_icse_amd/ops.py b/fira_icse_amd/ops.py
--- a/fira_icse_amd/ops.py
+++ b/fira_icse_amd/ops.py
@@ -319,6 +319,31 @@
     return dq, dk, dv
 
 
+def attention_ragged_fwd_stats(q, k, v, key_valid, q_off, Tq, Tk, causal=False, self_kv=False, dtype=0, heads=8, k_off=None,
+                               qpk=1):
+    B = q_off.numel() - 1
+    o = torch.zeros_like(q)
+    stats = torch.zeros((q.shape[0], heads, 2), dtype=torch.float32, device=q.device)
+    ko = None if k_off is None else _i32(k_off)
+    check(_lib.lib().fira_attention_fwd_stats(cur_stream(), B, heads, Tq, Tk, ptr(q), q.stride(0), ptr(k), k.stride(0), ptr(v),
+                                              v.stride(0), ptr(_i32(key_valid)), int(causal), 0, ptr(o), 256, ptr(_i32(q_off)),
+                                              int(self_kv), dtype, ptr(ko), qpk, ptr(stats)), "fira_attention_fwd_stats")
+    return o, stats
+
+
+def attention_ragged_bwd_stats(q, k, v, key_valid, o, do, stats, q_off, Tq, Tk, causal=False, self_kv=False, dtype=0, heads=8,
+                               k_off=None, fill=0.0):
+    B = q_off.numel() - 1
+    dq, dk, dv = torch.full_like(q, fill), torch.full_like(k, fill), torch.full_like(v, fill)
+    ko = None if k_off is None else _i32(k_off)
+    check(_lib.lib().fira_attention_bwd_stats(cur_stream(), B, heads, Tq, Tk, ptr(q), q.stride(0), ptr(k), k.stride(0), ptr(v),
+                                              v.stride(0), ptr(_i32(key_valid)), int(causal), 0, ptr(_f32(o)), 256,
+                                              ptr(_f32(do)), 256, ptr(dq), dq.stride(0), ptr(dk), dk.stride(0), ptr(dv),
+                                              dv.stride(0), ptr(_i32(q_off)), int(self_kv), dtype, ptr(ko), ptr(_f32(stats))),
+          "fira_attention_bwd_stats")
+    return dq, dk, dv
+
+
 def attention_fwd(q, k, v, key_valid, causal=False, q_pos0=0, heads=8):
     B, Tq, _ = q.shape
     Tk = k.shape[1]
diff --git a/include/fira_hip.h b/include/fira_hip.h
--- a/include/fira_hip.h
+++ b/include/fira_hip.h
@@ -192,6 +192,16 @@
                           int causal, int q_pos0, const float* O, int ldo, const float* dO, int lddo,
                           float* dQ, int lddq, float* dK, int lddk, float* dV, int lddv,
                           const int32_t* q_off, int self_kv, int dtype, const int32_t* k_off);
+int fira_attention_fwd_stats(void* stream, int B, int H, int Tq, int Tk, const float* Q, int ldq,
+                             const float* K, int ldk, const float* V, int ldv, const int32_t* key_valid,
+                             int causal, int q_pos0, float* O, int ldo, const int32_t* q_off, int self_kv, int dtype,
+                             const int32_t* k_off, int qpk, float* stats);
+int fira_attention_bwd_stats(void* stream, int B, int H, int Tq, int Tk, const float* Q, int ldq,
+                             const float* K, int ldk, const float* V, int ldv, const int32_t* key_valid,
+                             int causal, int q_pos0, const float* O, int ldo, const float* dO, int lddo,
+                             float* dQ, int lddq, float* dK, int lddk, float* dV, int lddv,
+                             const int32_t* q_off, int self_kv, int dtype, const int32_t* k_off, const float* stats);
+const float* fira_train_attention_stats(const fira_dims* d, void* workspace, int B, int layer, int cross);
 
 int fira_decode_attention(void* stream, int BR, int H, int Tk, const float* Q, int ldq, const float* K, int ldk,
                           const float* V, int ldv, const int32_t* key_valid, float* O, int ldo, int kb, int kvb, int qpk,
```

Result: no change. 13650 commits/s (median of 6 runs) (+0.6%).
